# hashicorp/consul

Measured on NVIDIA H100. Metric: million node-ticks/sec, higher is better.
Workload: dtype u32

## Files before the change

__graft_entry__.py:

```python
from __future__ import annotations

import os
import subprocess
import sys

ROOT = os.path.dirname(os.path.abspath(__file__))
CSRC = os.path.join(ROOT, "consul_b200", "csrc")
LIBGSIM = os.path.join(ROOT, "consul_b200", "libgsim.so")
LIBORACLE = os.path.join(ROOT, "oracle", "liboracle.so")
LIBHOSTEMU = os.path.join(ROOT, "tests", "hostemu", "libgsim_hostemu.so")
LIBHOSTEMU_COUNTED = os.path.join(ROOT, "tests", "hostemu", "libgsim_hostemu_counted.so")
FACADE_DEMO = os.path.join(ROOT, "tests", "hostemu", "serf_facade_check")

NVCC_FLAGS = ["-gencode", "arch=compute_90a,code=sm_90a", "-lineinfo", "-O3", "-std=c++17", "-fmad=false",
              "-Xcompiler", "-fPIC", "-Xcompiler", "-ffp-contract=off", "-Xcompiler", "-pthread", "-shared"]


def _newer(target: str, sources) -> bool:
    if not os.path.exists(target):
        return False
    t = os.path.getmtime(target)
    return all(os.path.getmtime(s) <= t for s in sources)


def _run(cmd):
    print("+", " ".join(cmd), flush=True)
    subprocess.run(cmd, check=True, cwd=ROOT)


def _sources(*dirs_and_ext):
    out = []
    for d, exts in dirs_and_ext:
        for f in sorted(os.listdir(d)):
            if f.endswith(exts):
                out.append(os.path.join(d, f))
    return out


def build_oracle(force: bool = False) -> None:
    hdr = _sources((os.path.join(ROOT, "include"), (".h",)))
    osrc = [os.path.join(ROOT, "oracle", "oracle.cpp")]
    if force or not _newer(LIBORACLE, osrc + hdr):
        _run(["g++", "-O3", "-mavx2", "-ffp-contract=off", "-std=c++17", "-fopenmp", "-fPIC", "-shared", "-o",
              LIBORACLE] + osrc)


LIBORACLE_IMPAIR = os.path.join(ROOT, "tests", "oracle_impair", "liboracle_impair.so")
IMPAIR_PATCH = os.path.join(ROOT, "tests", "oracle_impair", "impair.patch")


def _apply_patch(text: str, patch: str, name: str = IMPAIR_PATCH) -> str:
    hunks, cur = [], None
    for line in patch.splitlines(keepends=True):
        if line.startswith("@@"):
            cur = ([], [])
            hunks.append(cur)
        elif cur is not None and line[:1] in (" ", "-", "+"):
            if line[:1] != "+":
                cur[0].append(line[1:])
            if line[:1] != "-":
                cur[1].append(line[1:])
    for old, new in hunks:
        old, new = "".join(old), "".join(new)
        if text.count(old) != 1:
            raise RuntimeError(f"{name}: a hunk does not apply to oracle/oracle.cpp")
        text = text.replace(old, new)
    return text


def build_impair_oracle(force: bool = False) -> None:
    import tempfile
    hdr = _sources((os.path.join(ROOT, "include"), (".h",)))
    osrc = [os.path.join(ROOT, "oracle", "oracle.cpp"), IMPAIR_PATCH]
    if not force and _newer(LIBORACLE_IMPAIR, osrc + hdr):
        return
    with open(osrc[0]) as f, open(IMPAIR_PATCH) as pf:
        text = _apply_patch(f.read(), pf.read())
    with tempfile.TemporaryDirectory() as tmp:
        src = os.path.join(tmp, "oracle_impair.cpp")
        with open(src, "w") as f:
            f.write(text)
        _run(["g++", "-O3", "-mavx2", "-ffp-contract=off", "-std=c++17", "-fopenmp", "-fPIC", "-shared",
              "-I", os.path.join(ROOT, "oracle"), "-o", LIBORACLE_IMPAIR, src])


LIBORACLE_PAUSE = os.path.join(ROOT, "tests", "oracle_pause", "liboracle_pause.so")
PAUSE_PATCH = os.path.join(ROOT, "tests", "oracle_pause", "pause.patch")


def build_pause_oracle(force: bool = False) -> None:
    import tempfile
    hdr = _sources((os.path.join(ROOT, "include"), (".h",)))
    osrc = [os.path.join(ROOT, "oracle", "oracle.cpp"), IMPAIR_PATCH, PAUSE_PATCH]
    if not force and _newer(LIBORACLE_PAUSE, osrc + hdr):
        return
    with open(osrc[0]) as f, open(IMPAIR_PATCH) as pf, open(PAUSE_PATCH) as qf:
        text = _apply_patch(_apply_patch(f.read(), pf.read()), qf.read(), PAUSE_PATCH)
    with tempfile.TemporaryDirectory() as tmp:
        src = os.path.join(tmp, "oracle_pause.cpp")
        with open(src, "w") as f:
            f.write(text)
        _run(["g++", "-O3", "-mavx2", "-ffp-contract=off", "-std=c++17", "-fopenmp", "-fPIC", "-shared",
              "-I", os.path.join(ROOT, "oracle"), "-o", LIBORACLE_PAUSE, src])


LIBORACLE_REACH = os.path.join(ROOT, "tests", "oracle_reach", "liboracle_reach.so")
REACH_PATCH = os.path.join(ROOT, "tests", "oracle_reach", "reach.patch")


def build_reach_oracle(force: bool = False) -> None:
    import tempfile
    hdr = _sources((os.path.join(ROOT, "include"), (".h",)))
    osrc = [os.path.join(ROOT, "oracle", "oracle.cpp"), IMPAIR_PATCH, PAUSE_PATCH, REACH_PATCH]
    if not force and _newer(LIBORACLE_REACH, osrc + hdr):
        return
    with open(osrc[0]) as f, open(IMPAIR_PATCH) as pf, open(PAUSE_PATCH) as qf, open(REACH_PATCH) as rf:
        text = _apply_patch(_apply_patch(_apply_patch(f.read(), pf.read()), qf.read(), PAUSE_PATCH), rf.read(),
                            REACH_PATCH)
    with tempfile.TemporaryDirectory() as tmp:
        src = os.path.join(tmp, "oracle_reach.cpp")
        with open(src, "w") as f:
            f.write(text)
        _run(["g++", "-O3", "-mavx2", "-ffp-contract=off", "-std=c++17", "-fopenmp", "-fPIC", "-shared",
              "-I", os.path.join(ROOT, "oracle"), "-o", LIBORACLE_REACH, src])


LIBORACLE_PIGGYBACK = os.path.join(ROOT, "tests", "oracle_piggyback", "liboracle_piggyback.so")
PIGGYBACK_PATCH = os.path.join(ROOT, "tests", "oracle_piggyback", "piggyback.patch")


def build_piggyback_oracle(force: bool = False) -> None:
    import tempfile
    hdr = _sources((os.path.join(ROOT, "include"), (".h",)))
    patches = [IMPAIR_PATCH, PAUSE_PATCH, REACH_PATCH, PIGGYBACK_PATCH]
    osrc = [os.path.join(ROOT, "oracle", "oracle.cpp")] + patches
    if not force and _newer(LIBORACLE_PIGGYBACK, osrc + hdr):
        return
    with open(osrc[0]) as f:
        text = f.read()
    for patch in patches:
        with open(patch) as pf:
            text = _apply_patch(text, pf.read(), patch)
    with tempfile.TemporaryDirectory() as tmp:
        src = os.path.join(tmp, "oracle_piggyback.cpp")
        with open(src, "w") as f:
            f.write(text)
        _run(["g++", "-O3", "-mavx2", "-ffp-contract=off", "-std=c++17", "-fopenmp", "-fPIC", "-shared",
              "-I", os.path.join(ROOT, "oracle"), "-o", LIBORACLE_PIGGYBACK, src])


def build(force: bool = False) -> None:
    hdr = _sources((CSRC, (".h",)), (os.path.join(ROOT, "include"), (".h", ".hpp")))
    srcs = [os.path.join(CSRC, "gs_cuda.cu"), os.path.join(CSRC, "gs_vmm.cu"), os.path.join(CSRC, "gs_api.cpp")]
    if force or not _newer(LIBGSIM, srcs + hdr):
        nvcc = os.environ.get("NVCC", "nvcc")
        _run([nvcc] + NVCC_FLAGS + ["-o", LIBGSIM] + srcs)
    build_oracle(force)
    build_impair_oracle(force)
    build_pause_oracle(force)
    build_reach_oracle(force)
    build_piggyback_oracle(force)
    hsrc = [os.path.join(CSRC, "gs_api.cpp"), os.path.join(ROOT, "tests", "hostemu", "hostemu_backend.cpp")]
    if force or not _newer(LIBHOSTEMU, hsrc + hdr):
        _run(["g++", "-O2", "-ffp-contract=off", "-std=c++17", "-pthread", "-fPIC", "-shared",
              "-DGS_MAKE_BACKEND=gs_make_hostemu_backend", "-o", LIBHOSTEMU] + hsrc)
    csrc = hsrc + [os.path.join(ROOT, "tests", "hostemu", "stretch_counting.cpp")]
    if force or not _newer(LIBHOSTEMU_COUNTED, csrc + hdr + [os.path.join(ROOT, "tests", "hostemu", "counting_backend.cpp")]):
        _run(["g++", "-O2", "-ffp-contract=off", "-std=c++17", "-pthread", "-fPIC", "-shared",
              "-DGS_MAKE_BACKEND=gs_make_stretch_counting_backend", "-o", LIBHOSTEMU_COUNTED] + csrc)
    sys.path.insert(0, ROOT)
    import consul_b200


def smoke() -> None:
    sys.path.insert(0, ROOT)
    sys.path.insert(0, os.path.join(ROOT, "tests"))
    if not (os.path.exists(LIBGSIM) and os.path.exists(LIBORACLE)):
        build()
    from consul_b200 import Pool, lan_config, PRED_ALL_RUMORS_CONVERGED
    from oracle_binding import OraclePool

    n = 4096
    cfg = lan_config(capacity=n + 1, n_initial=n, seed=0x5EED0001)
    gpu = Pool(cfg)
    ora = OraclePool(cfg)
    for p in (gpu, ora):
        x = p.member_add()
        assert p.join(x, [0]) == 1
    tg = gpu.run_until(PRED_ALL_RUMORS_CONVERGED, 0, 400, 1)
    to = ora.run_until(PRED_ALL_RUMORS_CONVERGED, 0, 400, 1)
    gpu.step(64)
    ora.step(64)
    hg, ho = gpu.state_hash(), ora.state_hash()
    assert tg == to, (tg, to)
    assert hg == ho, (hg, ho)
    assert gpu.launch_count() > 0
    print(f"smoke ok: n={n + 1} converged at tick {tg}, state hash {hg[0]:016x} == oracle, "
          f"{gpu.launch_count()} kernel launches")


if __name__ == "__main__":
    build(force="--force" in sys.argv)
    if "--smoke" in sys.argv:
        smoke()
```

consul_b200/csrc/gs_cuda.cu:

```cuda
#include <cuda_runtime.h>
#include <stdio.h>
#include <stdlib.h>
#include <string.h>

#include <map>

#include "gs_aux.h"
#include "gs_backend.h"
#include "gs_query.h"
#include "gs_vmm.h"

#define GS_BLOCK 256
#define GS_GRAPH_TICKS 64
#define GS_WIN_GRAPH 8
#ifndef GS_STRETCH_TICKS
#define GS_STRETCH_TICKS 16
#endif

namespace {

template <bool COORDS>
struct DevSinkT {
  static constexpr bool kCoords = COORDS;
  uint32_t* s_stat;
  uint32_t* s_heard;
  uint32_t* s_q;
  __device__ __forceinline__ void activity() { s_q[0] = 1u; }
  __device__ __forceinline__ void horizon(uint32_t h) { atomicMin(&s_q[1], h); }
  __device__ __forceinline__ void stat(int idx, uint32_t v) { atomicAdd(&s_stat[idx * 32 + (threadIdx.x & 31u)], v); }
  __device__ __forceinline__ void heard(uint32_t r) { atomicAdd(&s_heard[r * 32u + (threadIdx.x & 31u)], 1u); }
  __device__ __forceinline__ void crashed_dead(const GsDev& d, uint32_t t) {
    uint32_t old = atomicSub_system(d.crashed_alive, 1u);
    if (old == 1u) *d.crashed_dead_tick = t;
  }
  __device__ __forceinline__ void log_event(const GsDev& d, const GsGlobals& g, uint32_t t,
                                            uint32_t type, uint32_t subject, uint32_t observer,
                                            uint32_t ltime) {
    uint32_t pos = atomicAdd_system(&d.evlog_cursor[0], 1u);
    if (pos < g.evlog_cap) {
      GsEventRec e;
      e.tick = t;
      e.type = type;
      e.subject = subject;
      e.observer = observer;
      e.ltime = ltime;
      e.reserved = 0u;
      d.evlog[pos] = e;
    } else {
      atomicAdd_system(&d.evlog_cursor[1], 1u);
    }
  }
};
typedef DevSinkT<false> DevSink;

#ifndef GS_MIN_BLOCKS
#define GS_MIN_BLOCKS 4
#endif
#define GS_WARPS (GS_BLOCK / 32)
#define GS_ROUND 4

__device__ __forceinline__ uint32_t gs_smem_addr(const void* p) { return (uint32_t)__cvta_generic_to_shared(p); }
__device__ __forceinline__ void gs_mbar_init(uint64_t* bar, uint32_t arrivals) {
  asm volatile("mbarrier.init.shared::cta.b64 [%0], %1;" ::"r"(gs_smem_addr(bar)), "r"(arrivals) : "memory");
}
__device__ __forceinline__ void gs_mbar_expect_tx(uint64_t* bar, uint32_t bytes) {
  asm volatile("mbarrier.arrive.expect_tx.shared::cta.b64 _, [%0], %1;" ::"r"(gs_smem_addr(bar)), "r"(bytes) : "memory");
}
__device__ __forceinline__ void gs_bulk_g2s(void* smem_dst, const void* gsrc, uint32_t bytes, uint64_t* bar) {
  asm volatile("cp.async.bulk.shared::cluster.global.mbarrier::complete_tx::bytes [%0], [%1], %2, [%3];" ::"r"(
                   gs_smem_addr(smem_dst)),
               "l"(gsrc), "r"(bytes), "r"(gs_smem_addr(bar))
               : "memory");
}
__device__ __forceinline__ bool gs_mbar_wait(uint64_t* bar, uint32_t parity) {
  for (uint32_t spin = 0; spin < (1u << 24); ++spin) {
    uint32_t done;
    asm volatile(
        "{\n\t.reg .pred p;\n\t"
        "mbarrier.try_wait.parity.shared::cta.b64 p, [%1], %2;\n\t"
        "selp.u32 %0, 1, 0, p;\n\t}"
        : "=r"(done)
        : "r"(gs_smem_addr(bar)), "r"(parity)
        : "memory");
    if (done) return true;
  }
  return false;
}

__device__ __forceinline__ void gs_ranks_wait(const GsDev& d, const GsGlobals& g, uint32_t t) {
  if (threadIdx.x < g.world) {
    uint32_t v;
    do {
      asm volatile("ld.acquire.sys.global.u32 %0, [%1];" : "=r"(v) : "l"(d.tick_flags[g.rank] + threadIdx.x) : "memory");
    } while ((int32_t)(v - t) < 0);
  }
  __syncthreads();
}
__device__ __forceinline__ void gs_ranks_release(const GsDev& d, const GsGlobals& g, uint32_t t_done) {
  __syncthreads();
  if (threadIdx.x == 0u) {
    __threadfence_system();
    const uint32_t arrived = atomicAdd(d.done_ctr, 1u);
    if (arrived == gridDim.x - 1u) {
      __threadfence_system();
      *d.done_ctr = 0u;
      __threadfence_system();
      for (uint32_t r = 0; r < g.world; ++r)
        asm volatile("st.release.sys.global.u32 [%0], %1;" ::"l"(d.tick_flags[r] + g.rank), "r"(t_done) : "memory");
    }
  }
}

__device__ __forceinline__ void gs_q_publish(const GsDev& d, const GsGlobals& g, const uint32_t* s_q, uint32_t t) {
  if (s_q[0] != 0u) {
    if (g.world <= 1u) atomicMax(d.qstate[0] + GS_Q_LAST_ACTIVE, t + 1u);
    else for (uint32_t r = 0; r < g.world; ++r) atomicMax_system(d.qstate[r] + GS_Q_LAST_ACTIVE, t + 1u);
  }
  if (s_q[1] != GS_NEVER) {
    if (g.world <= 1u) atomicMin(d.qstate[0] + GS_Q_HORIZON, s_q[1]);
    else for (uint32_t r = 0; r < g.world; ++r) atomicMin_system(d.qstate[r] + GS_Q_HORIZON, s_q[1]);
  }
}

template <bool COORDS>
__device__ __noinline__ void gs_row_step_impaired_call(const GsDev* dp, const GsGlobals* gp, uint32_t i, uint32_t t,
                                                       uint32_t inb, uint32_t* s_stat, uint32_t* s_heard, uint32_t* s_q) {
  DevSinkT<COORDS> sink{s_stat, s_heard, s_q};
  gs_row_step_body<true>(*dp, *gp, i, t, t % gp->GI, inb, sink);
}
template <bool COORDS, bool IMPAIRED>
__device__ __noinline__ void gs_row_step_pig_call(const GsDev* dp, const GsGlobals* gp, uint32_t i, uint32_t t,
                                                  uint32_t inb, uint32_t* s_stat, uint32_t* s_heard, uint32_t* s_q) {
  DevSinkT<COORDS> sink{s_stat, s_heard, s_q};
  gs_row_step_body<IMPAIRED, true>(*dp, *gp, i, t, t % gp->GI, inb, sink);
}
template <bool COORDS>
__device__ __noinline__ void gs_row_step_call(const GsDev* dp, const GsGlobals* gp, uint32_t i, uint32_t t,
                                              uint32_t inb, uint32_t* s_stat, uint32_t* s_heard, uint32_t* s_q) {
  if (dp->imp_loss != nullptr) {
    gs_row_step_impaired_call<COORDS>(dp, gp, i, t, inb, s_stat, s_heard, s_q);
    return;
  }
  DevSinkT<COORDS> sink{s_stat, s_heard, s_q};
  gs_row_step_body<false>(*dp, *gp, i, t, t % gp->GI, inb, sink);
}

template <bool COORDS>
__device__ __forceinline__ void gs_row_step_any(const GsDev* dp, const GsGlobals* gp, uint32_t i, uint32_t t,
                                                uint32_t inb, uint32_t* s_stat, uint32_t* s_heard, uint32_t* s_q) {
  if (dp->pig == nullptr) gs_row_step_call<COORDS>(dp, gp, i, t, inb, s_stat, s_heard, s_q);
  else if (dp->imp_loss != nullptr) gs_row_step_pig_call<COORDS, true>(dp, gp, i, t, inb, s_stat, s_heard, s_q);
  else gs_row_step_pig_call<COORDS, false>(dp, gp, i, t, inb, s_stat, s_heard, s_q);
}

struct GsStretchCtl {
  GsStretch out;
  uint32_t violation;
  uint32_t end, floor, depth;
};
__device__ __forceinline__ uint32_t gs_stretch_stop(const GsStretchCtl& c, uint32_t last_active) {
  const uint32_t quiet_at = (last_active > c.floor ? last_active : c.floor) + c.depth;
  return quiet_at < c.end ? quiet_at : c.end;
}

template <bool COORDS>
__global__ void __launch_bounds__(GS_BLOCK, GS_MIN_BLOCKS)
    gs_tick_kernel(const __grid_constant__ GsDev d, const GsGlobals* __restrict__ gp, uint32_t k_off,
                   const GsStretchCtl* __restrict__ stretch) {
  __shared__ uint32_t s_stat[GS_NSTAT * 32];
  __shared__ uint32_t s_heard[32 * 32];
  __shared__ __align__(128) uint32_t s_inb[GS_WARPS][GS_ROUND][GS_TILE];
  __shared__ __align__(128) uint32_t s_due[GS_WARPS][GS_ROUND][GS_TILE];
  __shared__ __align__(8) uint64_t s_bar[GS_WARPS];
  __shared__ uint32_t s_q[2];
  __shared__ uint16_t s_work[GS_WARPS * GS_ROUND * GS_TILE];
  __shared__ uint32_t s_rtile[GS_WARPS];
  __shared__ uint32_t s_wn[2], s_wtake[2];
  static_assert(GS_WARPS <= 8 && GS_ROUND <= 4 && GS_TILE == 128, "s_work entries are 3 + 2 + 7 bits");
  const uint32_t tid = threadIdx.x;
  for (uint32_t x = tid; x < GS_NSTAT * 32u; x += GS_BLOCK) s_stat[x] = 0u;
  for (uint32_t x = tid; x < 32u * 32u; x += GS_BLOCK) s_heard[x] = 0u;
  if (tid == 64u) s_q[0] = 0u;
  if (tid == 65u) s_q[1] = GS_NEVER;
  if (tid >= 66u && tid < 68u) s_wn[tid - 66u] = 0u;
  if (tid >= 68u && tid < 70u) s_wtake[tid - 68u] = 0u;
  if (tid >= 96u && tid < 96u + GS_WARPS) gs_mbar_init(&s_bar[tid - 96u], 1u);
  asm volatile("fence.mbarrier_init.release.cluster;" ::: "memory");
  asm volatile("griddepcontrol.launch_dependents;" ::: "memory");
  asm volatile("griddepcontrol.wait;" ::: "memory");
  if (stretch != nullptr && *d.tick_base + k_off >= gs_stretch_stop(*stretch, __ldcg(d.qstate[0] + GS_Q_LAST_ACTIVE)))
    return;
  __syncthreads();
  const GsGlobals& g = *gp;
  const uint32_t t = *d.tick_base + k_off;
  if (g.world > 1u) gs_ranks_wait(d, g, t);
  const uint32_t cur = t & 1u, P = g.P, pslot = t % P, gslot = t % g.GI;
  const uint32_t pslot_t = (t + P - g.T % P) % P;
  const uint32_t lane = tid & 31u, wib = tid >> 5;
  uint32_t tile_lo = 0, tile_hi = (g.n + GS_TILE - 1u) / GS_TILE;
  if (g.world > 1u) {
    const uint32_t per = g.rows_per_rank / GS_TILE;
    tile_lo = g.rank * per < tile_hi ? g.rank * per : tile_hi;
    tile_hi = tile_lo + per < tile_hi ? tile_lo + per : tile_hi;
  }
  const uint32_t n_warps = gridDim.x * GS_WARPS, n_tiles = tile_hi - tile_lo;
  const uint32_t wid = blockIdx.x * GS_WARPS + wib;
  const uint32_t t_begin = tile_lo + (uint32_t)(((uint64_t)wid * n_tiles) / n_warps);
  const uint32_t t_end = tile_lo + (uint32_t)(((uint64_t)(wid + 1u) * n_tiles) / n_warps);
  const uint32_t* __restrict__ inbox_cur = d.inbox[t & g.ring_mask];
  const bool gated = g.phase_gate != 0u;
  const uint32_t shift = g.phase_shift;
  DevSinkT<COORDS> sink{s_stat, s_heard, s_q};

  const uint32_t max_run = (n_tiles + n_warps - 1u) / n_warps, n_rounds = (max_run + GS_ROUND - 1u) / GS_ROUND;
  bool did_work = false;
  const bool sys_scan = g.world > 1u && (g.flags & 4u);
  auto bring = [&](uint32_t r) {
    const uint32_t b0 = t_begin + r * GS_ROUND < t_end ? t_begin + r * GS_ROUND : t_end;
    const uint32_t b1 = b0 + GS_ROUND < t_end ? b0 + GS_ROUND : t_end;
    const uint32_t tiles = b1 - b0;
    if (!tiles) return;
    uint32_t gate_mask = 0;
    for (uint32_t x = 0; x < tiles; ++x) {
      bool gate = true;
      if (gated) {
        const uint32_t pp = gs_probe_phase(g.rot_p, (b0 + x) >> shift, P);
        gate = pp == pslot || pp == pslot_t;
      }
      gate_mask |= gate ? 1u << x : 0u;
    }
    const size_t off0 = (size_t)b0 * GS_TILE;
    if (sys_scan) {
      for (uint32_t x = 0; x < tiles; ++x) {
        uint4 v;
        asm volatile("ld.relaxed.sys.global.v4.u32 {%0,%1,%2,%3}, [%4];"
                     : "=r"(v.x), "=r"(v.y), "=r"(v.z), "=r"(v.w) : "l"(inbox_cur + off0 + x * GS_TILE + lane * 4u) : "memory");
        *reinterpret_cast<uint4*>(&s_inb[wib][x][lane * 4u]) = v;
        const uint4 dv = (gate_mask >> x) & 1u ? *reinterpret_cast<const uint4*>(d.due + off0 + x * GS_TILE + lane * 4u)
                                               : make_uint4(GS_NEVER, GS_NEVER, GS_NEVER, GS_NEVER);
        *reinterpret_cast<uint4*>(&s_due[wib][x][lane * 4u]) = dv;
      }
      __syncwarp();
      return;
    }
    for (uint32_t x = 0; x < tiles; ++x)
      if (!((gate_mask >> x) & 1u))
        *reinterpret_cast<uint4*>(&s_due[wib][x][lane * 4u]) = make_uint4(GS_NEVER, GS_NEVER, GS_NEVER, GS_NEVER);
    __syncwarp();
    if (lane == 0u) {
      asm volatile("fence.proxy.async.shared::cta;" ::: "memory");
      gs_mbar_expect_tx(&s_bar[wib], (tiles + __popc(gate_mask)) * GS_TILE * 4u);
      gs_bulk_g2s(&s_inb[wib][0][0], inbox_cur + off0, tiles * GS_TILE * 4u, &s_bar[wib]);
      for (uint32_t x = 0; x < tiles; ++x)
        if ((gate_mask >> x) & 1u) gs_bulk_g2s(&s_due[wib][x][0], d.due + off0 + x * GS_TILE, GS_TILE * 4u, &s_bar[wib]);
    }
  };
  bring(0u);
  for (uint32_t round = 0; round < n_rounds; ++round) {
  const uint32_t par = round & 1u;
  const uint32_t r_begin = t_begin + round * GS_ROUND < t_end ? t_begin + round * GS_ROUND : t_end;
  const uint32_t r_end = r_begin + GS_ROUND < t_end ? r_begin + GS_ROUND : t_end;
  if (r_end > r_begin && !sys_scan && !gs_mbar_wait(&s_bar[wib], round & 1u)) {
    if (lane == 0u) atomicExch(d.qstate[g.rank] + GS_Q_VIOLATION, t + 1u);
  }
  for (uint32_t tile = r_begin; tile < r_end; ++tile) {
    const uint32_t st = tile - r_begin;
    uint4 i4 = *reinterpret_cast<const uint4*>(&s_inb[wib][st][lane * 4u]);
    const uint4 d4 = *reinterpret_cast<const uint4*>(&s_due[wib][st][lane * 4u]);
    if (__any_sync(0xFFFFFFFFu, (i4.x | i4.y | i4.z | i4.w) != 0u)) {
      const uint32_t m0 = tile * GS_TILE + lane * 4u;
      const uint4 h4 = __ldcg(reinterpret_cast<const uint4*>(d.heard + m0));
      uint32_t* const w_cur = d.inbox[t & g.ring_mask] + m0;
      uint32_t* const w4 = &i4.x;
      const uint32_t* const h = &h4.x;
      const uint32_t* const du = &d4.x;
      bool stale_any = false;
#pragma unroll
      for (uint32_t u = 0; u < 4u; ++u) {
        const bool pp = g.pp_interval != 0u && gs_pp_due(g.pp_interval, g.rot_pp, (m0 + u) / g.phase_group, t);
        if (w4[u] != 0u && gs_mail_is_stale(g, w4[u], h[u], du[u] == t, pp)) {
          w_cur[u] = 0u;
          s_inb[wib][st][lane * 4u + u] = 0u;
          w4[u] = 0u;
          stale_any = true;
        }
      }
      if (stale_any) sink.activity();
    }
    bool mine = (i4.x | i4.y | i4.z | i4.w) != 0u || d4.x == t || d4.y == t || d4.z == t || d4.w == t;
    bool pp_tile = false;
    if (g.pp_interval != 0u) {
      if (gated) {
        pp_tile = gs_pp_due(g.pp_interval, g.rot_pp, tile >> shift, t);
      } else {
#pragma unroll
        for (uint32_t u = 0; u < 4u; ++u)
          pp_tile |= gs_pp_due(g.pp_interval, g.rot_pp, (tile * GS_TILE + lane * 4u + u) / g.phase_group, t);
      }
      mine |= pp_tile;
    }
    if (__any_sync(0xFFFFFFFFu, mine)) {
      did_work = true;
      __syncwarp();
      const uint32_t base = tile * GS_TILE + lane;
      bool act[4], cand[4];
      bool any_cand = false;
#pragma unroll
      for (int u = 0; u < 4; ++u) {
        const uint32_t w = s_inb[wib][st][u * 32 + lane];
        const bool due_now = s_due[wib][st][u * 32 + lane] == t;
        act[u] = w != 0u || due_now ||
                 (g.pp_interval != 0u && gs_pp_due(g.pp_interval, g.rot_pp, (base + 32u * u) / g.phase_group, t));
        cand[u] = w == 0u && due_now;
        any_cand |= cand[u];
      }
      if (__any_sync(0xFFFFFFFFu, any_cand)) {
        GsFastProbe f[4];
#pragma unroll
        for (int u = 0; u < 4; ++u)
          if (cand[u]) gs_fast_load(d, cur, base + 32u * u, f[u]);
#pragma unroll
        for (int u = 0; u < 4; ++u)
          if (cand[u]) cand[u] = gs_fast_target(d, g, cur, base + 32u * u, f[u]);
        uint32_t n_probe = 0, n_ack = 0;
#pragma unroll
        for (int u = 0; u < 4; ++u) {
          bool acked = false;
          const bool done = cand[u] && gs_fast_finish(d, g, sink, base + 32u * u, t, f[u], &acked);
          if (done) act[u] = false;
          n_probe += __popc(__ballot_sync(0xFFFFFFFFu, done));
          n_ack += __popc(__ballot_sync(0xFFFFFFFFu, done && acked));
        }
        if (lane == 0u && n_probe) {
          atomicAdd(&s_stat[GS_ST_PROBES * 32], n_probe);
          atomicAdd(&s_stat[GS_ST_ACTIVE_ROWS * 32], n_probe);
          if (n_ack) atomicAdd(&s_stat[GS_ST_ACKS * 32], n_ack);
        }
      }
      uint32_t bal[4], n_act = 0;
#pragma unroll
      for (int u = 0; u < 4; ++u) {
        bal[u] = __ballot_sync(0xFFFFFFFFu, act[u]);
        n_act += __popc(bal[u]);
      }
      if (n_act) {
        uint32_t pos = 0;
        if (lane == 0u) pos = atomicAdd(&s_wn[par], n_act);
        pos = __shfl_sync(0xFFFFFFFFu, pos, 0);
        const uint32_t below = (1u << lane) - 1u, key = (wib << 9) | (st << 7) | lane;
#pragma unroll
        for (int u = 0; u < 4; ++u) {
          if (act[u]) s_work[pos + __popc(bal[u] & below)] = (uint16_t)(key | ((uint32_t)u << 5));
          pos += __popc(bal[u]);
        }
      }
    }
  }
  if (lane == 0u) s_rtile[wib] = r_begin;
  __syncwarp();
  if (round + 1u < n_rounds) bring(round + 1u);
  __syncthreads();
  if (tid == 0u) s_wn[par ^ 1u] = s_wtake[par ^ 1u] = 0u;
  const uint32_t n_work = s_wn[par];
  for (;;) {
    uint32_t idx = 0;
    if (lane == 0u) idx = atomicAdd(&s_wtake[par], 32u);
    idx = __shfl_sync(0xFFFFFFFFu, idx, 0);
    if (idx >= n_work) break;
    did_work = true;
    if (idx + lane < n_work) {
      const uint32_t e = s_work[idx + lane];
      const uint32_t i = (s_rtile[e >> 9] + ((e >> 7) & 3u)) * GS_TILE + (e & 127u);
      gs_row_step_any<COORDS>(&d, gp, i, t, __ldcg(inbox_cur + i), s_stat, s_heard, s_q);
    }
  }
  __syncthreads();
  }
  if (g.world > 1u && did_work && !(g.flags & 8u)) __threadfence_system();
  __syncthreads();
  if (tid < GS_NSTAT) {
    uint32_t v = 0;
    for (uint32_t x = 0; x < 32u; ++x) v += s_stat[tid * 32u + ((x + tid) & 31u)];
    if (v) atomicAdd(&d.stats[tid], (unsigned long long)v);
  } else if (tid >= 32u && tid < 32u + GS_MAX_RUMORS) {
    uint32_t r = tid - 32u, c = 0;
    for (uint32_t x = 0; x < 32u; ++x) c += s_heard[r * 32u + ((x + r) & 31u)];
    if (c) {
      uint32_t old = atomicAdd_system(&d.heard_cnt[r], c);
      if (old + c == g.up_count) d.conv_tick[r] = t;
    }
  }
  if (tid == 0u) gs_q_publish(d, g, s_q, t);
  if (g.world > 1u) gs_ranks_release(d, g, t + 1u);
}

template <bool COORDS>
__device__ __noinline__ void gs_window_generic(const GsDev* dp, const GsGlobals* gp, uint32_t gb, uint32_t g_end,
                                               uint32_t tf00, uint32_t tf01, uint32_t tf02, uint32_t tf03,
                                               uint32_t tx00, uint32_t tx01, uint32_t tx02, uint32_t tx03,
                                               uint32_t t0, uint32_t w1, uint32_t* s_stat, uint32_t* s_heard,
                                               uint32_t* s_q, uint32_t* counts) {
  const GsDev& d = *dp;
  const GsGlobals& g = *gp;
  const GsHot h = gs_hot(g);
  const uint32_t P = h.P, T = h.T, lane = threadIdx.x & 31u;
  const uint32_t tf0[4] = {tf00, tf01, tf02, tf03}, tx0[4] = {tx00, tx01, tx02, tx03};
  const bool fast_ok =
      h.loss_thr == 0u && h.graph_n == 0u && d.coord == nullptr && d.imp_loss == nullptr && h.pp_interval == 0u;
  DevSinkT<COORDS> sink{s_stat, s_heard, s_q};
  uint32_t n_probe = 0, n_ack = 0;
  bool did_work = false;
  (void)did_work;
#pragma unroll 1
    for (uint32_t s0 = t0; s0 < w1; s0 += P) {
    const uint32_t off = s0 - t0;
    uint32_t tf[4], tx[4], due[4];
    bool cand[4], slow[4];
    bool any_slow = false;
#pragma unroll
    for (int u = 0; u < 4; ++u) {
      if (gb + u < g_end) {
        tf[u] = tf0[u] + off;
        tx[u] = tx0[u] + off;
        due[u] = __ldcg(d.due + (gb + u) * 32u + lane);
      } else {
        tf[u] = tx[u] = GS_NEVER;
        due[u] = GS_NEVER - 1u;
      }
      cand[u] = fast_ok && due[u] == tf[u] && tf[u] < w1;
      slow[u] = (due[u] == tf[u] && tf[u] < w1 && !fast_ok) || (due[u] == tx[u] && tx[u] < w1);
    }
    GsFastProbe f[4];
#pragma unroll
    for (int u = 0; u < 4; ++u)
      if (cand[u]) gs_fast_load(d, tf[u] & 1u, (gb + u) * 32u + lane, f[u]);
#pragma unroll
    for (int u = 0; u < 4; ++u)
      if (cand[u]) {
        const bool okk = gs_fast_target(d, h, tf[u] & 1u, (gb + u) * 32u + lane, f[u]);
        if (!okk) { cand[u] = false; slow[u] = true; }
      }
#pragma unroll
    for (int u = 0; u < 4; ++u) {
      bool acked = false, done = false;
      if (cand[u]) {
        done = gs_fast_finish(d, h, sink, (gb + u) * 32u + lane, tf[u], f[u], &acked);
        if (!done) slow[u] = true;
        else if (!acked && tf[u] + T < w1) slow[u] = true;
      }
      n_probe += done ? 1u : 0u;
      n_ack += done && acked ? 1u : 0u;
      any_slow |= slow[u];
    }
    if (__any_sync(0xFFFFFFFFu, any_slow)) {
      did_work = true;
#pragma unroll 1
      for (int u = 0; u < 4; ++u) {
        const bool sl = u == 0 ? slow[0] : u == 1 ? slow[1] : u == 2 ? slow[2] : slow[3];
        if (!__any_sync(0xFFFFFFFFu, sl)) continue;
        const uint32_t a = u == 0 ? tf[0] : u == 1 ? tf[1] : u == 2 ? tf[2] : tf[3];
        const uint32_t b = u == 0 ? tx[0] : u == 1 ? tx[1] : u == 2 ? tx[2] : tx[3];
        const uint32_t i = (gb + u) * 32u + lane;
#pragma unroll 1
        for (int which = 0; which < 2; ++which) {
          const uint32_t t = which == 0 ? (a < b ? a : b) : (a < b ? b : a);
          if (t >= w1) break;
          if (sl && __ldcg(d.due + i) == t) gs_row_step_any<COORDS>(&d, gp, i, t, 0u, s_stat, s_heard, s_q);
        }
      }
    }
    }
  counts[0] = n_probe;
  counts[1] = n_ack;
}

#ifndef GS_WIN_BLOCKS
#define GS_WIN_BLOCKS 4
#endif
#ifndef GS_WIN_BLOCKS_CLOSED
#define GS_WIN_BLOCKS_CLOSED 4
#endif

template <bool COORDS, bool PRISTINE>
__global__ void __launch_bounds__(GS_BLOCK, PRISTINE ? GS_WIN_BLOCKS_CLOSED : GS_WIN_BLOCKS)
    gs_window_kernel(const __grid_constant__ GsDev d, const GsGlobals* __restrict__ gp, uint32_t k_off, uint32_t n_ticks,
                     uint32_t mode) {
  __shared__ uint32_t s_stat[GS_NSTAT * 32];
  __shared__ uint32_t s_heard[32 * 32];
  __shared__ uint32_t s_q[2];
  __shared__ uint32_t s_spec[GS_MAX_SPECIAL + 1];
  const uint32_t tid = threadIdx.x;
  for (uint32_t x = tid; x < GS_NSTAT * 32u; x += GS_BLOCK) s_stat[x] = 0u;
  for (uint32_t x = tid; x < 32u * 32u; x += GS_BLOCK) s_heard[x] = 0u;
  if (tid == 64u) s_q[0] = 0u;
  if (tid == 65u) s_q[1] = GS_NEVER;
  asm volatile("griddepcontrol.launch_dependents;" ::: "memory");
  asm volatile("griddepcontrol.wait;" ::: "memory");
  if (tid == 66u) s_spec[GS_MAX_SPECIAL] = gs_special_members(*gp, s_spec);
  __syncthreads();
  const GsGlobals& g = *gp;
  const GsHot h = gs_hot(g);
  const bool cyclic = (mode & 2u) != 0u;
  const uint32_t world = g.world, rank = g.rank, n_spec = s_spec[GS_MAX_SPECIAL];
  uint32_t* const qs = d.qstate[rank];
  const uint32_t t0 = *d.tick_base + k_off;
  const uint32_t reached = __ldcg(qs + GS_Q_WIN_END), horizon = __ldcg(qs + GS_Q_HORIZON);
  if (reached < t0) return;
  uint32_t w1 = t0 + n_ticks;
  if (horizon < w1) w1 = horizon;
  if (w1 <= t0) return;
  if (world > 1u) gs_ranks_wait(d, g, t0);
  const uint32_t P = h.P, T = h.T, lane = tid & 31u, wib = tid >> 5;
  uint32_t tile_lo = 0, tile_hi = (h.n + GS_TILE - 1u) / GS_TILE;
  if (world > 1u) {
    const uint32_t per = g.rows_per_rank / GS_TILE;
    tile_lo = rank * per < tile_hi ? rank * per : tile_hi;
    tile_hi = tile_lo + per < tile_hi ? tile_lo + per : tile_hi;
  }
  const uint32_t n_warps = gridDim.x * GS_WARPS, grp_lo = tile_lo * 4u, grp_hi = tile_hi * 4u;
  const uint32_t run = (grp_hi - grp_lo + n_warps - 1u) / n_warps;
  const uint32_t wid = blockIdx.x * GS_WARPS + wib;
  const uint32_t g_begin = grp_lo + wid * run < grp_hi ? grp_lo + wid * run : grp_hi;
  const uint32_t g_end = g_begin + run < grp_hi ? g_begin + run : grp_hi;
  const uint32_t shift = g.phase_shift + 2u, t0_mod = t0 % P, rot_p = g.rot_p;
  const uint32_t win_q = (w1 - t0) / P, win_r = (w1 - t0) - win_q * P;
  const bool fast_ok =
      h.loss_thr == 0u && h.graph_n == 0u && d.coord == nullptr && d.imp_loss == nullptr && h.pp_interval == 0u;
  DevSinkT<COORDS> sink{s_stat, s_heard, s_q};
  bool did_work = false;
  uint32_t n_probe = 0, n_ack = 0;
  uint32_t pg = g_begin >> shift;
  uint32_t pp = (pg % P + rot_p) % P;
  const uint32_t g_first = cyclic ? (grp_lo + wid * 4u < grp_hi ? grp_lo + wid * 4u : grp_hi) : g_begin;
  const uint32_t g_step = cyclic ? n_warps * 4u : 4u, g_lim = cyclic ? grp_hi : g_end;
  for (uint32_t gb = g_first; gb < g_lim; gb += g_step) {
    if (cyclic) {
      pg = gb >> shift;
      pp = (pg % P + rot_p) % P;
    }
    uint32_t tf0[4], tx0[4];
#pragma unroll
    for (int u = 0; u < 4; ++u) {
      const uint32_t grp = gb + u;
      if (grp < g_lim) {
        const uint32_t q = grp >> shift;
        if (q != pg) {
          pp = pp + 1u == P ? 0u : pp + 1u;
          pg = q;
        }
        uint32_t a = pp + P - t0_mod;
        a = a >= P ? a - P : a;
        uint32_t b = a + T;
        b = b >= P ? b - P : b;
        tf0[u] = t0 + a;
        tx0[u] = t0 + b;
      } else {
        tf0[u] = tx0[u] = GS_NEVER;
      }
    }
    uint32_t lo = t0;
#pragma unroll 1
    for (;;) {
      uint32_t stuck = GS_NEVER;
      if constexpr (PRISTINE) {
        uint32_t cnt = 0;
        uint32_t du[4], kk[4], mm[4], cu[4], pa[4];
#pragma unroll
        for (int u = 0; u < 4; ++u) {
          const uint32_t i = (gb + u) * 32u + lane;
          du[u] = GS_NEVER;
          kk[u] = mm[u] = cu[u] = pa[u] = 0u;
          if (gb + u < g_lim) {
            du[u] = __ldcg(d.due + i);
            if (fast_ok) {
              kk[u] = d.key[tf0[u] & 1u][i];
              mm[u] = d.meta[i];
              cu[u] = d.cursor[i];
              pa[u] = d.pass[i];
            }
          }
        }
#pragma unroll
        for (int u = 0; u < 4; ++u) {
          if (gb + u >= g_lim) continue;
          const uint32_t i = (gb + u) * 32u + lane;
          uint32_t due = du[u];
          if (fast_ok && due >= lo && due < w1) {
            uint32_t later = 0u;
            bool on_phase = due == tf0[u];
            if (!on_phase && due > tf0[u]) {
              later = (due - tf0[u]) / P;
              on_phase = later * P == due - tf0[u];
            }
            if (on_phase) {
              const uint32_t k0 = ((due ^ tf0[u]) & 1u) ? d.key[due & 1u][i] : kk[u];
              const uint32_t m = mm[u];
              if (gs_key_truth(k0) == GS_TRUTH_UP && gs_key_rank(k0) == GS_RANK_ALIVE && gs_meta_stage(m) == GS_STAGE_IDLE &&
                  !(m & (GS_META_DIRTY | GS_META_ISOLATED))) {
                const GsU4 rk = gs_perm_keys(h.seed_lo, h.seed_hi, i, pa[u]);
                const uint32_t kt = win_q + (win_r > tf0[u] - t0 ? 1u : 0u) - later;
                const uint32_t k = gs_pristine_probes_k(h.n, h.perm_bits, rk, i, cu[u], kt, s_spec, n_spec);
                if (k) {
                  const uint32_t aw = gs_meta_aw(m);
                  if (aw) d.meta[i] = gs_meta_set_aw(m, aw > k ? aw - k : 0u);
                  d.cursor[i] = cu[u] + k;
                  due += k * P;
                  d.due[i] = due;
                  cnt += k;
                }
              }
            }
          }
          if (due >= lo && due < w1 && due < stuck) stuck = due;
        }
        n_probe += cnt;
        n_ack += cnt;
      } else
      {
        uint32_t mm[4], cu[4], du[4], m_in[4], cu_in[4], du_in[4], kt[4];
        GsU4 rk[4];
        bool live[4], in_rng[4];
        uint32_t cnt = 0;
        {
          uint32_t kk[4], pa[4];
#pragma unroll
          for (int u = 0; u < 4; ++u) {
            const uint32_t i = (gb + u) * 32u + lane;
            in_rng[u] = gb + u < g_lim;
            du[u] = GS_NEVER;
            kk[u] = mm[u] = cu[u] = pa[u] = 0u;
            if (in_rng[u]) {
              du[u] = __ldcg(d.due + i);
              if (fast_ok) {
                kk[u] = d.key[tf0[u] & 1u][i];
                mm[u] = d.meta[i];
                cu[u] = d.cursor[i];
                pa[u] = d.pass[i];
              }
            }
          }
#pragma unroll
          for (int u = 0; u < 4; ++u) {
            const uint32_t i = (gb + u) * 32u + lane;
            live[u] = false;
            kt[u] = 0u;
            m_in[u] = mm[u];
            cu_in[u] = cu[u];
            du_in[u] = du[u];
            if (!in_rng[u] || !fast_ok || du[u] < lo || du[u] >= w1) continue;
            uint32_t later = 0u;
            if (du[u] != tf0[u]) {
              if (du[u] < tf0[u]) continue;
              later = (du[u] - tf0[u]) / P;
              if (later * P != du[u] - tf0[u]) continue;
            }
            const uint32_t k = ((du[u] ^ tf0[u]) & 1u) ? d.key[du[u] & 1u][i] : kk[u];
            live[u] = gs_key_truth(k) == GS_TRUTH_UP && gs_key_rank(k) == GS_RANK_ALIVE &&
                      gs_meta_stage(mm[u]) == GS_STAGE_IDLE && !(mm[u] & (GS_META_DIRTY | GS_META_ISOLATED));
            rk[u] = gs_perm_keys(h.seed_lo, h.seed_hi, i, pa[u]);
            kt[u] = win_q + (win_r > tf0[u] - t0 ? 1u : 0u) - later;
          }
        }
        for (;;) {
          bool go[4];
          bool any = false;
#pragma unroll
          for (int u = 0; u < 4; ++u) {
            go[u] = live[u] && du[u] < w1;
            any |= go[u];
          }
          if (!__any_sync(0xFFFFFFFFu, any)) break;
          uint32_t c[4], kc[4];
#pragma unroll
          for (int u = 0; u < 4; ++u) {
            c[u] = 0u;
            if (go[u]) {
              if (cu[u] >= h.n) {
                live[u] = go[u] = false;
              } else {
                c[u] = gs_perm(cu[u], h.n, h.perm_bits, rk[u]);
                if (c[u] == (gb + u) * 32u + lane) live[u] = go[u] = false;
              }
            }
          }
#pragma unroll
          for (int u = 0; u < 4; ++u) kc[u] = go[u] ? gs_peer_key(d, du[u] & 1u, c[u], false) : 0u;
#pragma unroll
          for (int u = 0; u < 4; ++u) {
            if (!go[u]) continue;
            const uint32_t i = (gb + u) * 32u + lane;
            if (gs_key_truth(kc[u]) != GS_TRUTH_UP || gs_key_rank(kc[u]) != GS_RANK_ALIVE || gs_key_pending(kc[u]) ||
                gs_extra(h, nullptr, i, c[u]) + gs_extra(h, nullptr, c[u], i) > T) {
              live[u] = false;
              continue;
            }
            const uint32_t aw = gs_meta_aw(mm[u]);
            mm[u] = gs_meta_set_aw(mm[u], aw ? aw - 1u : 0u);
            du[u] += P;
            cu[u] += 1u;
            ++cnt;
          }
        }
#pragma unroll
        for (int u = 0; u < 4; ++u) {
          if (!in_rng[u]) continue;
          const uint32_t i = (gb + u) * 32u + lane;
          if (cu[u] != cu_in[u]) d.cursor[i] = cu[u];
          if (du[u] != du_in[u]) d.due[i] = du[u];
          if (mm[u] != m_in[u]) d.meta[i] = mm[u];
          if (du[u] >= lo && du[u] < w1 && du[u] < stuck) stuck = du[u];
        }
        n_probe += cnt;
        n_ack += cnt;
      }
      stuck = __reduce_min_sync(0xFFFFFFFFu, stuck);
      if (stuck == GS_NEVER) break;
      {
        const uint32_t off = (stuck - t0) / P * P, s_lo = t0 + off, s_hi = s_lo + P < w1 ? s_lo + P : w1;
        uint32_t add[2] = {0u, 0u};
        gs_window_generic<COORDS>(&d, gp, gb, g_lim, tf0[0] + off, tf0[1] + off, tf0[2] + off, tf0[3] + off, tx0[0] + off,
                                  tx0[1] + off, tx0[2] + off, tx0[3] + off, s_lo, s_hi, s_stat, s_heard, s_q, add);
        n_probe += add[0];
        n_ack += add[1];
        did_work = true;
        lo = s_lo + P;
        if (lo >= w1) break;
      }
    }
  }
  did_work |= n_probe != 0u;
  if (n_probe) {
    atomicAdd(&s_stat[GS_ST_PROBES * 32 + lane], n_probe);
    atomicAdd(&s_stat[GS_ST_ACTIVE_ROWS * 32 + lane], n_probe);
    if (n_ack) atomicAdd(&s_stat[GS_ST_ACKS * 32 + lane], n_ack);
  }
  if (world > 1u && did_work) __threadfence_system();
  __syncthreads();
  if (tid < GS_NSTAT) {
    uint32_t v = 0;
    for (uint32_t x = 0; x < 32u; ++x) v += s_stat[tid * 32u + ((x + tid) & 31u)];
    if (v) atomicAdd(&d.stats[tid], (unsigned long long)v);
  }
  if (tid == 0u) {
    if (s_q[0] != 0u || (n_ticks > P && s_q[1] != GS_NEVER)) atomicExch(qs + GS_Q_VIOLATION, t0 + 1u);
    s_q[0] = 0u;
    gs_q_publish(d, g, s_q, t0);
    atomicMax(qs + GS_Q_WIN_END, w1);
  }
  if (world > 1u) gs_ranks_release(d, g, w1);
}

__global__ void __launch_bounds__(GS_BLOCK)
    gs_quiet_scan_kernel(GsDev d, const GsGlobals* __restrict__ gp, uint32_t now, const uint32_t* now_at, uint32_t first,
                         uint32_t count) {
  __shared__ uint32_t s_min;
  if (threadIdx.x == 0u) s_min = GS_NEVER;
  __syncthreads();
  const GsGlobals& g = *gp;
  if (now_at != nullptr) now = *now_at;
  uint32_t h = GS_NEVER;
  for (uint32_t x = blockIdx.x * GS_BLOCK + threadIdx.x; x < count; x += gridDim.x * GS_BLOCK) {
    const uint32_t i = first + x;
    if (i >= g.n) break;
    if (gs_key_truth(d.key[now & 1u][i]) != GS_TRUTH_UP) continue;
    const uint32_t stage = gs_meta_stage(d.meta[i]);
    if (stage == GS_STAGE_IDLE) continue;
    const uint32_t due = d.due[i];
    const uint32_t e = stage == GS_STAGE_WAIT_T ? due - g.T + g.P : due;
    if (e < h) h = e;
  }
  h = __reduce_min_sync(0xFFFFFFFFu, h);
  if ((threadIdx.x & 31u) == 0u && h != GS_NEVER) atomicMin(&s_min, h);
  __syncthreads();
  if (threadIdx.x == 0u && s_min != GS_NEVER) {
    if (g.world <= 1u) atomicMin(d.qstate[0] + GS_Q_HORIZON, s_min);
    else for (uint32_t r = 0; r < g.world; ++r) atomicMin_system(d.qstate[r] + GS_Q_HORIZON, s_min);
  }
}

__global__ void gs_window_advance_kernel(uint32_t* tick_base, const uint32_t* qs) { *tick_base = qs[GS_Q_WIN_END]; }

__global__ void gs_advance_kernel(uint32_t* tick_base, uint32_t k, uint32_t* done_ctr) {
  *tick_base += k;
  if (done_ctr) *done_ctr = 0u;
}

__global__ void gs_stretch_begin_kernel(GsStretchCtl* c, uint32_t end, uint32_t floor, uint32_t depth) {
  c->out = GsStretch();
  c->violation = 0u;
  c->end = end;
  c->floor = floor;
  c->depth = depth;
}
__global__ void gs_stretch_pass_kernel(uint32_t* tick_base, const uint32_t* qs, GsStretchCtl* c, uint32_t k,
                                       cudaGraphConditionalHandle loop) {
  const uint32_t t = *tick_base, la = qs[GS_Q_LAST_ACTIVE];
  const uint32_t stop = gs_stretch_stop(*c, la);
  const uint32_t ran = stop <= t ? 0u : stop - t < k ? stop - t : k;
  *tick_base = t + ran;
  c->out.ran += ran;
  c->out.launches += k;
  if (t + ran >= stop || qs[GS_Q_VIOLATION] != 0u) {
    c->out.last_active = la;
    c->out.quiet = t + ran >= (la > c->floor ? la : c->floor) + c->depth ? 1u : 0u;
    c->violation = qs[GS_Q_VIOLATION];
    cudaGraphSetConditional(loop, 0u);
  }
}
__global__ void gs_stretch_end_kernel(const GsStretchCtl* c, uint32_t* qs, cudaGraphConditionalHandle probe) {
  if (c->out.quiet && !c->violation) {
    qs[GS_Q_HORIZON] = GS_NEVER;
    cudaGraphSetConditional(probe, 1u);
  }
}

__global__ void gs_xbar_kernel(GsXbar xb) {
  const uint32_t lane = threadIdx.x;
  const uint32_t e = *xb.epoch + 1u;
  __threadfence_system();
  if (lane < xb.world) {
    asm volatile("st.release.sys.global.u32 [%0], %1;" ::"l"(xb.flags[lane] + xb.rank), "r"(e) : "memory");
    uint32_t v;
    do {
      asm volatile("ld.acquire.sys.global.u32 %0, [%1];" : "=r"(v) : "l"(xb.flags[xb.rank] + lane) : "memory");
    } while ((int32_t)(v - e) < 0);
  }
  __syncwarp();
  __threadfence_system();
  if (lane == 0) *xb.epoch = e;
}

__global__ void __launch_bounds__(GS_BLOCK)
    gs_init_kernel(GsDev d, const GsGlobals* __restrict__ gp, uint32_t first, uint32_t count,
                   uint32_t now) {
  uint32_t x = blockIdx.x * GS_BLOCK + threadIdx.x;
  if (x < count) gs_init_row(d, *gp, first + x, now);
}

__global__ void __launch_bounds__(GS_BLOCK)
    gs_crash_kernel(GsDev d, const GsGlobals* __restrict__ gp, uint32_t thr, uint32_t salt,
                    uint32_t* n_crashed) {
  uint32_t i = blockIdx.x * GS_BLOCK + threadIdx.x;
  bool c = false;
  if (i < gp->n) c = gs_crash_row(d, *gp, i, thr, salt);
  unsigned b = __ballot_sync(0xFFFFFFFFu, c);
  if ((threadIdx.x & 31u) == 0u && b) atomicAdd(n_crashed, (uint32_t)__popc(b));
}

__global__ void __launch_bounds__(GS_BLOCK)
    gs_impair_kernel(GsDev d, const GsGlobals* __restrict__ gp, GsImpairCols c, uint32_t thr, uint32_t salt,
                     GsImpairVal v, uint32_t* counts) {
  const uint32_t i = blockIdx.x * GS_BLOCK + threadIdx.x;
  uint32_t r = 0u;
  if (i < gp->n) r = gs_impair_row(d.key[0][i], c, gp->seed_lo, gp->seed_hi, i, thr, salt, v);
  const unsigned sel = __ballot_sync(0xFFFFFFFFu, r & 1u), was = __ballot_sync(0xFFFFFFFFu, r & 2u);
  if ((threadIdx.x & 31u) == 0u && sel) {
    atomicAdd(&counts[0], (uint32_t)__popc(sel));
    if (was) atomicAdd(&counts[1], (uint32_t)__popc(was));
  }
}

__global__ void __launch_bounds__(GS_BLOCK)
    gs_pause_kernel(GsDev d, const GsGlobals* __restrict__ gp, uint32_t* pause_until, const uint32_t* __restrict__ ids,
                    uint32_t n, uint32_t thr, uint32_t salt, uint32_t until, uint32_t* n_paused) {
  const uint32_t x = blockIdx.x * GS_BLOCK + threadIdx.x;
  const GsGlobals& g = *gp;
  bool c = false;
  if (ids != nullptr) {
    if (x < n) c = gs_pause_row(d, g, pause_until, ids[x], until);
  } else if (x < g.n && gs_pause_pick(g, x, thr, salt)) {
    c = gs_pause_row(d, g, pause_until, x, until);
  }
  const unsigned b = __ballot_sync(0xFFFFFFFFu, c);
  if ((threadIdx.x & 31u) == 0u && b) atomicAdd(n_paused, (uint32_t)__popc(b));
}

__global__ void __launch_bounds__(GS_BLOCK)
    gs_resume_kernel(GsDev d, const GsGlobals* __restrict__ gp, uint32_t* pause_until, uint32_t t, uint32_t resume,
                     uint32_t log_events, uint32_t* counts) {
  const uint32_t i = blockIdx.x * GS_BLOCK + threadIdx.x;
  uint32_t r = 0u;
  if (i < gp->n) r = gs_resume_row(d, *gp, pause_until, i, t, resume != 0u);
  if (r == GS_RESUMED_DEAD && log_events) {
    DevSink sink{nullptr, nullptr, nullptr};
    sink.log_event(d, *gp, t, GS_EV_MEMBER_JOIN, i, GS_EMPTY32, 0u);
  }
  if (__ballot_sync(0xFFFFFFFFu, r != 0u) == 0u) return;
  for (uint32_t c = 0; c < 4u; ++c) {
    const unsigned b = __ballot_sync(0xFFFFFFFFu, r == c + 1u);
    if ((threadIdx.x & 31u) == 0u && b) atomicAdd(&counts[c], (uint32_t)__popc(b));
  }
}

__global__ void __launch_bounds__(GS_BLOCK)
    gs_reap_kernel(GsDev d, const GsGlobals* __restrict__ gp, uint32_t now, uint32_t reconnect_ticks,
                   uint32_t tombstone_ticks, uint32_t log_events, uint32_t* counts) {
  const uint32_t i = blockIdx.x * GS_BLOCK + threadIdx.x;
  uint32_t r = 0;
  if (i < gp->n) r = gs_reap_row(d, *gp, i, now, reconnect_ticks, tombstone_ticks);
  if (r && log_events) {
    DevSink sink{nullptr, nullptr, nullptr};
    sink.log_event(d, *gp, now, GS_EV_MEMBER_REAP, i, GS_EMPTY32, 0u);
  }
  const unsigned b0 = __ballot_sync(0xFFFFFFFFu, (r & 1u) != 0u), b1 = __ballot_sync(0xFFFFFFFFu, (r & 2u) != 0u);
  if ((threadIdx.x & 31u) == 0u) {
    if (b0) atomicAdd(&counts[0], (uint32_t)__popc(b0));
    if (b1) atomicAdd(&counts[1], (uint32_t)__popc(b1));
  }
}

__global__ void __launch_bounds__(GS_BLOCK)
    gs_recount_kernel(GsDev d, const GsGlobals* __restrict__ gp, uint32_t now, const uint32_t* now_at, uint32_t first,
                      uint32_t count, GsRecount* out) {
  __shared__ GsRecount s;
  uint32_t* sw = reinterpret_cast<uint32_t*>(&s);
  for (uint32_t x = threadIdx.x; x < sizeof(GsRecount) / 4; x += GS_BLOCK) sw[x] = 0u;
  __syncthreads();
  const GsGlobals& g = *gp;
  if (now_at != nullptr) now = *now_at;
  const uint32_t x = blockIdx.x * GS_BLOCK + threadIdx.x, i = first + x;
  if (x < count && i < g.n) {
    uint32_t k = d.key[now & 1u][i];
    uint32_t truth = gs_key_truth(k), rank = gs_key_rank(k);
    atomicAdd(&s.truth_cnt[truth], 1u);
    if (truth != GS_TRUTH_NONE) atomicAdd(&s.rank_cnt[rank], 1u);
    if (truth == GS_TRUTH_CRASHED && rank < GS_RANK_DEAD) atomicAdd(&s.crashed_alive, 1u);
    if ((truth == GS_TRUTH_CRASHED || truth == GS_TRUTH_GONE) && rank < GS_RANK_DEAD) atomicAdd(&s.unreachable_live, 1u);
    if (truth == GS_TRUTH_UP && (d.meta[i] & GS_META_ISOLATED)) atomicAdd(&s.isolated_up, 1u);
    if (truth != GS_TRUTH_NONE && gs_key_pending(k)) atomicAdd(&s.pending, 1u);
    if (truth == GS_TRUTH_UP && g.active_mask) {
      uint32_t h = d.heard[i] & g.active_mask, q = d.queued[i] & g.active_mask;
      while (h) {
        uint32_t r = __ffs(h) - 1;
        h &= h - 1;
        atomicAdd(&s.heard_cnt[r], 1u);
      }
      while (q) {
        uint32_t r = __ffs(q) - 1;
        q &= q - 1;
        atomicAdd(&s.queued_cnt[r], 1u);
      }
    }
  }
  __syncthreads();
  uint32_t* ow = reinterpret_cast<uint32_t*>(out);
  for (uint32_t x = threadIdx.x; x < sizeof(GsRecount) / 4; x += GS_BLOCK)
    if (sw[x]) atomicAdd(&ow[x], sw[x]);
}

__global__ void __launch_bounds__(GS_BLOCK)
    gs_hash_kernel(GsDev d, const GsGlobals* __restrict__ gp, uint32_t now,
                   unsigned long long* out) {
  __shared__ unsigned long long s[4];
  if (threadIdx.x < 4) s[threadIdx.x] = 0ull;
  __syncthreads();
  uint32_t i = blockIdx.x * GS_BLOCK + threadIdx.x;
  if (i < gp->n) {
    uint64_t h = gs_hash_row(d, *gp, i, now);
    if (h) {
      uint64_t lanes[4];
      gs_hash_lanes(h, lanes);
      for (int q = 0; q < 4; ++q) atomicAdd(&s[q], (unsigned long long)lanes[q]);
    }
  }
  __syncthreads();
  if (threadIdx.x < 4 && s[threadIdx.x]) atomicAdd(&out[threadIdx.x], s[threadIdx.x]);
}

static cudaError_t gs_launch_tick(uint32_t blocks, cudaStream_t stream, const GsDev& d,
                                  const GsGlobals* g_dev, uint32_t k, bool pdl,
                                  const GsStretchCtl* stretch = nullptr) {
  cudaLaunchConfig_t cfg = {};
  cfg.gridDim = dim3(blocks);
  cfg.blockDim = dim3(GS_BLOCK);
  cfg.dynamicSmemBytes = 0;
  cfg.stream = stream;
  cudaLaunchAttribute attr[1];
  attr[0].id = cudaLaunchAttributeProgrammaticStreamSerialization;
  attr[0].val.programmaticStreamSerializationAllowed = 1;
  cfg.attrs = attr;
  cfg.numAttrs = pdl ? 1 : 0;
  return d.coord ? cudaLaunchKernelEx(&cfg, gs_tick_kernel<true>, d, g_dev, k, stretch)
                 : cudaLaunchKernelEx(&cfg, gs_tick_kernel<false>, d, g_dev, k, stretch);
}

static cudaError_t gs_launch_window(uint32_t blocks, cudaStream_t stream, const GsDev& d, const GsGlobals* g_dev,
                                    uint32_t k_off, uint32_t n_ticks, bool pdl, uint32_t mode) {
  cudaLaunchConfig_t cfg = {};
  cfg.gridDim = dim3(blocks);
  cfg.blockDim = dim3(GS_BLOCK);
  cfg.dynamicSmemBytes = 0;
  cfg.stream = stream;
  cudaLaunchAttribute attr[1];
  attr[0].id = cudaLaunchAttributeProgrammaticStreamSerialization;
  attr[0].val.programmaticStreamSerializationAllowed = 1;
  cfg.attrs = attr;
  cfg.numAttrs = pdl ? 1 : 0;
  if (mode & 1u)
    return d.coord ? cudaLaunchKernelEx(&cfg, gs_window_kernel<true, true>, d, g_dev, k_off, n_ticks, mode)
                   : cudaLaunchKernelEx(&cfg, gs_window_kernel<false, true>, d, g_dev, k_off, n_ticks, mode);
  return d.coord ? cudaLaunchKernelEx(&cfg, gs_window_kernel<true, false>, d, g_dev, k_off, n_ticks, mode)
                 : cudaLaunchKernelEx(&cfg, gs_window_kernel<false, false>, d, g_dev, k_off, n_ticks, mode);
}

#define GS_ROWS_MAX 64u
struct GsRowIds {
  uint32_t n;
  uint32_t id[GS_ROWS_MAX];
};
__global__ void gs_rows_read_kernel(GsDev d, GsRowIds r, uint32_t* out) {
  const uint32_t* col[8] = {d.key[0], d.key[1], d.meta, d.heard, d.queued, d.ltime_member, d.ltime_event, d.event_min};
  const uint32_t t = threadIdx.x;
  if (t < r.n * 8u) out[t] = col[t & 7u][r.id[t >> 3]];
}

__global__ void gs_write_batch_kernel(const __grid_constant__ GsWriteBatch b) {
  for (uint32_t k = 0; k < b.n; ++k) gs_apply_write(b.op[k]);
  __threadfence_system();
}

__global__ void gs_copy_word_kernel(uint32_t* dst, const uint32_t* src) { *dst = *src; }

__global__ void __launch_bounds__(GS_BLOCK) gs_fill32_kernel(uint32_t* dst, uint32_t value, size_t count) {
  for (size_t x = (size_t)blockIdx.x * GS_BLOCK + threadIdx.x; x < count; x += (size_t)gridDim.x * GS_BLOCK)
    dst[x] = value;
}

__global__ void __launch_bounds__(GS_BLOCK) gs_and_kernel(GsDev d, uint32_t first, uint32_t count, uint32_t keep) {
  const uint32_t x = blockIdx.x * GS_BLOCK + threadIdx.x, i = first + x;
  if (x >= count) return;
  uint32_t v;
  v = d.heard[i];
  if (v & ~keep) d.heard[i] = v & keep;
  v = d.queued[i];
  if (v & ~keep) d.queued[i] = v & keep;
  for (uint32_t s = 0; s < GS_RING_MAX && d.inbox[s] != nullptr; ++s) {
    v = d.inbox[s][i];
    if (v & ~keep) d.inbox[s][i] = v & keep;
  }
}

__global__ void __launch_bounds__(GS_BLOCK)
    gs_coord_rows_kernel(GsDev d, uint32_t cap, uint32_t first, uint32_t count, double* rows) {
  __shared__ GsCoord s[GS_BLOCK];
  const uint32_t x0 = blockIdx.x * GS_BLOCK;
  const uint32_t m = count - x0 < GS_BLOCK ? count - x0 : GS_BLOCK;
  if (threadIdx.x < m) gs_coord_pick(d.coord, d.ctag, cap, first + x0 + threadIdx.x, s[threadIdx.x]);
  __syncthreads();
  const double* sw = reinterpret_cast<const double*>(s);
  double* out = rows + (size_t)x0 * GS_COORD_WORDS;
  for (uint32_t t = threadIdx.x; t < m * GS_COORD_WORDS; t += GS_BLOCK) out[t] = sw[t];
}

__global__ void __launch_bounds__(GS_BLOCK)
    gs_coord_pairs_kernel(GsDev d, const GsGlobals* __restrict__ gp, const uint32_t* a, const uint32_t* b, uint32_t n,
                          double* est, double* tru) {
  const uint32_t k = blockIdx.x * GS_BLOCK + threadIdx.x;
  if (k >= n) return;
  const GsGlobals& g = *gp;
  const uint32_t i = a[k], j = b[k];
  GsCoord ci, cj;
  gs_coord_pick(d.coord, d.ctag, g.cap, i, ci);
  gs_coord_pick(d.coord, d.ctag, g.cap, j, cj);
  est[k] = gs_coord_distance_seconds(ci, cj);
  if (tru != nullptr) tru[k] = gs_model_rtt(g, d.imp_delay, i, j);
}

__global__ void __launch_bounds__(GS_BLOCK)
    gs_coord_dist_kernel(GsDev d, const GsGlobals* __restrict__ gp, uint32_t now, uint32_t from, const uint32_t* ids,
                         uint32_t n, uint32_t router, uint64_t* key, uint32_t* val) {
  const uint32_t x = blockIdx.x * GS_BLOCK + threadIdx.x;
  if (x >= n) return;
  const GsGlobals& g = *gp;
  GsCoord cf;
  gs_coord_pick(d.coord, d.ctag, g.cap, from, cf);
  const uint32_t s = ids != nullptr ? ids[x] : x;
  uint64_t k;
  uint32_t v = s;
  if (router) {
    gs_router_entry(d, g, now, from, cf, s, &k, &v);
  } else {
    GsCoord c;
    gs_coord_pick(d.coord, d.ctag, g.cap, s, c);
    k = gs_dist_key(gs_coord_distance_seconds(cf, c));
  }
  if (v != GS_EMPTY32 && !gs_dist_key_ok(k)) __trap();
  key[x] = k;
  val[x] = v;
}

__global__ void __launch_bounds__(GS_BLOCK)
    gs_coord_error_kernel(GsDev d, const GsGlobals* __restrict__ gp, uint32_t now, uint32_t n_draws, uint32_t salt,
                          uint64_t* key, uint32_t* val, double* part) {
  static_assert(GS_ERR_CHUNK == GS_BLOCK, "one CTA per chunk of draws");
  __shared__ double s[GS_BLOCK];
  const uint32_t k = blockIdx.x * GS_BLOCK + threadIdx.x;
  double e = -1.0;
  if (k < n_draws) {
    e = gs_error_draw(d, *gp, now, k, salt);
    const uint64_t bits = e < 0.0 ? ~0ull : gs_dist_key(e);
    if (e >= 0.0 && !gs_dist_key_ok(bits)) __trap();
    key[k] = bits;
    val[k] = k;
  }
  s[threadIdx.x] = e;
  __syncthreads();
  if (threadIdx.x == 0) {
    double sum = 0.0, kept = 0.0;
    for (uint32_t x = 0; x < GS_BLOCK; ++x)
      if (s[x] >= 0.0) {
        sum = sum + s[x];
        kept += 1.0;
      }
    part[blockIdx.x] = sum;
    part[gridDim.x + blockIdx.x] = kept;
  }
}

__global__ void gs_coord_error_finish_kernel(const uint64_t* sorted, uint32_t n_draws, const double* part, double* out) {
  gs_error_finish(sorted, n_draws, part, out);
}

__global__ void gs_dc_medians_kernel(const uint64_t* key, const uint32_t* val, uint32_t n, uint32_t n_dcs, double* med,
                                     uint32_t* cnt) {
  const uint32_t c = threadIdx.x;
  if (c >= n_dcs) return;
  uint32_t lo = 0, hi = n;
  while (lo < hi) {
    const uint32_t mid = lo + (hi - lo) / 2u;
    if (gs_dc_digit(val[mid], n_dcs) < c) lo = mid + 1u; else hi = mid;
  }
  uint32_t end = lo, top = n;
  while (end < top) {
    const uint32_t mid = end + (top - end) / 2u;
    if (gs_dc_digit(val[mid], n_dcs) <= c) end = mid + 1u; else top = mid;
  }
  cnt[c] = end - lo;
  med[c] = end > lo ? gs_key_dist(key[lo + (end - lo) / 2u]) : gs_key_dist(0x7FF0000000000000ull);
}

#define GS_RS_TILE 4096u
#define GS_RS_PASSES 9u
struct GsRsCtl {
  uint32_t skip[GS_RS_PASSES];
  uint32_t src[GS_RS_PASSES];
  uint32_t fin;
};
struct GsRsBufs {
  uint64_t* key[2];
  uint32_t* val[2];
};

__device__ __forceinline__ uint32_t gs_rs_digit(uint64_t k, uint32_t v, uint32_t p, uint32_t n_dcs) {
  return p < 8u ? (uint32_t)(k >> (8u * p)) & 255u : gs_dc_digit(v, n_dcs);
}

__global__ void __launch_bounds__(GS_BLOCK)
    gs_rs_hist_kernel(const uint64_t* key, const uint32_t* val, uint32_t n, uint32_t n_dcs, uint32_t np, uint32_t* ghist) {
  __shared__ uint32_t s[GS_RS_PASSES * 256];
  for (uint32_t x = threadIdx.x; x < np * 256u; x += GS_BLOCK) s[x] = 0u;
  __syncthreads();
  for (size_t x = (size_t)blockIdx.x * GS_BLOCK + threadIdx.x; x < n; x += (size_t)gridDim.x * GS_BLOCK) {
    const uint64_t k = key[x];
    const uint32_t v = np > 8u ? val[x] : 0u;
    for (uint32_t p = 0; p < np; ++p) atomicAdd(&s[p * 256u + gs_rs_digit(k, v, p, n_dcs)], 1u);
  }
  __syncthreads();
  for (uint32_t x = threadIdx.x; x < np * 256u; x += GS_BLOCK)
    if (s[x]) atomicAdd(&ghist[x], s[x]);
}

__global__ void gs_rs_plan_kernel(const uint32_t* ghist, uint32_t n, uint32_t np, GsRsCtl* c) {
  uint32_t src = 0u;
  for (uint32_t p = 0; p < np; ++p) {
    uint32_t top = 0u;
    for (uint32_t dg = 0; dg < 256u; ++dg) top = ghist[p * 256u + dg] > top ? ghist[p * 256u + dg] : top;
    c->skip[p] = top == n ? 1u : 0u;
    c->src[p] = src;
    if (top != n) src ^= 1u;
  }
  c->fin = src;
}

__global__ void __launch_bounds__(GS_BLOCK)
    gs_rs_upsweep_kernel(GsRsBufs b, const GsRsCtl* c, uint32_t p, uint32_t n, uint32_t n_dcs, uint32_t* hist) {
  if (c->skip[p]) return;
  __shared__ uint32_t s[256];
  s[threadIdx.x] = 0u;
  __syncthreads();
  const uint64_t* key = b.key[c->src[p]];
  const uint32_t* val = b.val[c->src[p]];
  const size_t t0 = (size_t)blockIdx.x * GS_RS_TILE, t1 = t0 + GS_RS_TILE < n ? t0 + GS_RS_TILE : n;
  for (size_t x = t0 + threadIdx.x; x < t1; x += GS_BLOCK)
    atomicAdd(&s[gs_rs_digit(key[x], p == 8u ? val[x] : 0u, p, n_dcs)], 1u);
  __syncthreads();
  hist[(size_t)threadIdx.x * gridDim.x + blockIdx.x] = s[threadIdx.x];
}

__device__ __forceinline__ uint32_t gs_block_scan(uint32_t v, uint32_t* sw, uint32_t* total) {
  const uint32_t lane = threadIdx.x & 31u, w = threadIdx.x >> 5;
  uint32_t incl = v;
  for (uint32_t o = 1; o < 32u; o <<= 1) {
    const uint32_t y = __shfl_up_sync(0xFFFFFFFFu, incl, o);
    if (lane >= o) incl += y;
  }
  if (lane == 31u) sw[w] = incl;
  __syncthreads();
  if (w == 0) {
    uint32_t t = lane < GS_WARPS ? sw[lane] : 0u, ti = t;
    for (uint32_t o = 1; o < 32u; o <<= 1) {
      const uint32_t y = __shfl_up_sync(0xFFFFFFFFu, ti, o);
      if (lane >= o) ti += y;
    }
    if (lane < GS_WARPS) sw[lane] = ti - t;
    if (lane == GS_WARPS - 1u) sw[GS_WARPS] = ti;
  }
  __syncthreads();
  const uint32_t r = sw[w] + incl - v;
  *total = sw[GS_WARPS];
  __syncthreads();
  return r;
}

__global__ void __launch_bounds__(GS_BLOCK) gs_rs_scan_kernel(const GsRsCtl* c, uint32_t p, uint32_t nb, uint32_t* hist) {
  if (c->skip[p]) return;
  __shared__ uint32_t sw[GS_WARPS + 1];
  uint32_t* row = hist + (size_t)blockIdx.x * nb;
  uint32_t carry = 0u;
  for (uint32_t x0 = 0; x0 < nb; x0 += GS_BLOCK) {
    const uint32_t x = x0 + threadIdx.x;
    const uint32_t v = x < nb ? row[x] : 0u;
    uint32_t total;
    const uint32_t e = gs_block_scan(v, sw, &total);
    if (x < nb) row[x] = carry + e;
    carry += total;
  }
}

__global__ void __launch_bounds__(GS_BLOCK)
    gs_rs_scatter_kernel(GsRsBufs b, const GsRsCtl* c, uint32_t p, uint32_t n, uint32_t n_dcs, const uint32_t* hist,
                         const uint32_t* ghist) {
  if (c->skip[p]) return;
  __shared__ uint32_t base[256];
  __shared__ uint32_t wcnt[GS_WARPS][256];
  __shared__ uint32_t woff[GS_WARPS][256];
  __shared__ uint32_t sw[GS_WARPS + 1];
  const uint32_t tid = threadIdx.x, lane = tid & 31u, w = tid >> 5;
  uint32_t total;
  const uint32_t before = gs_block_scan(ghist[p * 256u + tid], sw, &total);
  base[tid] = before + hist[(size_t)tid * gridDim.x + blockIdx.x];
  for (uint32_t q = 0; q < GS_WARPS; ++q) wcnt[q][tid] = 0u;
  __syncthreads();
  const uint32_t s = c->src[p];
  const uint64_t* ks = b.key[s];
  const uint32_t* vs = b.val[s];
  uint64_t* kd = b.key[s ^ 1u];
  uint32_t* vd = b.val[s ^ 1u];
  const size_t t0 = (size_t)blockIdx.x * GS_RS_TILE, t1 = t0 + GS_RS_TILE < n ? t0 + GS_RS_TILE : n;
  const uint32_t lt = (1u << lane) - 1u;
  for (size_t r0 = t0; r0 < t1; r0 += GS_BLOCK) {
    const size_t x = r0 + tid;
    const bool valid = x < t1;
    uint64_t k = 0;
    uint32_t v = 0, dg = 256u;
    if (valid) {
      k = ks[x];
      v = vs[x];
      dg = gs_rs_digit(k, v, p, n_dcs);
    }
    const uint32_t peers = __match_any_sync(0xFFFFFFFFu, dg);
    const uint32_t rank = __popc(peers & lt);
    if (valid && rank == 0u) wcnt[w][dg] = __popc(peers);
    __syncthreads();
    {
      uint32_t acc = base[tid];
      for (uint32_t q = 0; q < GS_WARPS; ++q) {
        const uint32_t cq = wcnt[q][tid];
        woff[q][tid] = acc;
        acc += cq;
        wcnt[q][tid] = 0u;
      }
      base[tid] = acc;
    }
    __syncthreads();
    if (valid) {
      const uint32_t pos = woff[w][dg] + rank;
      kd[pos] = k;
      vd[pos] = v;
    }
  }
}

__global__ void __launch_bounds__(GS_BLOCK) gs_rs_copyback_kernel(GsRsBufs b, const GsRsCtl* c, uint32_t n) {
  if (c->fin == 0u) return;
  for (size_t x = (size_t)blockIdx.x * GS_BLOCK + threadIdx.x; x < n; x += (size_t)gridDim.x * GS_BLOCK) {
    b.key[0][x] = b.key[1][x];
    b.val[0][x] = b.val[1][x];
  }
}

class CudaBackend : public GsBackend {
 public:
  explicit CudaBackend(int dev) : dev_(dev) {
    err_[0] = 0;
    cudaStreamCreateWithFlags(&stream_, cudaStreamNonBlocking);
    cudaEventCreate(&ev0_);
    cudaEventCreate(&ev1_);
    int sms = 132, occ = 4;
    cudaDeviceGetAttribute(&sms, cudaDevAttrMultiProcessorCount, dev);
    sms_ = (uint32_t)sms;
    if (cudaOccupancyMaxActiveBlocksPerMultiprocessor(&occ, gs_tick_kernel<false>, GS_BLOCK, 0) != cudaSuccess || occ < 1)
      occ = 4;
    full_grid_ = (uint32_t)(sms * occ);
    int wocc = GS_WIN_BLOCKS;
    if (cudaOccupancyMaxActiveBlocksPerMultiprocessor(&wocc, gs_window_kernel<false, false>, GS_BLOCK, 0) != cudaSuccess || wocc < 1)
      wocc = GS_WIN_BLOCKS;
    win_grid_ = (uint32_t)(sms * wocc);
    if (const char* e = getenv("GSIM_GRID_MAX")) {
      const long cap = atol(e);
      if (cap > 0 && (unsigned long)cap < full_grid_) full_grid_ = (uint32_t)cap;
      if (cap > 0 && (unsigned long)cap < win_grid_) win_grid_ = (uint32_t)cap;
    }
    scratch_ = nullptr;
    cudaMalloc(&scratch_, 4096);
  }
  ~CudaBackend() override {
    cudaSetDevice(dev_);
    for (auto& kv : graphs_) cudaGraphExecDestroy(kv.second);
    for (auto& kv : wgraphs_) cudaGraphExecDestroy(kv.second);
    for (auto& kv : sgraphs_) cudaGraphExecDestroy(kv.second);
    if (sharded_) vmm_.destroy();
    if (scratch_) cudaFree(scratch_);
    if (rs_mem_) cudaFree(rs_mem_);
    cudaEventDestroy(ev0_);
    cudaEventDestroy(ev1_);
    cudaStreamDestroy(stream_);
  }
  const char* name() const override { return "cuda-sm_90a"; }
  void* alloc(size_t bytes) override {
    cudaSetDevice(dev_);
    void* p = nullptr;
    if (!ok(cudaMalloc(&p, bytes ? bytes : 4), "cudaMalloc")) return nullptr;
    return p;
  }
  void release(void* p) override {
    cudaSetDevice(dev_);
    if (p && !sharded_) cudaFree(p);
  }
  bool h2d(void* dst, const void* src, size_t bytes) override {
    cudaSetDevice(dev_);
    return ok(cudaMemcpyAsync(dst, src, bytes, cudaMemcpyHostToDevice, stream_), "h2d") &&
           ok(cudaStreamSynchronize(stream_), "h2d sync");
  }
  bool d2h(void* dst, const void* src, size_t bytes) override {
    cudaSetDevice(dev_);
    return ok(cudaMemcpyAsync(dst, src, bytes, cudaMemcpyDeviceToHost, stream_), "d2h") &&
           ok(cudaStreamSynchronize(stream_), "d2h sync");
  }
  void* host_alloc(size_t bytes) override {
    void* q = nullptr;
    cudaSetDevice(dev_);
    return cudaHostAlloc(&q, bytes, cudaHostAllocDefault) == cudaSuccess ? q : nullptr;
  }
  void host_free(void* q) override { cudaFreeHost(q); }
  bool h2d_word(void* dst, const void* src, size_t bytes) override {
    if (bytes > 16384) return h2d(dst, src, bytes);
    cudaSetDevice(dev_);
    return ok(cudaMemcpyAsync(dst, src, bytes, cudaMemcpyHostToDevice, stream_), "h2d");
  }
  bool write_batch(const GsWriteBatch& b) override {
    if (!b.n) return true;
    cudaSetDevice(dev_);
    gs_write_batch_kernel<<<1, 1, 0, stream_>>>(b);
    ++launches_;
    return ok(cudaGetLastError(), "write batch launch");
  }
  bool h2d_async(void* dst, const void* src, size_t bytes) override {
    cudaSetDevice(dev_);
    return ok(cudaMemcpyAsync(dst, src, bytes, cudaMemcpyHostToDevice, stream_), "h2d");
  }
  bool row_read(const GsDev& d, uint32_t i, uint32_t out[8]) override { return rows_read(d, &i, 1u, out); }
  bool rows_read(const GsDev& d, const uint32_t* ids, uint32_t n, uint32_t* out) override {
    cudaSetDevice(dev_);
    uint32_t* w = reinterpret_cast<uint32_t*>(scratch_) + 256;
    for (uint32_t x0 = 0; x0 < n; x0 += GS_ROWS_MAX) {
      GsRowIds r;
      r.n = n - x0 < GS_ROWS_MAX ? n - x0 : GS_ROWS_MAX;
      memcpy(r.id, ids + x0, r.n * 4);
      gs_rows_read_kernel<<<1, GS_ROWS_MAX * 8, 0, stream_>>>(d, r, w);
      ++launches_;
      if (!ok(cudaGetLastError(), "rows read launch") || !d2h(out + (size_t)x0 * 8, w, (size_t)r.n * 32)) return false;
    }
    return true;
  }
  bool fill32(uint32_t* dst, uint32_t value, size_t count) override {
    cudaSetDevice(dev_);
    if ((value & 0xFFu) == ((value >> 8) & 0xFFu) && (value & 0xFFFFu) == (value >> 16))
      return ok(cudaMemsetAsync(dst, (int)(value & 0xFFu), count * 4, stream_), "memset");
    return ok(cudaMemsetD32Async_(dst, value, count), "memset32");
  }
  bool fill8(uint8_t* dst, uint8_t value, size_t count) override {
    cudaSetDevice(dev_);
    return ok(cudaMemsetAsync(dst, value, count, stream_), "memset8");
  }
  bool init_rows(const GsDev& d, const GsGlobals* g_dev, const GsGlobals&, uint32_t first,
                 uint32_t count, uint32_t now) override {
    if (!count) return true;
    cudaSetDevice(dev_);
    gs_init_kernel<<<(count + GS_BLOCK - 1) / GS_BLOCK, GS_BLOCK, 0, stream_>>>(d, g_dev, first,
                                                                                count, now);
    ++launches_;
    return ok(cudaGetLastError(), "init launch");
  }
  bool run_ticks(const GsDev& d, const GsGlobals* g_dev, const GsGlobals& g, uint32_t t0,
                 uint32_t nticks, bool use_graph, double* kernel_ms, uint64_t* launches,
                 const GsXbar* xbar) override {
    uint32_t last_active = 0;
    return run_ticks_read(d, g_dev, g, t0, nticks, use_graph, kernel_ms, launches, xbar, &last_active);
  }
  bool run_ticks_read(const GsDev& d, const GsGlobals* g_dev, const GsGlobals& g, uint32_t t0, uint32_t nticks,
                      bool use_graph, double* kernel_ms, uint64_t* launches, const GsXbar* xbar,
                      uint32_t* last_active) override {
    (void)t0;
    if (!nticks || !g.n) {
      if (nticks) {
        gs_advance_kernel<<<1, 1, 0, stream_>>>(d.tick_base, nticks, nullptr);
        ++launches_;
        return ok(cudaGetLastError(), "advance") && d2h(last_active, d.qstate[g.rank] + GS_Q_LAST_ACTIVE, 4);
      }
      return d2h(last_active, d.qstate[g.rank] + GS_Q_LAST_ACTIVE, 4);
    }
    cudaSetDevice(dev_);
    l2_window(d, g);
    const uint32_t blocks = tick_blocks(g);
    if (!ok(cudaEventRecord(ev0_, stream_), "event")) return false;
    uint32_t left = nticks;
    if (use_graph && (!xbar || !no_shard_graph_) && left >= GS_GRAPH_TICKS) {
      cudaGraphExec_t ge = graph_for(d, g_dev, blocks, xbar);
      if (!ge) return false;
      while (left >= GS_GRAPH_TICKS) {
        if (!ok(cudaGraphLaunch(ge, stream_), "graph launch")) return false;
        left -= GS_GRAPH_TICKS;
        launches_ += GS_GRAPH_TICKS + 1;
      }
    }
    if (left) {
      for (uint32_t k = 0; k < left; ++k) {
        if (!ok(gs_launch_tick(blocks, stream_, d, g_dev, k, pdl_ && !xbar), "tick launch")) return false;
      }
      gs_advance_kernel<<<1, 1, 0, stream_>>>(d.tick_base, left, nullptr);
      launches_ += left + 1;
      if (!ok(cudaGetLastError(), "tick launch")) return false;
    }
    if (!ok(cudaEventRecord(ev1_, stream_), "event")) return false;
    uint32_t qs[GS_Q_WORDS] = {0, 0, 0, 0};
    if (!ok(cudaMemcpyAsync(qs, d.qstate[g.rank], sizeof(qs), cudaMemcpyDeviceToHost, stream_), "tick d2h"))
      return false;
    if (!ok(cudaStreamSynchronize(stream_), "tick sync")) return false;
    const uint32_t violation = qs[GS_Q_VIOLATION];
    *last_active = qs[GS_Q_LAST_ACTIVE];
    float ms = 0.f;
    cudaEventElapsedTime(&ms, ev0_, ev1_);
    if (kernel_ms) *kernel_ms += ms;
    if (launches) *launches += nticks;
    if (violation != 0u) {
      snprintf(err_, sizeof(err_), "tick %u: a bulk copy of the mailbox scan did not complete (kernel invariant broken)", violation - 1u);
      return false;
    }
    return true;
  }
  bool run_tick_stretch(const GsDev& d, const GsGlobals* g_dev, const GsGlobals& g, uint32_t t0, uint32_t nticks,
                        uint32_t floor, bool counts, double* kernel_ms, GsStretch* out) override {
    if (!g.n) return GsBackend::run_tick_stretch(d, g_dev, g, t0, nticks, floor, counts, kernel_ms, out);
    cudaSetDevice(dev_);
    l2_window(d, g);
    cudaGraphExec_t ge = stretch_graph_for(d, g_dev, g, tick_blocks(g), counts);
    if (!ge) return false;
    GsStretchCtl* c = stretch_ctl();
    if (!ok(cudaEventRecord(ev0_, stream_), "event")) return false;
    gs_stretch_begin_kernel<<<1, 1, 0, stream_>>>(c, t0 + nticks, floor, g.ring_mask + 1u);
    if (!ok(cudaGetLastError(), "stretch begin") || !ok(cudaGraphLaunch(ge, stream_), "stretch graph launch")) return false;
    uint8_t back[sizeof(GsStretch) + 4];
    if (!ok(cudaMemcpyAsync(back, c, sizeof(back), cudaMemcpyDeviceToHost, stream_), "stretch d2h") ||
        !ok(cudaStreamSynchronize(stream_), "stretch sync"))
      return false;
    memcpy(out, back, sizeof(GsStretch));
    uint32_t violation;
    memcpy(&violation, back + sizeof(GsStretch), 4);
    const uint32_t passes = out->launches / GS_STRETCH_TICKS;
    launches_ += 1u + out->launches + passes + 1u + (out->quiet ? (counts ? 3u : 2u) : 0u);
    float ms = 0.f;
    cudaEventElapsedTime(&ms, ev0_, ev1_);
    if (kernel_ms) *kernel_ms += ms;
    if (violation != 0u) {
      snprintf(err_, sizeof(err_), "tick %u: a bulk copy of the mailbox scan did not complete (kernel invariant broken)", violation - 1u);
      return false;
    }
    return true;
  }
  bool run_windows(const GsDev& d, const GsGlobals* g_dev, const GsGlobals& g, uint32_t t0, uint32_t nticks,
                   uint32_t per_launch, bool use_graph, double* kernel_ms, uint64_t* launches, uint32_t* ticks_done,
                   const GsXbar* xbar, bool pristine) override {
    cudaSetDevice(dev_);
    *ticks_done = 0;
    if (!nticks || !g.n) return true;
    uint32_t* qs = d.qstate[g.rank];
    uint32_t init[2] = {t0, 0u};
    if (!ok(cudaMemcpyAsync(qs + GS_Q_WIN_END, init, 8, cudaMemcpyHostToDevice, stream_), "window init")) return false;
    uint32_t tiles = (g.n + GS_TILE - 1) / GS_TILE;
    if (g.world > 1 && tiles > g.rows_per_rank / GS_TILE) tiles = g.rows_per_rank / GS_TILE;
    uint32_t blocks = (tiles * 4u + GS_WARPS - 1) / GS_WARPS;
    if (blocks > win_grid_) blocks = win_grid_;
    const uint32_t K = per_launch < g.P ? g.P : per_launch;
    const bool sharded = xbar != nullptr;
    const bool pdl = pdl_ && !sharded;
    if (!ok(cudaEventRecord(ev0_, stream_), "event")) return false;
    uint32_t left = nticks, n_launch = 0;
    if (use_graph && K == g.P && (!sharded || !no_shard_graph_)) {
      while (left >= GS_WIN_GRAPH * K) {
        cudaGraphExec_t ge = window_graph_for(d, g_dev, blocks, K, pdl, g.rank);
        if (!ge) return false;
        if (!ok(cudaGraphLaunch(ge, stream_), "window graph launch")) return false;
        left -= GS_WIN_GRAPH * K;
        n_launch += GS_WIN_GRAPH;
        launches_ += GS_WIN_GRAPH + 1;
      }
    }
    if (left) {
      uint32_t k = 0;
      while (left) {
        const uint32_t c = left < K ? left : K;
        if (!ok(gs_launch_window(blocks, stream_, d, g_dev, k, c, pdl, (pristine ? 1u : 0u) | win_mode_), "window launch"))
          return false;
        k += c;
        left -= c;
        ++n_launch;
        ++launches_;
      }
      gs_window_advance_kernel<<<1, 1, 0, stream_>>>(d.tick_base, qs);
      ++launches_;
      if (!ok(cudaGetLastError(), "window launch")) return false;
    }
    if (!ok(cudaEventRecord(ev1_, stream_), "event")) return false;
    uint32_t back[2] = {0, 0};
    if (!ok(cudaMemcpyAsync(back, qs + GS_Q_WIN_END, 8, cudaMemcpyDeviceToHost, stream_), "window d2h")) return false;
    if (!ok(cudaStreamSynchronize(stream_), "window sync")) return false;
    float ms = 0.f;
    cudaEventElapsedTime(&ms, ev0_, ev1_);
    if (kernel_ms) *kernel_ms += ms;
    if (launches) *launches += n_launch;
    if (back[1] != 0u) {
      snprintf(err_, sizeof(err_), "quiet window starting at tick %u met mail or posted some (scheduling invariant broken)", back[1] - 1u);
      return false;
    }
    if (back[0] < t0 || back[0] > t0 + nticks) {
      snprintf(err_, sizeof(err_), "window chain ended at tick %u outside [%u, %u]", back[0], t0, t0 + nticks);
      return false;
    }
    *ticks_done = back[0] - t0;
    return true;
  }
  bool quiet_scan(const GsDev& d, const GsGlobals* g_dev, const GsGlobals& g, uint32_t now, uint32_t first,
                  uint32_t count) override {
    cudaSetDevice(dev_);
    if (!count) return true;
    uint32_t blocks = (count + GS_BLOCK - 1) / GS_BLOCK;
    if (blocks > sms_ * 8u) blocks = sms_ * 8u;
    gs_quiet_scan_kernel<<<blocks, GS_BLOCK, 0, stream_>>>(d, g_dev, now, nullptr, first, count);
    ++launches_;
    (void)g;
    return ok(cudaGetLastError(), "quiet scan launch") && ok(cudaStreamSynchronize(stream_), "quiet scan");
  }
  bool quiet_probe(const GsDev& d, const GsGlobals* g_dev, const GsGlobals& g, uint32_t now, uint32_t* horizon,
                   GsRecount* counts) override {
    cudaSetDevice(dev_);
    GsRecount* dr = reinterpret_cast<GsRecount*>(scratch_);
    uint32_t* dh = reinterpret_cast<uint32_t*>(dr + 1);
    uint32_t* qh = d.qstate[0] + GS_Q_HORIZON;
    if (!ok(cudaMemsetAsync(qh, 0xFF, 4, stream_), "memset")) return false;
    if (g.n) {
      uint32_t blocks = (g.n + GS_BLOCK - 1) / GS_BLOCK;
      if (blocks > sms_ * 8u) blocks = sms_ * 8u;
      gs_quiet_scan_kernel<<<blocks, GS_BLOCK, 0, stream_>>>(d, g_dev, now, nullptr, 0u, g.n);
      ++launches_;
    }
    gs_copy_word_kernel<<<1, 1, 0, stream_>>>(dh, qh);
    ++launches_;
    if (counts) {
      if (!ok(cudaMemsetAsync(dr, 0, sizeof(GsRecount), stream_), "memset")) return false;
      if (g.n) {
        gs_recount_kernel<<<(g.n + GS_BLOCK - 1) / GS_BLOCK, GS_BLOCK, 0, stream_>>>(d, g_dev, now, nullptr, 0u, g.n, dr);
        ++launches_;
      }
    }
    if (!ok(cudaGetLastError(), "quiet probe launch")) return false;
    uint8_t back[sizeof(GsRecount) + 4];
    const size_t off = counts ? 0 : sizeof(GsRecount);
    if (!d2h(back + off, reinterpret_cast<uint8_t*>(scratch_) + off, sizeof(back) - off)) return false;
    if (counts) memcpy(counts, back, sizeof(GsRecount));
    memcpy(horizon, back + sizeof(GsRecount), 4);
    return true;
  }
  bool crash_fraction(const GsDev& d, const GsGlobals* g_dev, const GsGlobals& g, uint32_t thr,
                      uint32_t salt, uint32_t, uint32_t* n_crashed) override {
    cudaSetDevice(dev_);
    uint32_t* cnt = reinterpret_cast<uint32_t*>(scratch_);
    if (!ok(cudaMemsetAsync(cnt, 0, 4, stream_), "memset")) return false;
    if (g.n) {
      gs_crash_kernel<<<(g.n + GS_BLOCK - 1) / GS_BLOCK, GS_BLOCK, 0, stream_>>>(d, g_dev, thr,
                                                                                 salt, cnt);
      ++launches_;
    }
    return ok(cudaGetLastError(), "crash launch") && d2h(n_crashed, cnt, 4);
  }
  bool impair_dir_fraction(const GsDev& d, const GsGlobals* g_dev, const GsGlobals& g, const GsImpairCols& c,
                           uint32_t thr, uint32_t salt, const GsImpairVal& v, uint32_t counts[2]) override {
    cudaSetDevice(dev_);
    uint32_t* cnt = reinterpret_cast<uint32_t*>(scratch_);
    if (!ok(cudaMemsetAsync(cnt, 0, 8, stream_), "memset")) return false;
    if (g.n) {
      gs_impair_kernel<<<(g.n + GS_BLOCK - 1) / GS_BLOCK, GS_BLOCK, 0, stream_>>>(d, g_dev, c, thr, salt, v, cnt);
      ++launches_;
    }
    return ok(cudaGetLastError(), "impair launch") && d2h(counts, cnt, 8);
  }
  bool pause_rows(const GsDev& d, const GsGlobals* g_dev, const GsGlobals& g, uint32_t* pause_until,
                  const uint32_t* ids, uint32_t n, uint32_t thr, uint32_t salt, uint32_t until,
                  uint32_t* n_paused) override {
    cudaSetDevice(dev_);
    uint32_t* cnt = reinterpret_cast<uint32_t*>(scratch_);
    if (!ok(cudaMemsetAsync(cnt, 0, 4, stream_), "memset")) return false;
    const uint32_t rows = ids ? n : g.n;
    uint32_t* dids = nullptr;
    if (ids && n) {
      if (!ok(cudaMallocAsync(reinterpret_cast<void**>(&dids), (size_t)n * 4, stream_), "malloc")) return false;
      if (!ok(cudaMemcpyAsync(dids, ids, (size_t)n * 4, cudaMemcpyHostToDevice, stream_), "h2d")) {
        cudaFreeAsync(dids, stream_);
        return false;
      }
    }
    if (rows) {
      gs_pause_kernel<<<(rows + GS_BLOCK - 1) / GS_BLOCK, GS_BLOCK, 0, stream_>>>(d, g_dev, pause_until, dids, n, thr,
                                                                                 salt, until, cnt);
      ++launches_;
    }
    const bool launched = ok(cudaGetLastError(), "pause launch");
    if (dids) cudaFreeAsync(dids, stream_);
    return launched && d2h(n_paused, cnt, 4);
  }
  bool resume_rows(const GsDev& d, const GsGlobals* g_dev, const GsGlobals& g, uint32_t* pause_until, uint32_t t,
                   bool resume, bool log_events, uint32_t counts[4]) override {
    cudaSetDevice(dev_);
    uint32_t* cnt = reinterpret_cast<uint32_t*>(scratch_);
    if (!ok(cudaMemsetAsync(cnt, 0, 16, stream_), "memset")) return false;
    if (g.n) {
      gs_resume_kernel<<<(g.n + GS_BLOCK - 1) / GS_BLOCK, GS_BLOCK, 0, stream_>>>(
          d, g_dev, pause_until, t, resume ? 1u : 0u, log_events ? 1u : 0u, cnt);
      ++launches_;
    }
    return ok(cudaGetLastError(), "resume launch") && d2h(counts, cnt, 16);
  }
  bool coord_rows(const GsDev& d, const GsGlobals& g, uint32_t first, uint32_t count, double* rows) override {
    cudaSetDevice(dev_);
    if (!count) return true;
    gs_coord_rows_kernel<<<(count + GS_BLOCK - 1) / GS_BLOCK, GS_BLOCK, 0, stream_>>>(d, g.cap, first, count, rows);
    ++launches_;
    return ok(cudaGetLastError(), "coordinate rows launch");
  }
  bool coord_pairs(const GsDev& d, const GsGlobals* g_dev, const GsGlobals&, const uint32_t* a, const uint32_t* b,
                   uint32_t n, double* est, double* tru) override {
    cudaSetDevice(dev_);
    if (!n) return true;
    gs_coord_pairs_kernel<<<(n + GS_BLOCK - 1) / GS_BLOCK, GS_BLOCK, 0, stream_>>>(d, g_dev, a, b, n, est, tru);
    ++launches_;
    return ok(cudaGetLastError(), "coordinate pairs launch");
  }
  bool coord_dist_from(const GsDev& d, const GsGlobals* g_dev, const GsGlobals&, uint32_t now, uint32_t from,
                       const uint32_t* ids, uint32_t n, bool router, uint64_t* key, uint32_t* val) override {
    cudaSetDevice(dev_);
    if (!n) return true;
    gs_coord_dist_kernel<<<(n + GS_BLOCK - 1) / GS_BLOCK, GS_BLOCK, 0, stream_>>>(d, g_dev, now, from, ids, n,
                                                                                 router ? 1u : 0u, key, val);
    ++launches_;
    return ok(cudaGetLastError(), "coordinate distance launch");
  }
  bool sort_pairs(const GsGlobals& g, uint64_t* key, uint32_t* val, uint32_t n, uint32_t n_dcs) override {
    cudaSetDevice(dev_);
    if (n < 2u) return true;
    if (!rs_reserve(g.cap > n ? g.cap : n)) return false;
    const uint32_t np = n_dcs ? GS_RS_PASSES : 8u, nb = (n + GS_RS_TILE - 1u) / GS_RS_TILE;
    uint32_t hb = nb < sms_ * 4u ? nb : sms_ * 4u;
    if (!ok(cudaMemsetAsync(rs_ghist_, 0, GS_RS_PASSES * 256 * 4, stream_), "memset")) return false;
    gs_rs_hist_kernel<<<hb, GS_BLOCK, 0, stream_>>>(key, val, n, n_dcs, np, rs_ghist_);
    gs_rs_plan_kernel<<<1, 1, 0, stream_>>>(rs_ghist_, n, np, rs_ctl_);
    GsRsBufs b;
    b.key[0] = key;
    b.key[1] = rs_key_;
    b.val[0] = val;
    b.val[1] = rs_val_;
    for (uint32_t p = 0; p < np; ++p) {
      gs_rs_upsweep_kernel<<<nb, GS_BLOCK, 0, stream_>>>(b, rs_ctl_, p, n, n_dcs, rs_hist_);
      gs_rs_scan_kernel<<<256, GS_BLOCK, 0, stream_>>>(rs_ctl_, p, nb, rs_hist_);
      gs_rs_scatter_kernel<<<nb, GS_BLOCK, 0, stream_>>>(b, rs_ctl_, p, n, n_dcs, rs_hist_, rs_ghist_);
    }
    hb = (n + GS_BLOCK - 1) / GS_BLOCK < sms_ * 8u ? (n + GS_BLOCK - 1) / GS_BLOCK : sms_ * 8u;
    gs_rs_copyback_kernel<<<hb, GS_BLOCK, 0, stream_>>>(b, rs_ctl_, n);
    launches_ += 3u + 3u * np;
    return ok(cudaGetLastError(), "radix sort launch");
  }
  bool dc_medians(const GsGlobals&, const uint64_t* key, const uint32_t* val, uint32_t n, uint32_t n_dcs, double* med,
                  uint32_t* cnt) override {
    cudaSetDevice(dev_);
    gs_dc_medians_kernel<<<1, GS_MAX_DCS, 0, stream_>>>(key, val, n, n_dcs, med, cnt);
    ++launches_;
    return ok(cudaGetLastError(), "medians launch");
  }
  bool coord_error(const GsDev& d, const GsGlobals* g_dev, const GsGlobals& g, uint32_t now, uint32_t n_draws,
                   uint32_t salt, uint64_t* key, uint32_t* val, double* part, double* out) override {
    cudaSetDevice(dev_);
    const uint32_t nch = (n_draws + GS_ERR_CHUNK - 1u) / GS_ERR_CHUNK;
    gs_coord_error_kernel<<<nch, GS_BLOCK, 0, stream_>>>(d, g_dev, now, n_draws, salt, key, val, part);
    ++launches_;
    if (!ok(cudaGetLastError(), "error sample launch") || !sort_pairs(g, key, val, n_draws, 0u)) return false;
    gs_coord_error_finish_kernel<<<1, 1, 0, stream_>>>(key, n_draws, part, out);
    ++launches_;
    return ok(cudaGetLastError(), "error finish launch");
  }
  bool reap_rows(const GsDev& d, const GsGlobals* g_dev, const GsGlobals& g, uint32_t now,
                 uint32_t reconnect_ticks, uint32_t tombstone_ticks, bool log_events,
                 uint32_t counts[2]) override {
    cudaSetDevice(dev_);
    uint32_t* cnt = reinterpret_cast<uint32_t*>(scratch_);
    if (!ok(cudaMemsetAsync(cnt, 0, 8, stream_), "memset")) return false;
    if (g.n) {
      gs_reap_kernel<<<(g.n + GS_BLOCK - 1) / GS_BLOCK, GS_BLOCK, 0, stream_>>>(
          d, g_dev, now, reconnect_ticks, tombstone_ticks, log_events ? 1u : 0u, cnt);
      ++launches_;
    }
    return ok(cudaGetLastError(), "reap launch") && d2h(counts, cnt, 8);
  }
  bool recount(const GsDev& d, const GsGlobals* g_dev, const GsGlobals& g, uint32_t now, uint32_t first, uint32_t count,
               GsRecount* out) override {
    cudaSetDevice(dev_);
    GsRecount* dr = reinterpret_cast<GsRecount*>(scratch_);
    if (!ok(cudaMemsetAsync(dr, 0, sizeof(GsRecount), stream_), "memset")) return false;
    if (first < g.n && count) {
      if (count > g.n - first) count = g.n - first;
      gs_recount_kernel<<<(count + GS_BLOCK - 1) / GS_BLOCK, GS_BLOCK, 0, stream_>>>(d, g_dev, now, nullptr, first, count, dr);
      ++launches_;
    }
    return ok(cudaGetLastError(), "recount launch") && d2h(out, dr, sizeof(GsRecount));
  }
  bool state_hash(const GsDev& d, const GsGlobals* g_dev, const GsGlobals& g, uint32_t now,
                  uint64_t out[4]) override {
    cudaSetDevice(dev_);
    unsigned long long* dh = reinterpret_cast<unsigned long long*>(scratch_);
    if (!ok(cudaMemsetAsync(dh, 0, 32, stream_), "memset")) return false;
    if (g.n) {
      gs_hash_kernel<<<(g.n + GS_BLOCK - 1) / GS_BLOCK, GS_BLOCK, 0, stream_>>>(d, g_dev, now, dh);
      ++launches_;
    }
    return ok(cudaGetLastError(), "hash launch") && d2h(out, dh, 32);
  }
  bool shard_begin(uint32_t world, uint32_t rank) override {
    cudaSetDevice(dev_);
    cudaFree(0);
    sharded_ = vmm_.init(dev_, world, rank, err_, sizeof(err_));
    return sharded_;
  }
  size_t shard_granularity() override { return vmm_.granularity(); }
  void* shard_alloc(size_t slice_bytes, size_t planes) override {
    void* q = vmm_.reserve(slice_bytes, planes);
    if (!q) snprintf(err_, sizeof(err_), "%s", vmm_.last_error());
    return q;
  }
  bool shard_commit(const int** fds, size_t* n) override {
    if (!vmm_.commit()) {
      snprintf(err_, sizeof(err_), "%s", vmm_.last_error());
      return false;
    }
    *fds = vmm_.export_fds().data();
    *n = vmm_.export_fds().size();
    return true;
  }
  bool shard_attach(uint32_t peer, const int* fds, size_t n) override {
    cudaSetDevice(dev_);
    if (!vmm_.attach(peer, fds, n)) {
      snprintf(err_, sizeof(err_), "%s", vmm_.last_error());
      return false;
    }
    return true;
  }
  bool xbar_host(const GsXbar& xb) override {
    cudaSetDevice(dev_);
    gs_xbar_kernel<<<1, 32, 0, stream_>>>(xb);
    ++launches_;
    return ok(cudaGetLastError(), "xbar launch") && ok(cudaStreamSynchronize(stream_), "xbar");
  }
  bool and_columns(const GsDev& d, const GsGlobals& g, uint32_t keep, uint32_t first, uint32_t count) override {
    cudaSetDevice(dev_);
    if (first >= g.n || !count) return true;
    if (count > g.n - first) count = g.n - first;
    gs_and_kernel<<<(count + GS_BLOCK - 1) / GS_BLOCK, GS_BLOCK, 0, stream_>>>(d, first, count, keep);
    ++launches_;
    return ok(cudaGetLastError(), "and launch");
  }
  bool sync() override {
    cudaSetDevice(dev_);
    return ok(cudaStreamSynchronize(stream_), "sync");
  }
  const char* last_error() const override { return err_; }
  uint64_t total_launches() const override { return launches_; }

 private:
  void l2_window(const GsDev& d, const GsGlobals& g) {
    if (d.kst != nullptr && !l2_window_set_ && getenv("GSIM_NO_L2_WINDOW") == nullptr) {
      l2_window_set_ = true;
      cudaDeviceProp prop;
      if (cudaGetDeviceProperties(&prop, dev_) == cudaSuccess && prop.persistingL2CacheMaxSize > 0) {
        size_t bytes = g.cap;
        if (bytes > (size_t)prop.accessPolicyMaxWindowSize) bytes = (size_t)prop.accessPolicyMaxWindowSize;
        size_t carve = bytes < (size_t)prop.persistingL2CacheMaxSize ? bytes : (size_t)prop.persistingL2CacheMaxSize;
        cudaDeviceSetLimit(cudaLimitPersistingL2CacheSize, carve);
        cudaStreamAttrValue v;
        memset(&v, 0, sizeof(v));
        v.accessPolicyWindow.base_ptr = d.kst;
        v.accessPolicyWindow.num_bytes = bytes;
        v.accessPolicyWindow.hitRatio = bytes <= carve ? 1.0f : (float)carve / (float)bytes;
        v.accessPolicyWindow.hitProp = cudaAccessPropertyPersisting;
        v.accessPolicyWindow.missProp = cudaAccessPropertyStreaming;
        cudaStreamSetAttribute(stream_, cudaStreamAttributeAccessPolicyWindow, &v);
        cudaGetLastError();
      }
    }
  }
  uint32_t tick_blocks(const GsGlobals& g) const {
    uint32_t tiles = (g.n + GS_TILE - 1) / GS_TILE;
    if (g.world > 1 && tiles > g.rows_per_rank / GS_TILE) tiles = g.rows_per_rank / GS_TILE;
    uint32_t blocks = (tiles + GS_WARPS - 1) / GS_WARPS;
    return blocks < full_grid_ ? blocks : full_grid_;
  }
  cudaError_t cudaMemsetD32Async_(uint32_t* dst, uint32_t value, size_t count) {
    if (!count) return cudaSuccess;
    size_t blocks = (count + GS_BLOCK - 1) / GS_BLOCK;
    if (blocks > sms_ * 16u) blocks = sms_ * 16u;
    gs_fill32_kernel<<<(unsigned)blocks, GS_BLOCK, 0, stream_>>>(dst, value, count);
    ++launches_;
    return cudaGetLastError();
  }
  void drop_stale_graphs(const GsDev& d) {
    if (have_graph_dev_ && memcmp(&graph_dev_, &d, sizeof(GsDev)) != 0) {
      for (auto& kv : graphs_) cudaGraphExecDestroy(kv.second);
      graphs_.clear();
      for (auto& kv : wgraphs_) cudaGraphExecDestroy(kv.second);
      wgraphs_.clear();
      for (auto& kv : sgraphs_) cudaGraphExecDestroy(kv.second);
      sgraphs_.clear();
    }
    graph_dev_ = d;
    have_graph_dev_ = true;
  }
  cudaGraphExec_t graph_for(const GsDev& d, const GsGlobals* g_dev, uint32_t blocks, const GsXbar* xbar) {
    drop_stale_graphs(d);
    auto it = graphs_.find(blocks);
    if (it != graphs_.end()) return it->second;
    cudaGraph_t graph = nullptr;
    cudaGraphExec_t ge = nullptr;
    if (!ok(cudaStreamBeginCapture(stream_, cudaStreamCaptureModeThreadLocal), "capture"))
      return nullptr;
    for (uint32_t k = 0; k < GS_GRAPH_TICKS; ++k)
      if (!ok(gs_launch_tick(blocks, stream_, d, g_dev, k, pdl_ && !xbar), "tick capture")) {
        cudaGraph_t dead = nullptr;
        cudaStreamEndCapture(stream_, &dead);
        if (dead) cudaGraphDestroy(dead);
        return nullptr;
      }

    gs_advance_kernel<<<1, 1, 0, stream_>>>(d.tick_base, GS_GRAPH_TICKS, nullptr);
    if (!ok(cudaStreamEndCapture(stream_, &graph), "end capture")) return nullptr;
    if (!ok(cudaGraphInstantiate(&ge, graph, 0), "instantiate")) {
      cudaGraphDestroy(graph);
      return nullptr;
    }
    cudaGraphDestroy(graph);
    graphs_[blocks] = ge;
    return ge;
  }
  GsStretchCtl* stretch_ctl() { return reinterpret_cast<GsStretchCtl*>(reinterpret_cast<uint8_t*>(scratch_) + 3072); }
  cudaGraphExec_t stretch_graph_for(const GsDev& d, const GsGlobals* g_dev, const GsGlobals& g, uint32_t blocks, bool counts) {
    drop_stale_graphs(d);
    const uint64_t key = ((uint64_t)blocks << 1) | (counts ? 1u : 0u);
    auto it = sgraphs_.find(key);
    if (it != sgraphs_.end()) return it->second;
    GsStretchCtl* c = stretch_ctl();
    uint32_t* qs = d.qstate[0];
    cudaGraph_t graph = nullptr;
    cudaGraphExec_t ge = nullptr;
    if (!ok(cudaGraphCreate(&graph, 0), "stretch graph")) return nullptr;
    cudaGraphConditionalHandle loop = 0, probe = 0;
    cudaGraphNode_t wn = nullptr, rn = nullptr, en = nullptr, pn = nullptr;
    cudaGraphNodeParams wp = {};
    wp.type = cudaGraphNodeTypeConditional;
    cudaGraphNodeParams pp = wp;
    bool good = ok(cudaGraphConditionalHandleCreate(&loop, graph, 1u, cudaGraphCondAssignDefault), "loop handle") &&
                ok(cudaGraphConditionalHandleCreate(&probe, graph, 0u, cudaGraphCondAssignDefault), "probe handle");
    if (good) {
      wp.conditional.handle = loop;
      wp.conditional.type = cudaGraphCondTypeWhile;
      wp.conditional.size = 1;
      good = ok(cudaGraphAddNode(&wn, graph, nullptr, 0, &wp), "while node");
    }
    if (good && ok(cudaStreamBeginCaptureToGraph(stream_, wp.conditional.phGraph_out[0], nullptr, nullptr, 0,
                                                 cudaStreamCaptureModeThreadLocal), "capture")) {
      for (uint32_t k = 0; k < GS_STRETCH_TICKS && good; ++k)
        good = ok(gs_launch_tick(blocks, stream_, d, g_dev, k, pdl_, c), "tick capture");
      if (good) {
        gs_stretch_pass_kernel<<<1, 1, 0, stream_>>>(d.tick_base, qs, c, GS_STRETCH_TICKS, loop);
        good = ok(cudaGetLastError(), "pass capture");
      }
      cudaGraph_t body = nullptr;
      good = ok(cudaStreamEndCapture(stream_, &body), "end capture") && good;
    } else {
      good = false;
    }
    if (good) good = ok(cudaGraphAddEventRecordNode(&rn, graph, &wn, 1, ev1_), "event node");
    if (good) {
      void* args[] = {&c, &qs, &probe};
      cudaKernelNodeParams kp = {};
      kp.func = reinterpret_cast<void*>(gs_stretch_end_kernel);
      kp.gridDim = dim3(1);
      kp.blockDim = dim3(1);
      kp.kernelParams = args;
      good = ok(cudaGraphAddKernelNode(&en, graph, &rn, 1, &kp), "end node");
    }
    if (good) {
      pp.conditional.handle = probe;
      pp.conditional.type = cudaGraphCondTypeIf;
      pp.conditional.size = 1;
      good = ok(cudaGraphAddNode(&pn, graph, &en, 1, &pp), "if node");
    }
    if (good && ok(cudaStreamBeginCaptureToGraph(stream_, pp.conditional.phGraph_out[0], nullptr, nullptr, 0,
                                                 cudaStreamCaptureModeThreadLocal), "capture")) {
      uint32_t sblocks = (g.cap + GS_BLOCK - 1) / GS_BLOCK;
      if (sblocks > sms_ * 8u) sblocks = sms_ * 8u;
      gs_quiet_scan_kernel<<<sblocks, GS_BLOCK, 0, stream_>>>(d, g_dev, 0u, d.tick_base, 0u, g.cap);
      gs_copy_word_kernel<<<1, 1, 0, stream_>>>(&c->out.horizon, qs + GS_Q_HORIZON);
      if (counts)
        gs_recount_kernel<<<(g.cap + GS_BLOCK - 1) / GS_BLOCK, GS_BLOCK, 0, stream_>>>(d, g_dev, 0u, d.tick_base, 0u, g.cap,
                                                                                      &c->out.counts);
      good = ok(cudaGetLastError(), "probe capture");
      cudaGraph_t body = nullptr;
      good = ok(cudaStreamEndCapture(stream_, &body), "end capture") && good;
    } else {
      good = false;
    }
    if (good) good = ok(cudaGraphInstantiate(&ge, graph, 0), "instantiate");
    cudaGraphDestroy(graph);
    if (!good) return nullptr;
    sgraphs_[key] = ge;
    return ge;
  }
  cudaGraphExec_t window_graph_for(const GsDev& d, const GsGlobals* g_dev, uint32_t blocks, uint32_t K, bool pdl, uint32_t rank) {
    drop_stale_graphs(d);
    const uint64_t key = ((uint64_t)blocks << 32) | K;
    auto it = wgraphs_.find(key);
    if (it != wgraphs_.end()) return it->second;
    cudaGraph_t graph = nullptr;
    cudaGraphExec_t ge = nullptr;
    if (!ok(cudaStreamBeginCapture(stream_, cudaStreamCaptureModeThreadLocal), "capture")) return nullptr;
    bool good = true;
    for (uint32_t j = 0; j < GS_WIN_GRAPH && good; ++j)
      good = ok(gs_launch_window(blocks, stream_, d, g_dev, j * K, K, pdl, win_mode_), "window capture");
    if (good) gs_window_advance_kernel<<<1, 1, 0, stream_>>>(d.tick_base, d.qstate[rank]);
    if (!ok(cudaStreamEndCapture(stream_, &graph), "end capture") || !good) {
      if (graph) cudaGraphDestroy(graph);
      return nullptr;
    }
    if (!ok(cudaGraphInstantiate(&ge, graph, 0), "instantiate")) {
      cudaGraphDestroy(graph);
      return nullptr;
    }
    cudaGraphDestroy(graph);
    wgraphs_[key] = ge;
    return ge;
  }
  bool rs_reserve(size_t n) {
    if (n <= rs_n_) return true;
    if (rs_mem_) cudaFree(rs_mem_);
    rs_mem_ = nullptr;
    rs_n_ = 0;
    const size_t nb = (n + GS_RS_TILE - 1) / GS_RS_TILE;
    const size_t kb = n * 8, vb = (n * 4 + 255) / 256 * 256, hb = (256 * nb * 4 + 255) / 256 * 256;
    const size_t gb = GS_RS_PASSES * 256 * 4;
    if (!ok(cudaMalloc(&rs_mem_, kb + vb + hb + gb + sizeof(GsRsCtl)), "radix sort scratch")) {
      rs_mem_ = nullptr;
      return false;
    }
    uint8_t* q = reinterpret_cast<uint8_t*>(rs_mem_);
    rs_key_ = reinterpret_cast<uint64_t*>(q);
    rs_val_ = reinterpret_cast<uint32_t*>(q + kb);
    rs_hist_ = reinterpret_cast<uint32_t*>(q + kb + vb);
    rs_ghist_ = reinterpret_cast<uint32_t*>(q + kb + vb + hb);
    rs_ctl_ = reinterpret_cast<GsRsCtl*>(q + kb + vb + hb + gb);
    rs_n_ = n;
    return true;
  }
  bool ok(cudaError_t e, const char* what) {
    if (e == cudaSuccess) return true;
    snprintf(err_, sizeof(err_), "%s: %s", what, cudaGetErrorString(e));
    return false;
  }
  int dev_;
  cudaStream_t stream_;
  cudaEvent_t ev0_, ev1_;
  void* scratch_;
  void* rs_mem_ = nullptr;
  size_t rs_n_ = 0;
  uint64_t* rs_key_ = nullptr;
  uint32_t* rs_val_ = nullptr;
  uint32_t* rs_hist_ = nullptr;
  uint32_t* rs_ghist_ = nullptr;
  GsRsCtl* rs_ctl_ = nullptr;
  uint32_t sms_ = 132;
  uint32_t full_grid_ = 528;
  uint32_t win_grid_ = 528;
  GsVmm vmm_;
  bool sharded_ = false;
  bool pdl_ = getenv("GSIM_NO_PDL") == nullptr;
  bool no_shard_graph_ = getenv("GSIM_SHARD_GRAPH") == nullptr;
  uint32_t win_mode_ = getenv("GSIM_WIN_CYCLIC") && atoi(getenv("GSIM_WIN_CYCLIC")) ? 2u : 0u;
  std::map<uint32_t, cudaGraphExec_t> graphs_;
  std::map<uint64_t, cudaGraphExec_t> wgraphs_;
  std::map<uint64_t, cudaGraphExec_t> sgraphs_;
  GsDev graph_dev_;
  bool have_graph_dev_ = false;
  bool l2_window_set_ = false;
  uint64_t launches_ = 0;
  char err_[256];
};

}

GsBackend* gs_make_cuda_backend(int device, char* err, size_t err_cap) {
  int count = 0;
  cudaError_t e = cudaGetDeviceCount(&count);
  if (e != cudaSuccess || count == 0) {
    snprintf(err, err_cap, "no CUDA device: %s (libgsim has no CPU fallback)",
             e == cudaSuccess ? "device count is 0" : cudaGetErrorString(e));
    return nullptr;
  }
  if (device < 0) {
    if (cudaGetDevice(&device) != cudaSuccess) device = 0;
  }
  if (device >= count) {
    snprintf(err, err_cap, "CUDA device %d out of range (%d devices)", device, count);
    return nullptr;
  }
  cudaDeviceProp prop;
  if (cudaGetDeviceProperties(&prop, device) != cudaSuccess || prop.major != 9 || prop.minor != 0) {
    snprintf(err, err_cap, "device %d is not sm_90 (libgsim ships sm_90a SASS only)", device);
    return nullptr;
  }
  if (cudaSetDevice(device) != cudaSuccess) {
    snprintf(err, err_cap, "cudaSetDevice(%d) failed", device);
    return nullptr;
  }
  return new CudaBackend(device);
}
```

consul_b200/csrc/gs_row.h:

```cpp
#pragma once
#include <string.h>

#include "gs_core.h"
#include "gs_coord.h"

#if defined(__CUDA_ARCH__)
#define GS_DEV __device__ __forceinline__
__device__ __forceinline__ uint32_t gs_atomic_or_sys(uint32_t* p, uint32_t v) {
  uint32_t old;
  asm volatile("atom.global.sys.or.b32 %0, [%1], %2;" : "=r"(old) : "l"(p), "r"(v) : "memory");
  return old;
}
__device__ __forceinline__ uint64_t gs_atomic_min_sys(uint64_t* p, uint64_t v) {
  unsigned long long old;
  asm volatile("atom.global.sys.min.u64 %0, [%1], %2;" : "=l"(old) : "l"(p), "l"((unsigned long long)v) : "memory");
  return old;
}
__device__ __forceinline__ void gs_red_or_sys(uint32_t* p, uint32_t v) {
  asm volatile("red.global.sys.or.b32 [%0], %1;" ::"l"(p), "r"(v) : "memory");
}
__device__ __forceinline__ void gs_red_or_gpu(uint32_t* p, uint32_t v) {
  asm volatile("red.global.gpu.or.b32 [%0], %1;" ::"l"(p), "r"(v) : "memory");
}
#define GS_ATOMIC_OR32(p, v) (g.world > 1u ? gs_atomic_or_sys((p), (v)) : atomicOr((p), (v)))
#define GS_POST_OR32(p, v)                                                         \
  do {                                                                             \
    if (g.world <= 1u) gs_red_or_gpu((p), (v));                                    \
    else if (g.flags & 128u) (void)gs_atomic_or_sys((p), (v));                     \
    else gs_red_or_sys((p), (v));                                                  \
  } while (0)
#define GS_ATOMIC_MIN64(p, v)                                                    \
  (g.world > 1u ? gs_atomic_min_sys((uint64_t*)(p), (uint64_t)(v))               \
                : (uint64_t)atomicMin((unsigned long long*)(p), (unsigned long long)(v)))
__device__ __forceinline__ uint32_t gs_ld_sys(const uint32_t* p) {
  uint32_t v;
  asm volatile("ld.relaxed.sys.global.u32 %0, [%1];" : "=r"(v) : "l"(p) : "memory");
  return v;
}
__device__ __forceinline__ uint64_t gs_ld_sys64(const uint64_t* p) {
  unsigned long long v;
  asm volatile("ld.relaxed.sys.global.u64 %0, [%1];" : "=l"(v) : "l"(p) : "memory");
  return v;
}
#define GS_LD_OTHER(p) __ldcg(p)
#define GS_LD_OTHER64(p) gs_ld_sys64(p)
__device__ __forceinline__ uint32_t gs_atomic_min32_sys(uint32_t* p, uint32_t v) {
  uint32_t old;
  asm volatile("atom.global.sys.min.u32 %0, [%1], %2;" : "=r"(old) : "l"(p), "r"(v) : "memory");
  return old;
}
__device__ __forceinline__ uint32_t gs_atomic_max32_sys(uint32_t* p, uint32_t v) {
  uint32_t old;
  asm volatile("atom.global.sys.max.u32 %0, [%1], %2;" : "=r"(old) : "l"(p), "r"(v) : "memory");
  return old;
}
#define GS_ATOMIC_MIN32(p, v) (g.world > 1u ? gs_atomic_min32_sys((p), (v)) : atomicMin((p), (v)))
#define GS_ATOMIC_MAX32(p, v) (g.world > 1u ? gs_atomic_max32_sys((p), (v)) : atomicMax((p), (v)))
#else
#define GS_DEV inline
#define GS_ATOMIC_OR32(p, v) __atomic_fetch_or((p), (v), __ATOMIC_RELAXED)
#define GS_POST_OR32(p, v) (void)__atomic_fetch_or((p), (v), __ATOMIC_RELAXED)
static inline uint64_t gs_host_atomic_min64(uint64_t* p, uint64_t v) {
  uint64_t old = __atomic_load_n(p, __ATOMIC_RELAXED);
  while (old > v && !__atomic_compare_exchange_n(p, &old, v, true, __ATOMIC_RELAXED,
                                                 __ATOMIC_RELAXED)) {
  }
  return old;
}
#define GS_ATOMIC_MIN64(p, v) gs_host_atomic_min64((uint64_t*)(p), (uint64_t)(v))
static inline uint32_t gs_host_atomic_min32(uint32_t* p, uint32_t v) {
  uint32_t old = __atomic_load_n(p, __ATOMIC_RELAXED);
  while (old > v && !__atomic_compare_exchange_n(p, &old, v, true, __ATOMIC_RELAXED, __ATOMIC_RELAXED)) {
  }
  return old;
}
static inline uint32_t gs_host_atomic_max32(uint32_t* p, uint32_t v) {
  uint32_t old = __atomic_load_n(p, __ATOMIC_RELAXED);
  while (old < v && !__atomic_compare_exchange_n(p, &old, v, true, __ATOMIC_RELAXED, __ATOMIC_RELAXED)) {
  }
  return old;
}
#define GS_ATOMIC_MIN32(p, v) gs_host_atomic_min32((p), (v))
#define GS_ATOMIC_MAX32(p, v) gs_host_atomic_max32((p), (v))
#define GS_LD_OTHER(p) (*(p))
#define GS_LD_OTHER64(p) (*(p))
#endif

enum {
  GS_ST_PROBES = 0,
  GS_ST_ACKS,
  GS_ST_INDIRECT_PINGS,
  GS_ST_NACKS,
  GS_ST_PROBE_FAILURES,
  GS_ST_SUSPECTS,
  GS_ST_CONFIRMATIONS,
  GS_ST_DEADS,
  GS_ST_REFUTES,
  GS_ST_GOSSIP_PACKETS,
  GS_ST_RUMORS_SENT,
  GS_ST_RUMORS_ACCEPTED,
  GS_ST_RUMORS_DROPPED,
  GS_ST_PACKETS_LOST,
  GS_ST_ACTIVE_ROWS,
  GS_ST_PUSH_PULLS
};

GS_DEV void gs_key_store(const GsDev& d, const GsGlobals& g, uint32_t buf, uint32_t i, uint32_t k) {
  if (d.kst != nullptr) {
    const uint32_t b = d.kst[i], code = gs_kst_code(k);
    d.kst[i] = (uint8_t)(buf ? ((b & 0x0Fu) | (code << 4)) : ((b & 0xF0u) | code));
  }
  if (g.world <= 1u) {
    d.key[buf][i] = k;
    return;
  }
  for (uint32_t r = 0; r < g.world; ++r) d.key_rep[buf][(size_t)r * g.key_stride + i] = k;
}

GS_DEV uint32_t gs_peer_key(const GsDev& d, uint32_t cur, uint32_t c, bool need_inc) {
  if (d.kst != nullptr && !need_inc) {
#if defined(__CUDA_ARCH__)
    const uint32_t b = __ldcg(reinterpret_cast<const unsigned char*>(d.kst) + c);
#else
    const uint32_t b = d.kst[c];
#endif
    const uint32_t code = (b >> (cur * 4u)) & 15u;
    if (code != GS_KST_PENDING) return code;
  }
  return GS_LD_OTHER(&d.key[cur][c]);
}

template <class Sink>
GS_DEV void gs_post(const GsDev& d, const GsGlobals& g, Sink& sink, uint32_t slot, uint32_t j, uint32_t bits) {
  sink.activity();
  GS_POST_OR32(&d.inbox[slot][j], bits);
}

#define GS_PEER_INC(d, cur, c, k) gs_key_inc(gs_peer_key((d), (cur), (c), true))

struct GsHot {
  uint32_t n, P, T, seed_lo, seed_hi, perm_bits, loss_thr, graph_n, pp_interval, rot_pp, phase_group, n_dcs;
  const uint8_t* lat;
};
GS_DEV GsHot gs_hot(const GsGlobals& g) {
  GsHot h;
  h.n = g.n; h.P = g.P; h.T = g.T; h.seed_lo = g.seed_lo; h.seed_hi = g.seed_hi;
  h.perm_bits = g.perm_bits; h.loss_thr = g.loss_thr; h.graph_n = g.graph_n;
  h.pp_interval = g.pp_interval; h.rot_pp = g.rot_pp; h.phase_group = g.phase_group; h.n_dcs = g.n_dcs;
  h.lat = g.lat;
  return h;
}

template <class G>
GS_DEV uint32_t gs_extra(const G& g, const uint8_t* delay, uint32_t src, uint32_t dst) {
  uint32_t e = g.n_dcs == 0u ? 0u : g.lat[((src / GS_TILE) % g.n_dcs) * GS_MAX_DCS + (dst / GS_TILE) % g.n_dcs];
  if (delay != nullptr) e += delay[dst];
  return e;
}

struct GsLossCols {
  const uint32_t* send;
  const uint32_t* recv;
};

GS_DEV bool gs_loss_rule(const GsGlobals& g, const GsLossCols& loss, const GsU4& r, uint32_t src, uint32_t dst) {
  return r.x < g.loss_thr || (loss.send != nullptr && (r.y < loss.send[src] || r.z < loss.recv[dst]));
}

GS_DEV bool gs_lost_quiet(const GsGlobals& g, const GsLossCols& loss, uint32_t src, uint32_t dst, uint32_t t,
                          uint32_t kind, uint32_t idx) {
  if (g.loss_thr == 0u && loss.send == nullptr) return false;
  GsU4 r = gs_philox(g.seed_lo, g.seed_hi, src, dst, t, GS_PUR_LOSS | (kind << 8) | (idx << 16));
  return gs_loss_rule(g, loss, r, src, dst);
}

template <class Sink>
GS_DEV bool gs_lost(const GsGlobals& g, const GsLossCols& loss, Sink& sink, uint32_t src, uint32_t dst, uint32_t t,
                    uint32_t kind, uint32_t idx) {
  if (g.loss_thr == 0u && loss.send == nullptr) return false;
  GsU4 r = gs_philox(g.seed_lo, g.seed_hi, src, dst, t, GS_PUR_LOSS | (kind << 8) | (idx << 16));
  bool lost = gs_loss_rule(g, loss, r, src, dst);
  if (lost) sink.stat(GS_ST_PACKETS_LOST, 1);
  return lost;
}

GS_DEV bool gs_no_tcp(const uint8_t* flags, uint32_t i, uint32_t j) {
  return flags != nullptr && ((flags[i] | flags[j]) & GS_IMPAIR_NO_TCP) != 0u;
}

GS_DEV bool gs_knows(const GsDev& d, const GsGlobals& g, uint32_t i, uint32_t c, uint32_t kc,
                     uint32_t meta_i) {
  if (c == i) return true;
  if (!gs_key_pending(kc)) return !(meta_i & GS_META_ISOLATED);
  const uint32_t heard_i = d.heard[i];
  uint32_t am = g.class_mask[0] & g.active_mask;
  while (am) {
#if defined(__CUDA_ARCH__)
    uint32_t r = __ffs(am) - 1;
#else
    uint32_t r = (uint32_t)__builtin_ctz(am);
#endif
    am &= am - 1;
    if (g.rumors[r].kind == GS_RUMOR_ALIVE && g.rumors[r].subject == c) return (heard_i >> r) & 1u;
  }
  return false;
}

GS_DEV uint32_t gs_peer_count(const GsDev& d, const GsGlobals& g, uint32_t i) {
  if (g.graph_n == 0u) return g.n;
  return i < g.graph_n ? d.row_ptr[i + 1u] - d.row_ptr[i] : 0u;
}
GS_DEV uint32_t gs_peer_at(const GsDev& d, const GsGlobals& g, uint32_t i, uint32_t idx) {
  return g.graph_n == 0u ? idx : d.col_idx[d.row_ptr[i] + idx];
}

GS_DEV uint32_t gs_coord_slot_for_reader(const uint32_t* ctag, size_t cap, uint32_t j, uint32_t t) {
  const uint32_t a = GS_LD_OTHER(&ctag[j]), b = GS_LD_OTHER(&ctag[cap + j]);
  return (b <= t && (a > t || b > a)) ? 1u : 0u;
}
GS_DEV void gs_coord_load(const double* coord, size_t cap, uint32_t slot, uint32_t j, GsCoord& c) {
  const double* base = coord + ((size_t)slot * GS_COORD_WORDS) * cap + j;
  double w[GS_COORD_WORDS];
  for (uint32_t x = 0; x < GS_COORD_WORDS; ++x) {
    const uint64_t bits = GS_LD_OTHER64(reinterpret_cast<const uint64_t*>(base + (size_t)x * cap));
    memcpy(&w[x], &bits, 8);
  }
  for (uint32_t x = 0; x < GS_COORD_DIM; ++x) c.vec[x] = w[x];
  c.error = w[8];
  c.adjustment = w[9];
  c.height = w[10];
}
#if defined(__CUDA_ARCH__)
__device__ __noinline__
#else
inline
#endif
void gs_coord_on_ack(double* coord, uint32_t* ctag, double* adj, uint32_t* adj_idx, const uint8_t* imp_delay,
                     const GsGlobals& g, uint32_t i,
                     uint32_t j, uint32_t t) {
  const size_t cap = g.cap;
  const uint32_t ta = ctag[i], tb = ctag[cap + i];
  const uint32_t mine = tb > ta ? 1u : 0u, spare = mine ^ 1u;
  GsCoord c, other;
  gs_coord_load(coord, cap, mine, i, c);
  gs_coord_load(coord, cap, gs_coord_slot_for_reader(ctag, cap, j, t), j, other);
  const double rtt =
      g.coord_base_rtt_s + (double)(gs_extra(g, imp_delay, i, j) + gs_extra(g, imp_delay, j, i)) * g.tick_seconds;
  uint32_t idx = adj_idx[i];
  gs_coord_client_update(c, other, rtt, adj + i, cap, &idx, g.seed_lo, g.seed_hi, i, t);
  adj_idx[i] = idx;
  double* out = coord + ((size_t)spare * GS_COORD_WORDS) * cap + i;
  for (uint32_t x = 0; x < GS_COORD_DIM; ++x) out[(size_t)x * cap] = c.vec[x];
  out[(size_t)8 * cap] = c.error;
  out[(size_t)9 * cap] = c.adjustment;
  out[(size_t)10 * cap] = c.height;
  ctag[(size_t)spare * cap + i] = t + 1u;
}

GS_DEV uint32_t gs_krandom(const GsDev& d, const GsGlobals& g, uint32_t i, uint32_t t,
                           uint32_t purpose, uint32_t k, uint32_t mode, uint32_t exclude2,
                           uint32_t meta_i, uint32_t* out) {
  const uint32_t n = gs_peer_count(d, g, i);
  if (n == 0u) return 0u;
  uint32_t tries = 3u * n;
  if (tries > GS_KR_MAX_TRIES || n > 0x55555555u) tries = GS_KR_MAX_TRIES;
  uint32_t cnt = 0;
  for (uint32_t b4 = 0; b4 * 4u < tries && cnt < k; ++b4) {
    const GsU4 blk = gs_philox(g.seed_lo, g.seed_hi, i, t, purpose, b4);
    uint32_t cc[4], kk[4];
#pragma unroll
    for (uint32_t x = 0; x < 4u; ++x) {
      const uint32_t draw = gs_u4_get(blk, x);
      cc[x] = gs_peer_at(d, g, i, g.graph_n == 0u ? gs_fastmod(draw, n, g.n_magic) : draw % n);
      kk[x] = (b4 * 4u + x < tries && cc[x] != i && cc[x] != exclude2) ? gs_peer_key(d, t & 1u, cc[x], false) : 0u;
    }
#pragma unroll
    for (uint32_t x = 0; x < 4u; ++x) {
      if (!(b4 * 4u + x < tries && cnt < k)) continue;
      const uint32_t c = cc[x], kc = kk[x];
      if (c == i || c == exclude2) continue;
      if (gs_key_truth(kc) == GS_TRUTH_NONE) continue;
      const uint32_t rank = gs_key_rank(kc);
      if (mode == 1u) {
        if (rank != GS_RANK_ALIVE) continue;
      } else {
        if (rank == GS_RANK_LEFT) continue;
        if (rank == GS_RANK_DEAD && (t - GS_LD_OTHER(&d.change_tick[c])) > g.gtd_ticks) continue;
      }
      if (!gs_knows(d, g, i, c, kc, meta_i)) continue;
      bool dup = false;
      for (uint32_t q = 0; q < cnt; ++q) dup = dup || (out[q] == c);
      if (dup) continue;
      out[cnt++] = c;
    }
  }
  return cnt;
}

GS_DEV uint32_t gs_select_packet_in(const GsDev& d, const GsGlobals& g, uint32_t i, uint32_t queued, uint32_t avail) {
  if (g.active_bytes <= avail) return queued;
  uint32_t total = 0, qm = queued;
  while (qm) {
#if defined(__CUDA_ARCH__)
    uint32_t r = __ffs(qm) - 1;
#else
    uint32_t r = (uint32_t)__builtin_ctz(qm);
#endif
    qm &= qm - 1;
    total += g.rumors[r].size + (g.rumors[r].qclass ? 3u : 2u);
  }
  if (total <= avail) return queued;
  uint32_t used = 0, mask = 0;
  for (uint32_t cls = 0; cls < 3; ++cls) {
    uint32_t cm = queued & g.class_mask[cls];
    const uint32_t ovh = cls ? 3u : 2u;
    while (cm) {
      if (avail <= used + ovh) break;
      const uint32_t free_b = avail - used - ovh;
      uint32_t best = GS_EMPTY32, best_key = GS_EMPTY32, scan = cm;
      while (scan) {
#if defined(__CUDA_ARCH__)
        uint32_t r = __ffs(scan) - 1;
#else
        uint32_t r = (uint32_t)__builtin_ctz(scan);
#endif
        scan &= scan - 1;
        uint32_t sz = g.rumors[r].size;
        if (sz > free_b) continue;
        uint32_t tx = d.tx[GS_TX(r, g.cap, i)];
        uint32_t key = (tx << 24) | ((0xFFFFu - (sz & 0xFFFFu)) << 8) | (31u - r);
        if (key < best_key) {
          best_key = key;
          best = r;
        }
      }
      if (best == GS_EMPTY32) break;
      mask |= 1u << best;
      cm &= ~(1u << best);
      used += ovh + g.rumors[best].size;
    }
  }
  return mask;
}

GS_DEV uint32_t gs_select_packet(const GsDev& d, const GsGlobals& g, uint32_t i, uint32_t queued) {
  return gs_select_packet_in(d, g, i, queued, g.udp_avail);
}

GS_DEV void gs_pig_count(const GsDev& d, uint32_t i, uint32_t which, uint32_t v) {
#if defined(__CUDA_ARCH__)
  atomicAdd(&d.pig->stats[which][i & 31u], (unsigned long long)v);
#else
  __atomic_fetch_add(&d.pig->stats[which][i & 31u], (unsigned long long)v, __ATOMIC_RELAXED);
#endif
}

GS_DEV bool gs_pig_gate(const GsDev& d, uint32_t t) { return d.pig->gate[t % GS_PIG_GATES] == t + 1u; }

GS_DEV void gs_pig_stamp(const GsDev& d, uint32_t t, uint32_t delta) {
  for (uint32_t s = t + 1u; s != t + 1u + delta; ++s)
    if (d.pig->gate[s % GS_PIG_GATES] != s + 1u) d.pig->gate[s % GS_PIG_GATES] = s + 1u;
}

GS_DEV uint32_t gs_pig_wake_delta(const GsGlobals& g, uint32_t gslot, uint32_t gphase) {
  const uint32_t next = gslot + 1u == g.GI ? 0u : gslot + 1u;
  const uint32_t delta = (gphase >= next ? gphase - next : gphase + g.GI - next) + 1u;
  return delta > g.ring_mask + 1u ? 1u : delta;
}

GS_DEV uint32_t gs_pig_take(const GsDev& d, const GsGlobals& g, uint32_t i, uint32_t& queued, uint32_t kind) {
  if (queued == 0u) return 0u;
  const uint32_t pkt = gs_select_packet_in(d, g, i, queued, d.pig->budget[kind]);
  if (pkt == 0u) return 0u;
  const uint32_t q0 = queued;
  uint32_t pm = pkt, c = 0;
  while (pm) {
#if defined(__CUDA_ARCH__)
    const uint32_t r = __ffs(pm) - 1;
#else
    const uint32_t r = (uint32_t)__builtin_ctz(pm);
#endif
    pm &= pm - 1;
    const uint32_t tx = (uint32_t)d.tx[GS_TX(r, g.cap, i)] + 1u;
    d.tx[GS_TX(r, g.cap, i)] = (uint8_t)tx;
    if (tx >= g.retransmit_limit) queued &= ~(1u << r);
    ++c;
  }
  if (queued != q0) d.queued[i] = queued;
  gs_pig_count(d, i, GS_PIG_ST_PACKETS, 1u);
  gs_pig_count(d, i, GS_PIG_ST_BCASTS, c);
  return pkt;
}

template <class Sink>
GS_DEV void gs_pig_owe(const GsDev& d, const GsGlobals& g, Sink& sink, uint32_t nxt, uint32_t inxt, uint32_t sender,
                       uint32_t receiver, uint32_t kind, bool lost) {
  uint32_t* req = d.pig_req + (size_t)nxt * GS_PIGK * g.cap;
  uint32_t v = (receiver << 3) | (kind << 1) | (lost ? 1u : 0u);
  bool kept = false;
  for (uint32_t s = 0; s < GS_PIGK; ++s) {
    const uint32_t old = GS_ATOMIC_MIN32(&req[(size_t)s * g.cap + sender], v);
    if (old == GS_EMPTY32) {
      kept = true;
      break;
    }
    if (old > v) v = old;
  }
  if (!kept) gs_pig_count(d, sender, GS_PIG_ST_DROPPED, 1u);
  gs_post(d, g, sink, inxt, sender, GS_ACC_BIT);
}

template <class Sink>
GS_DEV void gs_log_event(const GsDev& d, const GsGlobals& g, Sink& sink, uint32_t t, uint32_t type,
                         uint32_t subject, uint32_t observer, uint32_t ltime) {
  sink.log_event(d, g, t, type, subject, observer, ltime);
}

GS_DEV bool gs_tile_probe_gate(const GsGlobals& g, uint32_t tile, uint32_t pslot, uint32_t pslot_t) {
  if (!g.phase_gate) return true;
  const uint32_t group = tile >> g.phase_shift;
  const uint32_t pp = gs_probe_phase(g.rot_p, group, g.P);
  return pp == pslot || pp == pslot_t;
}

GS_DEV uint32_t gs_queue_wake_slot(const GsGlobals& g, uint32_t t, uint32_t gslot, uint32_t gphase) {
  const uint32_t next = gslot + 1u == g.GI ? 0u : gslot + 1u;
  const uint32_t delta = (gphase >= next ? gphase - next : gphase + g.GI - next) + 1u;
  return (delta > g.ring_mask + 1u ? t + 1u : t + delta) & g.ring_mask;
}

GS_DEV bool gs_mail_is_stale(const GsGlobals& g, uint32_t w, uint32_t heard, bool due_now, bool pp_now) {
  return (w & (GS_WAKE_BIT | GS_ACC_BIT)) == 0u && !due_now && !pp_now && (w & g.active_mask & ~heard) == 0u;
}

template <bool IMPAIRED, bool PIG = false, class Sink>
GS_DEV void gs_row_step_body(const GsDev& d, const GsGlobals& g, uint32_t i, uint32_t t, uint32_t gslot,
                             uint32_t inb, Sink& sink) {
  const GsLossCols imp_loss = {IMPAIRED ? d.imp_loss : nullptr, IMPAIRED ? d.imp_recv : nullptr};
  const uint8_t* const imp_delay = IMPAIRED ? d.imp_delay : nullptr;
  const uint8_t* const imp_flags = IMPAIRED ? d.imp_flags : nullptr;
  const uint32_t cur = t & 1u, nxt = cur ^ 1u;
  const uint32_t icur = t & g.ring_mask, inxt = (t + 1u) & g.ring_mask;
  const uint32_t rbits = inb & ~(GS_ACC_BIT | GS_WAKE_BIT) & g.active_mask;
  const uint32_t k0 = d.key[cur][i], m0 = d.meta[i], due0 = d.due[i], queued0 = d.queued[i];
  const uint32_t heard0 = rbits != 0u ? d.heard[i] : 0u;
  const uint32_t truth = gs_key_truth(k0);
  if (inb != 0u) sink.activity();
  if (truth == GS_TRUTH_NONE) {
    if (inb != 0u) d.inbox[icur][i] = 0u;
    return;
  }
  const bool up = truth == GS_TRUTH_UP;
  const bool gossip_slot = up && gslot == gs_meta_gphase(m0);
  uint32_t queued = up ? queued0 : 0u;
  if (inb != 0u) d.inbox[icur][i] = 0u;
  const bool pp_now = up && g.pp_interval != 0u && gs_pp_due(g.pp_interval, g.rot_pp, i / g.phase_group, t);
  if (inb != 0u && gs_mail_is_stale(g, inb, heard0, due0 == t, pp_now)) return;
  sink.stat(GS_ST_ACTIVE_ROWS, 1);

  if ((inb & ~GS_WAKE_BIT) == 0u && gs_key_rank(k0) == GS_RANK_ALIVE && !(up && due0 == t) &&
      !(gossip_slot && queued != 0u) && !pp_now) {
    if (m0 & GS_META_DIRTY) {
      gs_key_store(d, g, nxt, i, k0);
      d.meta[i] = m0 & ~GS_META_DIRTY;
    }
    if (queued != 0u) gs_post(d, g, sink, gs_queue_wake_slot(g, t, gslot, gs_meta_gphase(m0)), i, GS_WAKE_BIT);
    if constexpr (PIG) {
      if (queued != 0u) gs_pig_stamp(d, t, gs_pig_wake_delta(g, gslot, gs_meta_gphase(m0)));
    }
    return;
  }

  uint32_t k = k0, m = m0, due = due0;
  const size_t cap = g.cap;
  uint32_t heard = 0;

  if ((inb & ~GS_WAKE_BIT) != 0u) {
    if ((inb & GS_ACC_BIT) && g.pp_interval != 0u) {
      uint32_t* clk = d.pp_clk + (size_t)cur * 2u * cap;
      const uint32_t cm = GS_LD_OTHER(&clk[i]), ce = GS_LD_OTHER(&clk[cap + i]);
      if (cm | ce) {
        clk[i] = 0u;
        clk[cap + i] = 0u;
        if (up) {
          if (cm > d.ltime_member[i]) d.ltime_member[i] = cm;
          if (ce > d.ltime_event[i]) d.ltime_event[i] = ce;
        }
      }
    }
    if (rbits && up) {
      heard = heard0;
      uint32_t fresh = rbits & ~heard;
      uint32_t accepted = 0;
      while (fresh) {
#if defined(__CUDA_ARCH__)
        uint32_t r = __ffs(fresh) - 1;
#else
        uint32_t r = (uint32_t)__builtin_ctz(fresh);
#endif
        fresh &= fresh - 1;
        const GsRumor& ru = g.rumors[r];
        bool accept = true;
        if (ru.kind == GS_RUMOR_USER_EVENT) {
          uint32_t c = d.ltime_event[i];
          if (ru.ltime >= c) {
            c = ru.ltime + 1u;
            d.ltime_event[i] = c;
          }
          if (ru.ltime < d.event_min[i]) accept = false;
          else if (c > g.event_buffer && ru.ltime < c - g.event_buffer) accept = false;
          if (accept && (m & GS_META_WATCHED))
            gs_log_event(d, g, sink, t, GS_EV_USER, r, i, ru.ltime);
        } else if (ru.kind == GS_RUMOR_JOIN_INTENT || ru.kind == GS_RUMOR_LEAVE_INTENT) {
          uint32_t c = d.ltime_member[i];
          if (ru.ltime >= c) d.ltime_member[i] = ru.ltime + 1u;
        } else if (ru.kind == GS_RUMOR_ALIVE) {
          if (m & GS_META_WATCHED) gs_log_event(d, g, sink, t, GS_EV_MEMBER_JOIN, ru.subject, i, 0u);
        } else if (ru.kind == GS_RUMOR_UPDATE) {
          if (m & GS_META_WATCHED) gs_log_event(d, g, sink, t, GS_EV_MEMBER_UPDATE, ru.subject, i, 0u);
        }
        if (accept) {
          accepted |= 1u << r;
          d.tx[GS_TX(r, cap, i)] = 0;
          sink.heard(r);
          sink.stat(GS_ST_RUMORS_ACCEPTED, 1);
        } else {
          sink.stat(GS_ST_RUMORS_DROPPED, 1);
        }
      }
      if (accepted) {
        d.heard[i] = heard | accepted;
        queued |= accepted;
        d.queued[i] = queued;
      }
    }
    if (inb & GS_ACC_BIT) {
      uint64_t* acc = d.acc + (size_t)cur * GS_K1MAX * cap;
      for (uint32_t s = 0; s < GS_K1MAX; ++s) {
        uint64_t e = GS_LD_OTHER64(&acc[(size_t)s * cap + i]);
        if (e == GS_EMPTY64) break;
        acc[(size_t)s * cap + i] = GS_EMPTY64;
        uint32_t e_inc = ~(uint32_t)(e >> 32), from = (uint32_t)e;
        if (e_inc != gs_key_inc(k)) continue;
        uint32_t rank = gs_key_rank(k);
        if (rank == GS_RANK_ALIVE) {
          k = gs_key_with_rank(k, GS_RANK_SUSPECT);
          d.sus_start[i] = t - 1u;
          d.sus_from[i] = from;
          for (uint32_t q = 1; q < GS_K1MAX; ++q) d.sus_from[(size_t)q * cap + i] = GS_EMPTY32;
          sink.stat(GS_ST_SUSPECTS, 1);
        } else if (rank == GS_RANK_SUSPECT) {
          for (uint32_t q = 0; q <= g.sus_k && q < GS_K1MAX; ++q) {
            uint32_t f = d.sus_from[(size_t)q * cap + i];
            if (f == from) break;
            if (f == GS_EMPTY32) {
              d.sus_from[(size_t)q * cap + i] = from;
              sink.stat(GS_ST_CONFIRMATIONS, 1);
              break;
            }
          }
        }
      }
    }
    if ((inb & GS_ACC_BIT) && g.pp_interval != 0u) {
      uint32_t* req = d.ppreq + (size_t)cur * GS_PPK * cap;
      for (uint32_t s = 0; s < GS_PPK; ++s) {
        const uint32_t from = GS_LD_OTHER(&req[(size_t)s * cap + i]);
        if (from == GS_EMPTY32) break;
        req[(size_t)s * cap + i] = GS_EMPTY32;
        if (!up) continue;
        uint32_t* clk = d.pp_clk + (size_t)nxt * 2u * cap;
        GS_ATOMIC_MAX32(&clk[from], d.ltime_member[i]);
        GS_ATOMIC_MAX32(&clk[cap + from], d.ltime_event[i]);
        gs_post(d, g, sink, inxt, from, (d.heard[i] & g.active_mask) | GS_ACC_BIT);
      }
    }
    if constexpr (PIG) {
      if (inb & GS_ACC_BIT) {
        uint32_t* req = d.pig_req + (size_t)cur * GS_PIGK * cap;
        for (uint32_t s = 0; s < GS_PIGK; ++s) {
          const uint32_t e = GS_LD_OTHER(&req[(size_t)s * cap + i]);
          if (e == GS_EMPTY32) break;
          req[(size_t)s * cap + i] = GS_EMPTY32;
          if (!up) continue;
          gs_pig_count(d, i, GS_PIG_ST_SERVED, 1u);
          const uint32_t pkt = gs_pig_take(d, g, i, queued, (e >> 1) & 3u);
          if (pkt != 0u && !(e & 1u))
            gs_post(d, g, sink, (t + 1u + gs_extra(g, imp_delay, i, e >> 3)) & g.ring_mask, e >> 3, pkt);
        }
      }
    }
  }

  {
    uint32_t rank = gs_key_rank(k);
    if (up && !(m & GS_META_LEAVING) && (rank == GS_RANK_SUSPECT || rank == GS_RANK_DEAD)) {
      uint32_t inc = gs_key_inc(k);
      uint32_t accused = inc;
      inc = inc + 1u;
      if (accused >= inc) inc = accused + 1u;
      k = gs_key_with_rank(gs_key_with_inc(k, inc), GS_RANK_ALIVE);
      uint32_t aw = gs_meta_aw(m) + 1u;
      if (aw > g.awareness_max - 1u) aw = g.awareness_max - 1u;
      m = gs_meta_set_aw(m, aw);
      sink.stat(GS_ST_REFUTES, 1);
    } else if (rank == GS_RANK_SUSPECT) {
      uint32_t c = 0;
      for (uint32_t q = 1; q <= g.sus_k && q < GS_K1MAX; ++q)
        c += d.sus_from[(size_t)q * cap + i] != GS_EMPTY32;
      if (t - d.sus_start[i] >= g.sus_ticks[c]) {
        k = gs_key_with_rank(k, GS_RANK_DEAD);
        d.change_tick[i] = t;
        sink.stat(GS_ST_DEADS, 1);
        if (truth == GS_TRUTH_CRASHED) sink.crashed_dead(d, t);
        if (g.flags & 1u) gs_log_event(d, g, sink, t, GS_EV_MEMBER_FAILED, i, GS_EMPTY32, 0u);
      }
    }
  }

  if (up) {
    uint32_t stage = gs_meta_stage(m);
    if (stage == GS_STAGE_WAIT_T && due == t) {
      const uint32_t j = d.probe_tgt[i];
      const uint32_t kj = gs_peer_key(d, cur, j, false);
      const bool j_up = gs_key_truth(kj) == GS_TRUTH_UP;
      uint32_t relays[8];
      uint32_t kk = g.indirect_checks > 8u ? 8u : g.indirect_checks;
      uint32_t nr = gs_krandom(d, g, i, t, GS_PUR_RELAY, kk, 1u, j, m, relays);
      bool success = false;
      uint32_t nacks = 0;
      const uint32_t budget = g.P * (gs_meta_aw(m) + 1u) - g.T;
      bool pig_gate = false;
      if constexpr (PIG) pig_gate = gs_pig_gate(d, t);
      for (uint32_t q = 0; q < nr; ++q) {
        const uint32_t r = relays[q];
        const bool r_up = gs_key_truth(gs_peer_key(d, cur, r, false)) == GS_TRUTH_UP;
        sink.stat(GS_ST_INDIRECT_PINGS, 1);
        if constexpr (PIG) {
          const bool req_lost = gs_lost_quiet(g, imp_loss, i, r, t, GS_LK_INDREQ, q);
          const uint32_t pkt = gs_pig_take(d, g, i, queued, GS_PIG_INDREQ);
          if (pkt != 0u && !req_lost) gs_post(d, g, sink, (t + 1u + gs_extra(g, imp_delay, i, r)) & g.ring_mask, r, pkt);
          if (pig_gate && r_up && !req_lost) {
            const bool ping_lost = gs_lost_quiet(g, imp_loss, r, j, t, GS_LK_INDPING, q);
            gs_pig_owe(d, g, sink, nxt, inxt, r, j, GS_PIG_PING, ping_lost);
            const bool ack_lost = gs_lost_quiet(g, imp_loss, j, r, t, GS_LK_INDACK, q);
            if (j_up && !ping_lost) gs_pig_owe(d, g, sink, nxt, inxt, j, r, GS_PIG_ACK, ack_lost);
            const bool acked = j_up && !ping_lost && !ack_lost &&
                               gs_extra(g, imp_delay, r, j) + gs_extra(g, imp_delay, j, r) <= g.T;
            if (acked)
              gs_pig_owe(d, g, sink, nxt, inxt, r, i, GS_PIG_ACK, gs_lost_quiet(g, imp_loss, r, i, t, GS_LK_INDFWD, q));
            else
              gs_pig_owe(d, g, sink, nxt, inxt, r, i, GS_PIG_NACK, gs_lost_quiet(g, imp_loss, r, i, t, GS_LK_NACK, q));
          }
        }
        if (!(r_up && !gs_lost(g, imp_loss, sink, i, r, t, GS_LK_INDREQ, q))) continue;
        const uint32_t via = gs_extra(g, imp_delay, i, r) + gs_extra(g, imp_delay, r, i);
        const uint32_t rtt_rj = gs_extra(g, imp_delay, r, j) + gs_extra(g, imp_delay, j, r);
        bool relay_acked = j_up && !gs_lost(g, imp_loss, sink, r, j, t, GS_LK_INDPING, q) &&
                           !gs_lost(g, imp_loss, sink, j, r, t, GS_LK_INDACK, q) && rtt_rj <= g.T;
        if (relay_acked) {
          if (!gs_lost(g, imp_loss, sink, r, i, t, GS_LK_INDFWD, q) && via + rtt_rj <= budget) success = true;
        } else if (!gs_lost(g, imp_loss, sink, r, i, t, GS_LK_NACK, q) && via <= budget) {
          ++nacks;
          sink.stat(GS_ST_NACKS, 1);
        }
      }
      const uint32_t t0 = t - g.T;
      const uint32_t rtt_ij = gs_extra(g, imp_delay, i, j) + gs_extra(g, imp_delay, j, i);
      if (!g.disable_tcp && j_up && rtt_ij <= budget && !gs_no_tcp(imp_flags, i, j)) success = true;
      if ((g.n_dcs != 0u || imp_delay != nullptr) && j_up && rtt_ij > g.T && rtt_ij <= budget + g.T &&
          !gs_lost_quiet(g, imp_loss, i, j, t0, GS_LK_PING, 0) && !gs_lost_quiet(g, imp_loss, j, i, t0, GS_LK_ACK, 0))
        success = true;
      if (success) {
        uint32_t aw = gs_meta_aw(m);
        m = gs_meta_set_aw(m, aw ? aw - 1u : 0u);
        m = gs_meta_set_stage(m, GS_STAGE_IDLE);
        due = t0 + g.P;
        sink.stat(GS_ST_ACKS, 1);
      } else {
        uint32_t miss = nr > 0u ? nr - nacks : 1u;
        if (miss > 7u) miss = 7u;
        m = gs_meta_set_nmiss(gs_meta_set_stage(m, GS_STAGE_WAIT_P), miss);
        due = t0 + g.P * (gs_meta_aw(m) + 1u);
      }
      stage = gs_meta_stage(m);
    }
    if (stage == GS_STAGE_WAIT_P && due == t) {
      uint32_t aw = gs_meta_aw(m) + gs_meta_nmiss(m);
      if (aw > g.awareness_max - 1u) aw = g.awareness_max - 1u;
      m = gs_meta_set_stage(gs_meta_set_aw(m, aw), GS_STAGE_IDLE);
      const uint32_t j = d.probe_tgt[i];
      const uint64_t e = ((uint64_t)(~d.probe_inc[i]) << 32) | (uint64_t)i;
      uint64_t* acc = d.acc + (size_t)nxt * GS_K1MAX * cap;
      uint64_t v = e;
      for (uint32_t s = 0; s < GS_K1MAX; ++s) {
        uint64_t old = GS_ATOMIC_MIN64(&acc[(size_t)s * cap + j], v);
        if (old == v || old == GS_EMPTY64) break;
        if (old > v) v = old;
      }
      gs_post(d, g, sink, inxt, j, GS_ACC_BIT);
      sink.stat(GS_ST_PROBE_FAILURES, 1);
      stage = GS_STAGE_IDLE;
    }
    if (stage == GS_STAGE_IDLE && due == t) {
      uint32_t cursor = d.cursor[i], pass = d.pass[i];
      const uint32_t n = gs_peer_count(d, g, i);
      const uint32_t hb = g.graph_n == 0u ? g.perm_bits : gs_perm_bits_of(n);
      GsU4 rk = gs_perm_keys(g.seed_lo, g.seed_hi, i, pass);
      uint32_t checked = 0, target = GS_EMPTY32, ktarget = 0;
      const uint32_t limit = n < GS_PROBE_SKIP_CAP ? n : GS_PROBE_SKIP_CAP;
      while (checked < limit) {
        if (cursor >= n) {
          cursor = 0;
          ++pass;
          ++checked;
          rk = gs_perm_keys(g.seed_lo, g.seed_hi, i, pass);
          continue;
        }
        uint32_t c = gs_peer_at(d, g, i, gs_perm(cursor, n, hb, rk));
        ++cursor;
        uint32_t kc = gs_peer_key(d, cur, c, false);
        uint32_t rank = gs_key_rank(kc);
        if (c == i || gs_key_truth(kc) == GS_TRUTH_NONE || rank == GS_RANK_DEAD ||
            rank == GS_RANK_LEFT || !gs_knows(d, g, i, c, kc, m)) {
          ++checked;
          continue;
        }
        target = c;
        ktarget = kc;
        break;
      }
      d.cursor[i] = cursor;
      d.pass[i] = pass;
      if (target != GS_EMPTY32) {
        sink.stat(GS_ST_PROBES, 1);
        if constexpr (PIG) {
          const bool ping_lost = gs_lost_quiet(g, imp_loss, i, target, t, GS_LK_PING, 0);
          const uint32_t pkt = gs_pig_take(d, g, i, queued, GS_PIG_PING);
          if (pkt != 0u && !ping_lost)
            gs_post(d, g, sink, (t + 1u + gs_extra(g, imp_delay, i, target)) & g.ring_mask, target, pkt);
          if (gs_pig_gate(d, t) && gs_key_truth(ktarget) == GS_TRUTH_UP && !ping_lost)
            gs_pig_owe(d, g, sink, nxt, inxt, target, i, GS_PIG_ACK, gs_lost_quiet(g, imp_loss, target, i, t, GS_LK_ACK, 0));
        }
        bool ok = gs_key_truth(ktarget) == GS_TRUTH_UP && !gs_lost(g, imp_loss, sink, i, target, t, GS_LK_PING, 0) &&
                  !gs_lost(g, imp_loss, sink, target, i, t, GS_LK_ACK, 0) &&
                  gs_extra(g, imp_delay, i, target) + gs_extra(g, imp_delay, target, i) <= g.T;
        if (ok) {
          uint32_t aw = gs_meta_aw(m);
          m = gs_meta_set_aw(m, aw ? aw - 1u : 0u);
          due = t + g.P;
          sink.stat(GS_ST_ACKS, 1);
          if constexpr (Sink::kCoords) {
            if (d.coord != nullptr) gs_coord_on_ack(d.coord, d.ctag, d.adj, d.adj_idx, imp_delay, g, i, target, t);
          }
        } else {
          m = gs_meta_set_stage(m, GS_STAGE_WAIT_T);
          d.probe_tgt[i] = target;
          d.probe_inc[i] = GS_PEER_INC(d, cur, target, ktarget);
          due = t + g.T;
          sink.horizon(t + g.P);
        }
      } else {
        due = t + g.P;
      }
    }

    if (gossip_slot && queued != 0u) {
      uint32_t peers[8];
      uint32_t kk = g.gossip_nodes > 8u ? 8u : g.gossip_nodes;
      const bool whole = g.active_bytes <= g.udp_avail;
      uint64_t tx8 = 0;
      if (whole) {
        uint32_t pm = queued;
        for (uint32_t x = 0; x < 8u && pm != 0u; ++x) {
#if defined(__CUDA_ARCH__)
          const uint32_t r = __ffs(pm) - 1;
#else
          const uint32_t r = (uint32_t)__builtin_ctz(pm);
#endif
          pm &= pm - 1;
          tx8 |= (uint64_t)d.tx[GS_TX(r, cap, i)] << (8u * x);
        }
      }
      uint32_t np = gs_krandom(d, g, i, t, GS_PUR_GOSSIP, kk, 0u, GS_EMPTY32, m, peers);
      const uint32_t q0 = queued;
      if (whole && np != 0u) {
        uint32_t sends = 0, n_pkts = 0, n_q = 0, pm = queued;
        bool few = true;
        while (pm) {
          pm &= pm - 1;
          if (n_q == 8u) { few = false; break; }
          const uint32_t tx = (uint32_t)(tx8 >> (8u * n_q)) & 0xFFu;
          uint32_t room = g.retransmit_limit > tx ? g.retransmit_limit - tx : 1u;
          if (room == 0u) room = 1u;
          const uint32_t s = room < np ? room : np;
          sends |= s << (4u * n_q++);
          if (s > n_pkts) n_pkts = s;
        }
        if (few) {
          pm = queued;
          for (uint32_t x = 0; x < n_q; ++x) {
#if defined(__CUDA_ARCH__)
            const uint32_t r = __ffs(pm) - 1;
#else
            const uint32_t r = (uint32_t)__builtin_ctz(pm);
#endif
            pm &= pm - 1;
            const uint32_t s = (sends >> (4u * x)) & 15u;
            const uint32_t tx = ((uint32_t)(tx8 >> (8u * x)) & 0xFFu) + s;
            d.tx[GS_TX(r, cap, i)] = (uint8_t)tx;
            if (tx >= g.retransmit_limit) queued &= ~(1u << r);
            sink.stat(GS_ST_RUMORS_SENT, s);
          }
          sink.stat(GS_ST_GOSSIP_PACKETS, n_pkts);
          for (uint32_t q = 0; q < n_pkts; ++q) {
            uint32_t pkt = 0;
            pm = q0;
            for (uint32_t x = 0; x < n_q; ++x) {
#if defined(__CUDA_ARCH__)
              const uint32_t r = __ffs(pm) - 1;
#else
              const uint32_t r = (uint32_t)__builtin_ctz(pm);
#endif
              pm &= pm - 1;
              if (((sends >> (4u * x)) & 15u) > q) pkt |= 1u << r;
            }
            if (!gs_lost(g, imp_loss, sink, i, peers[q], t, GS_LK_GOSSIP, q))
              gs_post(d, g, sink, (t + 1u + gs_extra(g, imp_delay, i, peers[q])) & g.ring_mask, peers[q], pkt);
          }
          np = 0u;
        }
      }
      for (uint32_t q = 0; q < np && queued != 0u; ++q) {
        uint32_t pkt = gs_select_packet(d, g, i, queued);
        if (pkt == 0u) break;
        uint32_t pm = pkt;
        while (pm) {
#if defined(__CUDA_ARCH__)
          uint32_t r = __ffs(pm) - 1;
#else
          uint32_t r = (uint32_t)__builtin_ctz(pm);
#endif
          pm &= pm - 1;
          uint32_t tx = (uint32_t)d.tx[GS_TX(r, cap, i)] + 1u;
          d.tx[GS_TX(r, cap, i)] = (uint8_t)tx;
          if (tx >= g.retransmit_limit) queued &= ~(1u << r);
          sink.stat(GS_ST_RUMORS_SENT, 1);
        }
        sink.stat(GS_ST_GOSSIP_PACKETS, 1);
        if (!gs_lost(g, imp_loss, sink, i, peers[q], t, GS_LK_GOSSIP, q))
          gs_post(d, g, sink, (t + 1u + gs_extra(g, imp_delay, i, peers[q])) & g.ring_mask, peers[q], pkt);
      }
      if (queued != q0) d.queued[i] = queued;
    }

    if (pp_now && !(m & GS_META_ISOLATED)) {
      uint32_t partner[1];
      if (gs_krandom(d, g, i, t, GS_PUR_PUSHPULL, 1u, 1u, GS_EMPTY32, m, partner) != 0u) {
        const uint32_t j = partner[0];
        if (!gs_no_tcp(imp_flags, i, j)) {
          uint32_t* req = d.ppreq + (size_t)nxt * GS_PPK * cap;
          uint32_t v = i;
          for (uint32_t s = 0; s < GS_PPK; ++s) {
            const uint32_t old = GS_ATOMIC_MIN32(&req[(size_t)s * cap + j], v);
            if (old == v || old == GS_EMPTY32) break;
            if (old > v) v = old;
          }
          uint32_t* clk = d.pp_clk + (size_t)nxt * 2u * cap;
          GS_ATOMIC_MAX32(&clk[j], d.ltime_member[i]);
          GS_ATOMIC_MAX32(&clk[cap + j], d.ltime_event[i]);
          gs_post(d, g, sink, inxt, j, (d.heard[i] & g.active_mask) | GS_ACC_BIT);
        }
        sink.stat(GS_ST_PUSH_PULLS, 1);
      }
    }
  }

  if (k != k0) {
    gs_key_store(d, g, nxt, i, k);
    m |= GS_META_DIRTY;
  } else if (m0 & GS_META_DIRTY) {
    gs_key_store(d, g, nxt, i, k);
    m &= ~GS_META_DIRTY;
  }
  if (m != m0) d.meta[i] = m;
  if (due != due0) d.due[i] = due;
  if (gs_key_rank(k) == GS_RANK_SUSPECT || (m & GS_META_DIRTY))
    gs_post(d, g, sink, inxt, i, GS_WAKE_BIT);
  else if (queued != 0u)
    gs_post(d, g, sink, gs_queue_wake_slot(g, t, gslot, gs_meta_gphase(m)), i, GS_WAKE_BIT);
  if constexpr (PIG) {
    if (queued != 0u)
      gs_pig_stamp(d, t, gs_key_rank(k) == GS_RANK_SUSPECT || (m & GS_META_DIRTY) ? 1u
                                                                                    : gs_pig_wake_delta(g, gslot, gs_meta_gphase(m)));
  }
}

template <class Sink>
GS_DEV void gs_row_step(const GsDev& d, const GsGlobals& g, uint32_t i, uint32_t t, uint32_t gslot, uint32_t inb,
                        Sink& sink) {
  if (d.pig != nullptr) {
    if (d.imp_loss != nullptr) gs_row_step_body<true, true>(d, g, i, t, gslot, inb, sink);
    else gs_row_step_body<false, true>(d, g, i, t, gslot, inb, sink);
    return;
  }
  if (d.imp_loss != nullptr) gs_row_step_body<true>(d, g, i, t, gslot, inb, sink);
  else gs_row_step_body<false>(d, g, i, t, gslot, inb, sink);
}

struct GsFastProbe {
  uint32_t k, m, cursor, pass, c, kc;
};

GS_DEV void gs_fast_load(const GsDev& d, uint32_t cur, uint32_t i, GsFastProbe& f) {
  f.k = d.key[cur][i];
  f.m = d.meta[i];
  f.cursor = d.cursor[i];
  f.pass = d.pass[i];
}

template <class G>
GS_DEV bool gs_fast_target(const GsDev& d, const G& g, uint32_t cur, uint32_t i,
                           GsFastProbe& f) {
  if (g.loss_thr != 0u || g.graph_n != 0u || d.coord != nullptr || d.imp_loss != nullptr)
    return false;
  if (gs_key_truth(f.k) != GS_TRUTH_UP || gs_key_rank(f.k) != GS_RANK_ALIVE) return false;
  if (gs_meta_stage(f.m) != GS_STAGE_IDLE || (f.m & (GS_META_DIRTY | GS_META_ISOLATED))) return false;
  if (f.cursor >= g.n) return false;
  GsU4 rk = gs_perm_keys(g.seed_lo, g.seed_hi, i, f.pass);
  f.c = gs_perm(f.cursor, g.n, g.perm_bits, rk);
  if (f.c == i) return false;
  f.kc = gs_peer_key(d, cur, f.c, false);
  return true;
}

template <class G, class Sink>
GS_DEV bool gs_fast_finish(const GsDev& d, const G& g, Sink& sink, uint32_t i, uint32_t t,
                           const GsFastProbe& f, bool* acked) {
  const uint32_t rank = gs_key_rank(f.kc);
  if (gs_key_truth(f.kc) == GS_TRUTH_NONE || rank == GS_RANK_DEAD || rank == GS_RANK_LEFT ||
      gs_key_pending(f.kc))
    return false;
  if (g.pp_interval != 0u && gs_pp_due(g.pp_interval, g.rot_pp, i / g.phase_group, t))
    return false;
  if (d.pig != nullptr && gs_pig_gate(d, t)) return false;
  uint32_t m = f.m;
  if (gs_key_truth(f.kc) == GS_TRUTH_UP && gs_extra(g, nullptr, i, f.c) + gs_extra(g, nullptr, f.c, i) <= g.T) {
    const uint32_t aw = gs_meta_aw(m);
    m = gs_meta_set_aw(m, aw ? aw - 1u : 0u);
    d.due[i] = t + g.P;
    *acked = true;
  } else {
    m = gs_meta_set_stage(m, GS_STAGE_WAIT_T);
    d.probe_tgt[i] = f.c;
    d.probe_inc[i] = GS_PEER_INC(d, t & 1u, f.c, f.kc);
    d.due[i] = t + g.T;
    sink.horizon(t + g.P);
    *acked = false;
  }
  d.cursor[i] = f.cursor + 1u;
  if (m != f.m) d.meta[i] = m;
  return true;
}
```

Baseline: 775,700.

## Add PLAIN template specialization of row step for unimpaired single-GPU pools

Adds a PLAIN compile-time flag threaded through the row-step helpers so that, when the pool has no push-pull, graph, DCs, loss, impairments, piggybacking, coordinates and runs on one GPU, branches on world, loss threshold, DC latency and graph size fold away. System-scope atomics become GPU-scope ones and cross-GPU loads become plain cached loads. The kernel picks the specialized noinline call once per block through a shared flag. This adds another instantiation of the large body, which grows code size and may change register allocation. A new host-emulation step-kind test library is also built.

New measurement: 828,000, median of 6. +6.7%, better.

```diff
diff --git a/__graft_entry__.py b/__graft_entry__.py
--- a/__graft_entry__.py
+++ b/__graft_entry__.py
@@ -10,6 +10,7 @@
 LIBORACLE = os.path.join(ROOT, "oracle", "liboracle.so")
 LIBHOSTEMU = os.path.join(ROOT, "tests", "hostemu", "libgsim_hostemu.so")
 LIBHOSTEMU_COUNTED = os.path.join(ROOT, "tests", "hostemu", "libgsim_hostemu_counted.so")
+LIBHOSTEMU_STEPS = os.path.join(ROOT, "tests", "hostemu", "libgsim_hostemu_steps.so")
 FACADE_DEMO = os.path.join(ROOT, "tests", "hostemu", "serf_facade_check")
 
 NVCC_FLAGS = ["-gencode", "arch=compute_90a,code=sm_90a", "-lineinfo", "-O3", "-std=c++17", "-fmad=false",
@@ -168,6 +169,10 @@
     if force or not _newer(LIBHOSTEMU_COUNTED, csrc + hdr + [os.path.join(ROOT, "tests", "hostemu", "counting_backend.cpp")]):
         _run(["g++", "-O2", "-ffp-contract=off", "-std=c++17", "-pthread", "-fPIC", "-shared",
               "-DGS_MAKE_BACKEND=gs_make_stretch_counting_backend", "-o", LIBHOSTEMU_COUNTED] + csrc)
+    ssrc = hsrc + [os.path.join(ROOT, "tests", "hostemu", "step_kind_backend.cpp")]
+    if force or not _newer(LIBHOSTEMU_STEPS, ssrc + hdr + [os.path.join(ROOT, "tests", "hostemu", "counting_backend.cpp")]):
+        _run(["g++", "-O2", "-ffp-contract=off", "-std=c++17", "-pthread", "-fPIC", "-shared",
+              "-DGS_MAKE_BACKEND=gs_make_step_kind_backend", "-o", LIBHOSTEMU_STEPS] + ssrc)
     sys.path.insert(0, ROOT)
     import consul_b200
 
diff --git a/consul_b200/csrc/gs_cuda.cu b/consul_b200/csrc/gs_cuda.cu
--- a/consul_b200/csrc/gs_cuda.cu
+++ b/consul_b200/csrc/gs_cuda.cu
@@ -19,7 +19,7 @@
 
 namespace {
 
-template <bool COORDS>
+template <bool COORDS, bool ONE_GPU = false>
 struct DevSinkT {
   static constexpr bool kCoords = COORDS;
   uint32_t* s_stat;
@@ -30,13 +30,13 @@
   __device__ __forceinline__ void stat(int idx, uint32_t v) { atomicAdd(&s_stat[idx * 32 + (threadIdx.x & 31u)], v); }
   __device__ __forceinline__ void heard(uint32_t r) { atomicAdd(&s_heard[r * 32u + (threadIdx.x & 31u)], 1u); }
   __device__ __forceinline__ void crashed_dead(const GsDev& d, uint32_t t) {
-    uint32_t old = atomicSub_system(d.crashed_alive, 1u);
+    uint32_t old = ONE_GPU ? atomicSub(d.crashed_alive, 1u) : atomicSub_system(d.crashed_alive, 1u);
     if (old == 1u) *d.crashed_dead_tick = t;
   }
   __device__ __forceinline__ void log_event(const GsDev& d, const GsGlobals& g, uint32_t t,
                                             uint32_t type, uint32_t subject, uint32_t observer,
                                             uint32_t ltime) {
-    uint32_t pos = atomicAdd_system(&d.evlog_cursor[0], 1u);
+    uint32_t pos = ONE_GPU ? atomicAdd(&d.evlog_cursor[0], 1u) : atomicAdd_system(&d.evlog_cursor[0], 1u);
     if (pos < g.evlog_cap) {
       GsEventRec e;
       e.tick = t;
@@ -46,6 +46,8 @@
       e.ltime = ltime;
       e.reserved = 0u;
       d.evlog[pos] = e;
+    } else if (ONE_GPU) {
+      atomicAdd(&d.evlog_cursor[1], 1u);
     } else {
       atomicAdd_system(&d.evlog_cursor[1], 1u);
     }
@@ -144,10 +146,22 @@
   DevSinkT<COORDS> sink{s_stat, s_heard, s_q};
   gs_row_step_body<false>(*dp, *gp, i, t, t % gp->GI, inb, sink);
 }
+__device__ __noinline__ void gs_row_step_plain_call(const GsDev* dp, const GsGlobals* gp, uint32_t i, uint32_t t,
+                                                    uint32_t inb, uint32_t* s_stat, uint32_t* s_heard, uint32_t* s_q) {
+  DevSinkT<false, true> sink{s_stat, s_heard, s_q};
+  gs_row_step_body<false, false, true>(*dp, *gp, i, t, t % gp->GI, inb, sink);
+}
 
 template <bool COORDS>
 __device__ __forceinline__ void gs_row_step_any(const GsDev* dp, const GsGlobals* gp, uint32_t i, uint32_t t,
-                                                uint32_t inb, uint32_t* s_stat, uint32_t* s_heard, uint32_t* s_q) {
+                                                uint32_t inb, uint32_t* s_stat, uint32_t* s_heard, uint32_t* s_q,
+                                                bool plain) {
+  if constexpr (!COORDS) {
+    if (plain) {
+      gs_row_step_plain_call(dp, gp, i, t, inb, s_stat, s_heard, s_q);
+      return;
+    }
+  }
   if (dp->pig == nullptr) gs_row_step_call<COORDS>(dp, gp, i, t, inb, s_stat, s_heard, s_q);
   else if (dp->imp_loss != nullptr) gs_row_step_pig_call<COORDS, true>(dp, gp, i, t, inb, s_stat, s_heard, s_q);
   else gs_row_step_pig_call<COORDS, false>(dp, gp, i, t, inb, s_stat, s_heard, s_q);
@@ -176,6 +190,7 @@
   __shared__ uint16_t s_work[GS_WARPS * GS_ROUND * GS_TILE];
   __shared__ uint32_t s_rtile[GS_WARPS];
   __shared__ uint32_t s_wn[2], s_wtake[2];
+  __shared__ uint32_t s_plain;
   static_assert(GS_WARPS <= 8 && GS_ROUND <= 4 && GS_TILE == 128, "s_work entries are 3 + 2 + 7 bits");
   const uint32_t tid = threadIdx.x;
   for (uint32_t x = tid; x < GS_NSTAT * 32u; x += GS_BLOCK) s_stat[x] = 0u;
@@ -190,6 +205,7 @@
   asm volatile("griddepcontrol.wait;" ::: "memory");
   if (stretch != nullptr && *d.tick_base + k_off >= gs_stretch_stop(*stretch, __ldcg(d.qstate[0] + GS_Q_LAST_ACTIVE)))
     return;
+  if (!COORDS && tid == 70u) s_plain = gs_plain_pool(d, *gp) ? 1u : 0u;
   __syncthreads();
   const GsGlobals& g = *gp;
   const uint32_t t = *d.tick_base + k_off;
@@ -371,7 +387,7 @@
     if (idx + lane < n_work) {
       const uint32_t e = s_work[idx + lane];
       const uint32_t i = (s_rtile[e >> 9] + ((e >> 7) & 3u)) * GS_TILE + (e & 127u);
-      gs_row_step_any<COORDS>(&d, gp, i, t, __ldcg(inbox_cur + i), s_stat, s_heard, s_q);
+      gs_row_step_any<COORDS>(&d, gp, i, t, __ldcg(inbox_cur + i), s_stat, s_heard, s_q, s_plain != 0u);
     }
   }
   __syncthreads();
@@ -407,6 +423,7 @@
   const uint32_t tf0[4] = {tf00, tf01, tf02, tf03}, tx0[4] = {tx00, tx01, tx02, tx03};
   const bool fast_ok =
       h.loss_thr == 0u && h.graph_n == 0u && d.coord == nullptr && d.imp_loss == nullptr && h.pp_interval == 0u;
+  const bool plain = !COORDS && gs_plain_pool(d, g);
   DevSinkT<COORDS> sink{s_stat, s_heard, s_q};
   uint32_t n_probe = 0, n_ack = 0;
   bool did_work = false;
@@ -465,7 +482,7 @@
         for (int which = 0; which < 2; ++which) {
           const uint32_t t = which == 0 ? (a < b ? a : b) : (a < b ? b : a);
           if (t >= w1) break;
-          if (sl && __ldcg(d.due + i) == t) gs_row_step_any<COORDS>(&d, gp, i, t, 0u, s_stat, s_heard, s_q);
+          if (sl && __ldcg(d.due + i) == t) gs_row_step_any<COORDS>(&d, gp, i, t, 0u, s_stat, s_heard, s_q, plain);
         }
       }
     }
diff --git a/consul_b200/csrc/gs_row.h b/consul_b200/csrc/gs_row.h
--- a/consul_b200/csrc/gs_row.h
+++ b/consul_b200/csrc/gs_row.h
@@ -22,16 +22,16 @@
 __device__ __forceinline__ void gs_red_or_gpu(uint32_t* p, uint32_t v) {
   asm volatile("red.global.gpu.or.b32 [%0], %1;" ::"l"(p), "r"(v) : "memory");
 }
-#define GS_ATOMIC_OR32(p, v) (g.world > 1u ? gs_atomic_or_sys((p), (v)) : atomicOr((p), (v)))
+#define GS_ATOMIC_OR32(p, v) (gs_world<PLAIN>(g) > 1u ? gs_atomic_or_sys((p), (v)) : atomicOr((p), (v)))
 #define GS_POST_OR32(p, v)                                                         \
   do {                                                                             \
-    if (g.world <= 1u) gs_red_or_gpu((p), (v));                                    \
+    if (gs_world<PLAIN>(g) <= 1u) gs_red_or_gpu((p), (v));                         \
     else if (g.flags & 128u) (void)gs_atomic_or_sys((p), (v));                     \
     else gs_red_or_sys((p), (v));                                                  \
   } while (0)
 #define GS_ATOMIC_MIN64(p, v)                                                    \
-  (g.world > 1u ? gs_atomic_min_sys((uint64_t*)(p), (uint64_t)(v))               \
-                : (uint64_t)atomicMin((unsigned long long*)(p), (unsigned long long)(v)))
+  (gs_world<PLAIN>(g) > 1u ? gs_atomic_min_sys((uint64_t*)(p), (uint64_t)(v))    \
+                           : (uint64_t)atomicMin((unsigned long long*)(p), (unsigned long long)(v)))
 __device__ __forceinline__ uint32_t gs_ld_sys(const uint32_t* p) {
   uint32_t v;
   asm volatile("ld.relaxed.sys.global.u32 %0, [%1];" : "=r"(v) : "l"(p) : "memory");
@@ -54,8 +54,8 @@
   asm volatile("atom.global.sys.max.u32 %0, [%1], %2;" : "=r"(old) : "l"(p), "r"(v) : "memory");
   return old;
 }
-#define GS_ATOMIC_MIN32(p, v) (g.world > 1u ? gs_atomic_min32_sys((p), (v)) : atomicMin((p), (v)))
-#define GS_ATOMIC_MAX32(p, v) (g.world > 1u ? gs_atomic_max32_sys((p), (v)) : atomicMax((p), (v)))
+#define GS_ATOMIC_MIN32(p, v) (gs_world<PLAIN>(g) > 1u ? gs_atomic_min32_sys((p), (v)) : atomicMin((p), (v)))
+#define GS_ATOMIC_MAX32(p, v) (gs_world<PLAIN>(g) > 1u ? gs_atomic_max32_sys((p), (v)) : atomicMax((p), (v)))
 #else
 #define GS_DEV inline
 #define GS_ATOMIC_OR32(p, v) __atomic_fetch_or((p), (v), __ATOMIC_RELAXED)
@@ -105,12 +105,35 @@
   GS_ST_PUSH_PULLS
 };
 
+GS_DEV bool gs_plain_pool(const GsDev& d, const GsGlobals& g) {
+  return g.pp_interval == 0u && g.graph_n == 0u && g.n_dcs == 0u && g.world <= 1u && g.loss_thr == 0u &&
+         d.imp_loss == nullptr && d.pig == nullptr && d.coord == nullptr;
+}
+template <bool PLAIN, class G>
+GS_DEV uint32_t gs_world(const G& g) { return PLAIN ? 1u : g.world; }
+template <bool PLAIN, class G>
+GS_DEV uint32_t gs_graph_n(const G& g) { return PLAIN ? 0u : g.graph_n; }
+template <bool PLAIN, class G>
+GS_DEV uint32_t gs_n_dcs(const G& g) { return PLAIN ? 0u : g.n_dcs; }
+template <bool PLAIN, class G>
+GS_DEV uint32_t gs_loss_thr(const G& g) { return PLAIN ? 0u : g.loss_thr; }
+template <bool PLAIN, class G>
+GS_DEV uint32_t gs_pp_interval(const G& g) { return PLAIN ? 0u : g.pp_interval; }
+template <bool PLAIN>
+GS_DEV uint64_t gs_ld_other64(const uint64_t* p) {
+#if defined(__CUDA_ARCH__)
+  if (PLAIN) return __ldcg(reinterpret_cast<const unsigned long long*>(p));
+#endif
+  return GS_LD_OTHER64(p);
+}
+
+template <bool PLAIN = false>
 GS_DEV void gs_key_store(const GsDev& d, const GsGlobals& g, uint32_t buf, uint32_t i, uint32_t k) {
   if (d.kst != nullptr) {
     const uint32_t b = d.kst[i], code = gs_kst_code(k);
     d.kst[i] = (uint8_t)(buf ? ((b & 0x0Fu) | (code << 4)) : ((b & 0xF0u) | code));
   }
-  if (g.world <= 1u) {
+  if (gs_world<PLAIN>(g) <= 1u) {
     d.key[buf][i] = k;
     return;
   }
@@ -130,7 +153,7 @@
   return GS_LD_OTHER(&d.key[cur][c]);
 }
 
-template <class Sink>
+template <bool PLAIN = false, class Sink>
 GS_DEV void gs_post(const GsDev& d, const GsGlobals& g, Sink& sink, uint32_t slot, uint32_t j, uint32_t bits) {
   sink.activity();
   GS_POST_OR32(&d.inbox[slot][j], bits);
@@ -151,9 +174,9 @@
   return h;
 }
 
-template <class G>
+template <bool PLAIN = false, class G>
 GS_DEV uint32_t gs_extra(const G& g, const uint8_t* delay, uint32_t src, uint32_t dst) {
-  uint32_t e = g.n_dcs == 0u ? 0u : g.lat[((src / GS_TILE) % g.n_dcs) * GS_MAX_DCS + (dst / GS_TILE) % g.n_dcs];
+  uint32_t e = gs_n_dcs<PLAIN>(g) == 0u ? 0u : g.lat[((src / GS_TILE) % g.n_dcs) * GS_MAX_DCS + (dst / GS_TILE) % g.n_dcs];
   if (delay != nullptr) e += delay[dst];
   return e;
 }
@@ -163,23 +186,25 @@
   const uint32_t* recv;
 };
 
+template <bool PLAIN = false>
 GS_DEV bool gs_loss_rule(const GsGlobals& g, const GsLossCols& loss, const GsU4& r, uint32_t src, uint32_t dst) {
-  return r.x < g.loss_thr || (loss.send != nullptr && (r.y < loss.send[src] || r.z < loss.recv[dst]));
-}
-
+  return r.x < gs_loss_thr<PLAIN>(g) || (loss.send != nullptr && (r.y < loss.send[src] || r.z < loss.recv[dst]));
+}
+
+template <bool PLAIN = false>
 GS_DEV bool gs_lost_quiet(const GsGlobals& g, const GsLossCols& loss, uint32_t src, uint32_t dst, uint32_t t,
                           uint32_t kind, uint32_t idx) {
-  if (g.loss_thr == 0u && loss.send == nullptr) return false;
+  if (gs_loss_thr<PLAIN>(g) == 0u && loss.send == nullptr) return false;
   GsU4 r = gs_philox(g.seed_lo, g.seed_hi, src, dst, t, GS_PUR_LOSS | (kind << 8) | (idx << 16));
-  return gs_loss_rule(g, loss, r, src, dst);
-}
-
-template <class Sink>
+  return gs_loss_rule<PLAIN>(g, loss, r, src, dst);
+}
+
+template <bool PLAIN = false, class Sink>
 GS_DEV bool gs_lost(const GsGlobals& g, const GsLossCols& loss, Sink& sink, uint32_t src, uint32_t dst, uint32_t t,
                     uint32_t kind, uint32_t idx) {
-  if (g.loss_thr == 0u && loss.send == nullptr) return false;
+  if (gs_loss_thr<PLAIN>(g) == 0u && loss.send == nullptr) return false;
   GsU4 r = gs_philox(g.seed_lo, g.seed_hi, src, dst, t, GS_PUR_LOSS | (kind << 8) | (idx << 16));
-  bool lost = gs_loss_rule(g, loss, r, src, dst);
+  bool lost = gs_loss_rule<PLAIN>(g, loss, r, src, dst);
   if (lost) sink.stat(GS_ST_PACKETS_LOST, 1);
   return lost;
 }
@@ -206,12 +231,14 @@
   return false;
 }
 
+template <bool PLAIN = false>
 GS_DEV uint32_t gs_peer_count(const GsDev& d, const GsGlobals& g, uint32_t i) {
-  if (g.graph_n == 0u) return g.n;
+  if (gs_graph_n<PLAIN>(g) == 0u) return g.n;
   return i < g.graph_n ? d.row_ptr[i + 1u] - d.row_ptr[i] : 0u;
 }
+template <bool PLAIN = false>
 GS_DEV uint32_t gs_peer_at(const GsDev& d, const GsGlobals& g, uint32_t i, uint32_t idx) {
-  return g.graph_n == 0u ? idx : d.col_idx[d.row_ptr[i] + idx];
+  return gs_graph_n<PLAIN>(g) == 0u ? idx : d.col_idx[d.row_ptr[i] + idx];
 }
 
 GS_DEV uint32_t gs_coord_slot_for_reader(const uint32_t* ctag, size_t cap, uint32_t j, uint32_t t) {
@@ -257,10 +284,11 @@
   ctag[(size_t)spare * cap + i] = t + 1u;
 }
 
+template <bool PLAIN = false>
 GS_DEV uint32_t gs_krandom(const GsDev& d, const GsGlobals& g, uint32_t i, uint32_t t,
                            uint32_t purpose, uint32_t k, uint32_t mode, uint32_t exclude2,
                            uint32_t meta_i, uint32_t* out) {
-  const uint32_t n = gs_peer_count(d, g, i);
+  const uint32_t n = gs_peer_count<PLAIN>(d, g, i);
   if (n == 0u) return 0u;
   uint32_t tries = 3u * n;
   if (tries > GS_KR_MAX_TRIES || n > 0x55555555u) tries = GS_KR_MAX_TRIES;
@@ -271,7 +299,7 @@
 #pragma unroll
     for (uint32_t x = 0; x < 4u; ++x) {
       const uint32_t draw = gs_u4_get(blk, x);
-      cc[x] = gs_peer_at(d, g, i, g.graph_n == 0u ? gs_fastmod(draw, n, g.n_magic) : draw % n);
+      cc[x] = gs_peer_at<PLAIN>(d, g, i, gs_graph_n<PLAIN>(g) == 0u ? gs_fastmod(draw, n, g.n_magic) : draw % n);
       kk[x] = (b4 * 4u + x < tries && cc[x] != i && cc[x] != exclude2) ? gs_peer_key(d, t & 1u, cc[x], false) : 0u;
     }
 #pragma unroll
@@ -395,6 +423,7 @@
 template <class Sink>
 GS_DEV void gs_pig_owe(const GsDev& d, const GsGlobals& g, Sink& sink, uint32_t nxt, uint32_t inxt, uint32_t sender,
                        uint32_t receiver, uint32_t kind, bool lost) {
+  constexpr bool PLAIN = false;
   uint32_t* req = d.pig_req + (size_t)nxt * GS_PIGK * g.cap;
   uint32_t v = (receiver << 3) | (kind << 1) | (lost ? 1u : 0u);
   bool kept = false;
@@ -433,9 +462,10 @@
   return (w & (GS_WAKE_BIT | GS_ACC_BIT)) == 0u && !due_now && !pp_now && (w & g.active_mask & ~heard) == 0u;
 }
 
-template <bool IMPAIRED, bool PIG = false, class Sink>
+template <bool IMPAIRED, bool PIG = false, bool PLAIN = false, class Sink>
 GS_DEV void gs_row_step_body(const GsDev& d, const GsGlobals& g, uint32_t i, uint32_t t, uint32_t gslot,
                              uint32_t inb, Sink& sink) {
+  static_assert(!PLAIN || (!IMPAIRED && !PIG), "a plain pool has neither degraded members nor piggybacking");
   const GsLossCols imp_loss = {IMPAIRED ? d.imp_loss : nullptr, IMPAIRED ? d.imp_recv : nullptr};
   const uint8_t* const imp_delay = IMPAIRED ? d.imp_delay : nullptr;
   const uint8_t* const imp_flags = IMPAIRED ? d.imp_flags : nullptr;
@@ -454,17 +484,17 @@
   const bool gossip_slot = up && gslot == gs_meta_gphase(m0);
   uint32_t queued = up ? queued0 : 0u;
   if (inb != 0u) d.inbox[icur][i] = 0u;
-  const bool pp_now = up && g.pp_interval != 0u && gs_pp_due(g.pp_interval, g.rot_pp, i / g.phase_group, t);
+  const bool pp_now = up && gs_pp_interval<PLAIN>(g) != 0u && gs_pp_due(g.pp_interval, g.rot_pp, i / g.phase_group, t);
   if (inb != 0u && gs_mail_is_stale(g, inb, heard0, due0 == t, pp_now)) return;
   sink.stat(GS_ST_ACTIVE_ROWS, 1);
 
   if ((inb & ~GS_WAKE_BIT) == 0u && gs_key_rank(k0) == GS_RANK_ALIVE && !(up && due0 == t) &&
       !(gossip_slot && queued != 0u) && !pp_now) {
     if (m0 & GS_META_DIRTY) {
-      gs_key_store(d, g, nxt, i, k0);
+      gs_key_store<PLAIN>(d, g, nxt, i, k0);
       d.meta[i] = m0 & ~GS_META_DIRTY;
     }
-    if (queued != 0u) gs_post(d, g, sink, gs_queue_wake_slot(g, t, gslot, gs_meta_gphase(m0)), i, GS_WAKE_BIT);
+    if (queued != 0u) gs_post<PLAIN>(d, g, sink, gs_queue_wake_slot(g, t, gslot, gs_meta_gphase(m0)), i, GS_WAKE_BIT);
     if constexpr (PIG) {
       if (queued != 0u) gs_pig_stamp(d, t, gs_pig_wake_delta(g, gslot, gs_meta_gphase(m0)));
     }
@@ -476,7 +506,7 @@
   uint32_t heard = 0;
 
   if ((inb & ~GS_WAKE_BIT) != 0u) {
-    if ((inb & GS_ACC_BIT) && g.pp_interval != 0u) {
+    if ((inb & GS_ACC_BIT) && gs_pp_interval<PLAIN>(g) != 0u) {
       uint32_t* clk = d.pp_clk + (size_t)cur * 2u * cap;
       const uint32_t cm = GS_LD_OTHER(&clk[i]), ce = GS_LD_OTHER(&clk[cap + i]);
       if (cm | ce) {
@@ -537,7 +567,7 @@
     if (inb & GS_ACC_BIT) {
       uint64_t* acc = d.acc + (size_t)cur * GS_K1MAX * cap;
       for (uint32_t s = 0; s < GS_K1MAX; ++s) {
-        uint64_t e = GS_LD_OTHER64(&acc[(size_t)s * cap + i]);
+        uint64_t e = gs_ld_other64<PLAIN>(&acc[(size_t)s * cap + i]);
         if (e == GS_EMPTY64) break;
         acc[(size_t)s * cap + i] = GS_EMPTY64;
         uint32_t e_inc = ~(uint32_t)(e >> 32), from = (uint32_t)e;
@@ -562,7 +592,7 @@
         }
       }
     }
-    if ((inb & GS_ACC_BIT) && g.pp_interval != 0u) {
+    if ((inb & GS_ACC_BIT) && gs_pp_interval<PLAIN>(g) != 0u) {
       uint32_t* req = d.ppreq + (size_t)cur * GS_PPK * cap;
       for (uint32_t s = 0; s < GS_PPK; ++s) {
         const uint32_t from = GS_LD_OTHER(&req[(size_t)s * cap + i]);
@@ -572,7 +602,7 @@
         uint32_t* clk = d.pp_clk + (size_t)nxt * 2u * cap;
         GS_ATOMIC_MAX32(&clk[from], d.ltime_member[i]);
         GS_ATOMIC_MAX32(&clk[cap + from], d.ltime_event[i]);
-        gs_post(d, g, sink, inxt, from, (d.heard[i] & g.active_mask) | GS_ACC_BIT);
+        gs_post<PLAIN>(d, g, sink, inxt, from, (d.heard[i] & g.active_mask) | GS_ACC_BIT);
       }
     }
     if constexpr (PIG) {
@@ -586,7 +616,7 @@
           gs_pig_count(d, i, GS_PIG_ST_SERVED, 1u);
           const uint32_t pkt = gs_pig_take(d, g, i, queued, (e >> 1) & 3u);
           if (pkt != 0u && !(e & 1u))
-            gs_post(d, g, sink, (t + 1u + gs_extra(g, imp_delay, i, e >> 3)) & g.ring_mask, e >> 3, pkt);
+            gs_post<PLAIN>(d, g, sink, (t + 1u + gs_extra<PLAIN>(g, imp_delay, i, e >> 3)) & g.ring_mask, e >> 3, pkt);
         }
       }
     }
@@ -626,7 +656,7 @@
       const bool j_up = gs_key_truth(kj) == GS_TRUTH_UP;
       uint32_t relays[8];
       uint32_t kk = g.indirect_checks > 8u ? 8u : g.indirect_checks;
-      uint32_t nr = gs_krandom(d, g, i, t, GS_PUR_RELAY, kk, 1u, j, m, relays);
+      uint32_t nr = gs_krandom<PLAIN>(d, g, i, t, GS_PUR_RELAY, kk, 1u, j, m, relays);
       bool success = false;
       uint32_t nacks = 0;
       const uint32_t budget = g.P * (gs_meta_aw(m) + 1u) - g.T;
@@ -637,39 +667,39 @@
         const bool r_up = gs_key_truth(gs_peer_key(d, cur, r, false)) == GS_TRUTH_UP;
         sink.stat(GS_ST_INDIRECT_PINGS, 1);
         if constexpr (PIG) {
-          const bool req_lost = gs_lost_quiet(g, imp_loss, i, r, t, GS_LK_INDREQ, q);
+          const bool req_lost = gs_lost_quiet<PLAIN>(g, imp_loss, i, r, t, GS_LK_INDREQ, q);
           const uint32_t pkt = gs_pig_take(d, g, i, queued, GS_PIG_INDREQ);
-          if (pkt != 0u && !req_lost) gs_post(d, g, sink, (t + 1u + gs_extra(g, imp_delay, i, r)) & g.ring_mask, r, pkt);
+          if (pkt != 0u && !req_lost) gs_post<PLAIN>(d, g, sink, (t + 1u + gs_extra<PLAIN>(g, imp_delay, i, r)) & g.ring_mask, r, pkt);
           if (pig_gate && r_up && !req_lost) {
-            const bool ping_lost = gs_lost_quiet(g, imp_loss, r, j, t, GS_LK_INDPING, q);
+            const bool ping_lost = gs_lost_quiet<PLAIN>(g, imp_loss, r, j, t, GS_LK_INDPING, q);
             gs_pig_owe(d, g, sink, nxt, inxt, r, j, GS_PIG_PING, ping_lost);
-            const bool ack_lost = gs_lost_quiet(g, imp_loss, j, r, t, GS_LK_INDACK, q);
+            const bool ack_lost = gs_lost_quiet<PLAIN>(g, imp_loss, j, r, t, GS_LK_INDACK, q);
             if (j_up && !ping_lost) gs_pig_owe(d, g, sink, nxt, inxt, j, r, GS_PIG_ACK, ack_lost);
             const bool acked = j_up && !ping_lost && !ack_lost &&
-                               gs_extra(g, imp_delay, r, j) + gs_extra(g, imp_delay, j, r) <= g.T;
+                               gs_extra<PLAIN>(g, imp_delay, r, j) + gs_extra<PLAIN>(g, imp_delay, j, r) <= g.T;
             if (acked)
-              gs_pig_owe(d, g, sink, nxt, inxt, r, i, GS_PIG_ACK, gs_lost_quiet(g, imp_loss, r, i, t, GS_LK_INDFWD, q));
+              gs_pig_owe(d, g, sink, nxt, inxt, r, i, GS_PIG_ACK, gs_lost_quiet<PLAIN>(g, imp_loss, r, i, t, GS_LK_INDFWD, q));
             else
-              gs_pig_owe(d, g, sink, nxt, inxt, r, i, GS_PIG_NACK, gs_lost_quiet(g, imp_loss, r, i, t, GS_LK_NACK, q));
+              gs_pig_owe(d, g, sink, nxt, inxt, r, i, GS_PIG_NACK, gs_lost_quiet<PLAIN>(g, imp_loss, r, i, t, GS_LK_NACK, q));
           }
         }
-        if (!(r_up && !gs_lost(g, imp_loss, sink, i, r, t, GS_LK_INDREQ, q))) continue;
-        const uint32_t via = gs_extra(g, imp_delay, i, r) + gs_extra(g, imp_delay, r, i);
-        const uint32_t rtt_rj = gs_extra(g, imp_delay, r, j) + gs_extra(g, imp_delay, j, r);
-        bool relay_acked = j_up && !gs_lost(g, imp_loss, sink, r, j, t, GS_LK_INDPING, q) &&
-                           !gs_lost(g, imp_loss, sink, j, r, t, GS_LK_INDACK, q) && rtt_rj <= g.T;
+        if (!(r_up && !gs_lost<PLAIN>(g, imp_loss, sink, i, r, t, GS_LK_INDREQ, q))) continue;
+        const uint32_t via = gs_extra<PLAIN>(g, imp_delay, i, r) + gs_extra<PLAIN>(g, imp_delay, r, i);
+        const uint32_t rtt_rj = gs_extra<PLAIN>(g, imp_delay, r, j) + gs_extra<PLAIN>(g, imp_delay, j, r);
+        bool relay_acked = j_up && !gs_lost<PLAIN>(g, imp_loss, sink, r, j, t, GS_LK_INDPING, q) &&
+                           !gs_lost<PLAIN>(g, imp_loss, sink, j, r, t, GS_LK_INDACK, q) && rtt_rj <= g.T;
         if (relay_acked) {
-          if (!gs_lost(g, imp_loss, sink, r, i, t, GS_LK_INDFWD, q) && via + rtt_rj <= budget) success = true;
-        } else if (!gs_lost(g, imp_loss, sink, r, i, t, GS_LK_NACK, q) && via <= budget) {
+          if (!gs_lost<PLAIN>(g, imp_loss, sink, r, i, t, GS_LK_INDFWD, q) && via + rtt_rj <= budget) success = true;
+        } else if (!gs_lost<PLAIN>(g, imp_loss, sink, r, i, t, GS_LK_NACK, q) && via <= budget) {
           ++nacks;
           sink.stat(GS_ST_NACKS, 1);
         }
       }
       const uint32_t t0 = t - g.T;
-      const uint32_t rtt_ij = gs_extra(g, imp_delay, i, j) + gs_extra(g, imp_delay, j, i);
+      const uint32_t rtt_ij = gs_extra<PLAIN>(g, imp_delay, i, j) + gs_extra<PLAIN>(g, imp_delay, j, i);
       if (!g.disable_tcp && j_up && rtt_ij <= budget && !gs_no_tcp(imp_flags, i, j)) success = true;
-      if ((g.n_dcs != 0u || imp_delay != nullptr) && j_up && rtt_ij > g.T && rtt_ij <= budget + g.T &&
-          !gs_lost_quiet(g, imp_loss, i, j, t0, GS_LK_PING, 0) && !gs_lost_quiet(g, imp_loss, j, i, t0, GS_LK_ACK, 0))
+      if ((gs_n_dcs<PLAIN>(g) != 0u || imp_delay != nullptr) && j_up && rtt_ij > g.T && rtt_ij <= budget + g.T &&
+          !gs_lost_quiet<PLAIN>(g, imp_loss, i, j, t0, GS_LK_PING, 0) && !gs_lost_quiet<PLAIN>(g, imp_loss, j, i, t0, GS_LK_ACK, 0))
         success = true;
       if (success) {
         uint32_t aw = gs_meta_aw(m);
@@ -698,14 +728,14 @@
         if (old == v || old == GS_EMPTY64) break;
         if (old > v) v = old;
       }
-      gs_post(d, g, sink, inxt, j, GS_ACC_BIT);
+      gs_post<PLAIN>(d, g, sink, inxt, j, GS_ACC_BIT);
       sink.stat(GS_ST_PROBE_FAILURES, 1);
       stage = GS_STAGE_IDLE;
     }
     if (stage == GS_STAGE_IDLE && due == t) {
       uint32_t cursor = d.cursor[i], pass = d.pass[i];
-      const uint32_t n = gs_peer_count(d, g, i);
-      const uint32_t hb = g.graph_n == 0u ? g.perm_bits : gs_perm_bits_of(n);
+      const uint32_t n = gs_peer_count<PLAIN>(d, g, i);
+      const uint32_t hb = gs_graph_n<PLAIN>(g) == 0u ? g.perm_bits : gs_perm_bits_of(n);
       GsU4 rk = gs_perm_keys(g.seed_lo, g.seed_hi, i, pass);
       uint32_t checked = 0, target = GS_EMPTY32, ktarget = 0;
       const uint32_t limit = n < GS_PROBE_SKIP_CAP ? n : GS_PROBE_SKIP_CAP;
@@ -717,7 +747,7 @@
           rk = gs_perm_keys(g.seed_lo, g.seed_hi, i, pass);
           continue;
         }
-        uint32_t c = gs_peer_at(d, g, i, gs_perm(cursor, n, hb, rk));
+        uint32_t c = gs_peer_at<PLAIN>(d, g, i, gs_perm(cursor, n, hb, rk));
         ++cursor;
         uint32_t kc = gs_peer_key(d, cur, c, false);
         uint32_t rank = gs_key_rank(kc);
@@ -735,16 +765,16 @@
       if (target != GS_EMPTY32) {
         sink.stat(GS_ST_PROBES, 1);
         if constexpr (PIG) {
-          const bool ping_lost = gs_lost_quiet(g, imp_loss, i, target, t, GS_LK_PING, 0);
+          const bool ping_lost = gs_lost_quiet<PLAIN>(g, imp_loss, i, target, t, GS_LK_PING, 0);
           const uint32_t pkt = gs_pig_take(d, g, i, queued, GS_PIG_PING);
           if (pkt != 0u && !ping_lost)
-            gs_post(d, g, sink, (t + 1u + gs_extra(g, imp_delay, i, target)) & g.ring_mask, target, pkt);
+            gs_post<PLAIN>(d, g, sink, (t + 1u + gs_extra<PLAIN>(g, imp_delay, i, target)) & g.ring_mask, target, pkt);
           if (gs_pig_gate(d, t) && gs_key_truth(ktarget) == GS_TRUTH_UP && !ping_lost)
-            gs_pig_owe(d, g, sink, nxt, inxt, target, i, GS_PIG_ACK, gs_lost_quiet(g, imp_loss, target, i, t, GS_LK_ACK, 0));
-        }
-        bool ok = gs_key_truth(ktarget) == GS_TRUTH_UP && !gs_lost(g, imp_loss, sink, i, target, t, GS_LK_PING, 0) &&
-                  !gs_lost(g, imp_loss, sink, target, i, t, GS_LK_ACK, 0) &&
-                  gs_extra(g, imp_delay, i, target) + gs_extra(g, imp_delay, target, i) <= g.T;
+            gs_pig_owe(d, g, sink, nxt, inxt, target, i, GS_PIG_ACK, gs_lost_quiet<PLAIN>(g, imp_loss, target, i, t, GS_LK_ACK, 0));
+        }
+        bool ok = gs_key_truth(ktarget) == GS_TRUTH_UP && !gs_lost<PLAIN>(g, imp_loss, sink, i, target, t, GS_LK_PING, 0) &&
+                  !gs_lost<PLAIN>(g, imp_loss, sink, target, i, t, GS_LK_ACK, 0) &&
+                  gs_extra<PLAIN>(g, imp_delay, i, target) + gs_extra<PLAIN>(g, imp_delay, target, i) <= g.T;
         if (ok) {
           uint32_t aw = gs_meta_aw(m);
           m = gs_meta_set_aw(m, aw ? aw - 1u : 0u);
@@ -782,7 +812,7 @@
           tx8 |= (uint64_t)d.tx[GS_TX(r, cap, i)] << (8u * x);
         }
       }
-      uint32_t np = gs_krandom(d, g, i, t, GS_PUR_GOSSIP, kk, 0u, GS_EMPTY32, m, peers);
+      uint32_t np = gs_krandom<PLAIN>(d, g, i, t, GS_PUR_GOSSIP, kk, 0u, GS_EMPTY32, m, peers);
       const uint32_t q0 = queued;
       if (whole && np != 0u) {
         uint32_t sends = 0, n_pkts = 0, n_q = 0, pm = queued;
@@ -825,8 +855,8 @@
               pm &= pm - 1;
               if (((sends >> (4u * x)) & 15u) > q) pkt |= 1u << r;
             }
-            if (!gs_lost(g, imp_loss, sink, i, peers[q], t, GS_LK_GOSSIP, q))
-              gs_post(d, g, sink, (t + 1u + gs_extra(g, imp_delay, i, peers[q])) & g.ring_mask, peers[q], pkt);
+            if (!gs_lost<PLAIN>(g, imp_loss, sink, i, peers[q], t, GS_LK_GOSSIP, q))
+              gs_post<PLAIN>(d, g, sink, (t + 1u + gs_extra<PLAIN>(g, imp_delay, i, peers[q])) & g.ring_mask, peers[q], pkt);
           }
           np = 0u;
         }
@@ -848,15 +878,15 @@
           sink.stat(GS_ST_RUMORS_SENT, 1);
         }
         sink.stat(GS_ST_GOSSIP_PACKETS, 1);
-        if (!gs_lost(g, imp_loss, sink, i, peers[q], t, GS_LK_GOSSIP, q))
-          gs_post(d, g, sink, (t + 1u + gs_extra(g, imp_delay, i, peers[q])) & g.ring_mask, peers[q], pkt);
+        if (!gs_lost<PLAIN>(g, imp_loss, sink, i, peers[q], t, GS_LK_GOSSIP, q))
+          gs_post<PLAIN>(d, g, sink, (t + 1u + gs_extra<PLAIN>(g, imp_delay, i, peers[q])) & g.ring_mask, peers[q], pkt);
       }
       if (queued != q0) d.queued[i] = queued;
     }
 
     if (pp_now && !(m & GS_META_ISOLATED)) {
       uint32_t partner[1];
-      if (gs_krandom(d, g, i, t, GS_PUR_PUSHPULL, 1u, 1u, GS_EMPTY32, m, partner) != 0u) {
+      if (gs_krandom<PLAIN>(d, g, i, t, GS_PUR_PUSHPULL, 1u, 1u, GS_EMPTY32, m, partner) != 0u) {
         const uint32_t j = partner[0];
         if (!gs_no_tcp(imp_flags, i, j)) {
           uint32_t* req = d.ppreq + (size_t)nxt * GS_PPK * cap;
@@ -869,7 +899,7 @@
           uint32_t* clk = d.pp_clk + (size_t)nxt * 2u * cap;
           GS_ATOMIC_MAX32(&clk[j], d.ltime_member[i]);
           GS_ATOMIC_MAX32(&clk[cap + j], d.ltime_event[i]);
-          gs_post(d, g, sink, inxt, j, (d.heard[i] & g.active_mask) | GS_ACC_BIT);
+          gs_post<PLAIN>(d, g, sink, inxt, j, (d.heard[i] & g.active_mask) | GS_ACC_BIT);
         }
         sink.stat(GS_ST_PUSH_PULLS, 1);
       }
@@ -877,18 +907,18 @@
   }
 
   if (k != k0) {
-    gs_key_store(d, g, nxt, i, k);
+    gs_key_store<PLAIN>(d, g, nxt, i, k);
     m |= GS_META_DIRTY;
   } else if (m0 & GS_META_DIRTY) {
-    gs_key_store(d, g, nxt, i, k);
+    gs_key_store<PLAIN>(d, g, nxt, i, k);
     m &= ~GS_META_DIRTY;
   }
   if (m != m0) d.meta[i] = m;
   if (due != due0) d.due[i] = due;
   if (gs_key_rank(k) == GS_RANK_SUSPECT || (m & GS_META_DIRTY))
-    gs_post(d, g, sink, inxt, i, GS_WAKE_BIT);
+    gs_post<PLAIN>(d, g, sink, inxt, i, GS_WAKE_BIT);
   else if (queued != 0u)
-    gs_post(d, g, sink, gs_queue_wake_slot(g, t, gslot, gs_meta_gphase(m)), i, GS_WAKE_BIT);
+    gs_post<PLAIN>(d, g, sink, gs_queue_wake_slot(g, t, gslot, gs_meta_gphase(m)), i, GS_WAKE_BIT);
   if constexpr (PIG) {
     if (queued != 0u)
       gs_pig_stamp(d, t, gs_key_rank(k) == GS_RANK_SUSPECT || (m & GS_META_DIRTY) ? 1u
@@ -905,6 +935,7 @@
     return;
   }
   if (d.imp_loss != nullptr) gs_row_step_body<true>(d, g, i, t, gslot, inb, sink);
+  else if (gs_plain_pool(d, g)) gs_row_step_body<false, false, true>(d, g, i, t, gslot, inb, sink);
   else gs_row_step_body<false>(d, g, i, t, gslot, inb, sink);
 }
 
```
